# zhenxuan00/graphical-gan

Measured on AMD Instinct MI355X. Metric: images/sec (G+D+GP step) cifar10 32x32 bs=64, higher is better.
Workload: dtype f32; 1 GPU; gan_inference_cifar10.py MODE=wali-gp BATCH_SIZE=64 (per GPU) 32x32x3, CRITIC_ITERS=5; parallelism=dp1, global_batch=64, hip_graph=True, minibatch_feed=device-resident ring, read in place; one graph per iteration, finite_costs=True

## Files before the change

graphical_gan_amd/_lib.py:

```python
import ctypes as C
import os

_HERE = os.path.dirname(os.path.abspath(__file__))
LIB_PATH = os.path.join(_HERE, 'libggan.so')

ACT_NONE, ACT_LRELU, ACT_RELU, ACT_TANH, ACT_SIGMOID = 0, 1, 2, 3, 4
PACK_MAX = 64
HEAD_BCE_MAX_ROWS = 2048
BCE_HEADS = 2
PACK_ARRIVE_INTS = 33 * 1024
POSTERIOR_MAX_K = 8192
MODE_K = {'CONCRETE': 0, 'STRAIGHT_THROUGHT_CONCRETE': 1, 'STRAIGHT_THROUGHT': 2}
BCE_MAX = 16
TSNE_MAX_K = 128
TSNE_MAX_SPLITS = 64
ABI_VERSION = 800


class ConvGeom(C.Structure):
    _fields_ = [(n, C.c_int) for n in ('N', 'Ci', 'H', 'W', 'Co', 'Ho', 'Wo', 'k', 'stride', 'pad_t', 'pad_l',
                                       'plan_wgs', 'plan_wgs_filter', 'plan_flags')]


PLAN_PLAIN = 1


class ProfRec(C.Structure):
    _fields_ = [('name', C.c_char * 48), ('total_ms', C.c_double), ('launches', C.c_long),
                ('flops', C.c_double), ('bytes', C.c_double), ('grid', C.c_long)]


class GganError(RuntimeError):
    pass


_P = C.c_void_p
_F = C.c_float
_I = C.c_int
_Z = C.c_size_t
_G = C.POINTER(ConvGeom)

SIGNATURES = {
    'ggan_version': (_I, []),
    'ggan_last_error': (C.c_char_p, []),
    'ggan_conv2d_workspace': (_Z, [_G]),
    'ggan_conv2d_fwd': (_I, [_G, _P, _P, _P, _P, _I, _F, _P, _Z, _P]),
    'ggan_conv2d_bwd_data': (_I, [_G, _P, _P, _P, _P, _I, _F, _P, _Z, _P]),
    'ggan_conv2d_bwd_filter': (_I, [_G, _P, _P, _P, _P, _P, _Z, _P]),
    'ggan_conv2d_bwd_data_act': (_I, [_G, _P, _P, _I, _F, _P, _P, _P, _Z, _P]),
    'ggan_conv2d_bwd_filter_act': (_I, [_G, _P, _P, _P, _I, _F, _P, _P, _P, _Z, _P]),
    'ggan_conv2d_bwd_filter_parts': (_I, [_G, _P, _P, _P, _I, _F, _I, _P, _Z, C.POINTER(_I), C.POINTER(_Z), _P]),
    'ggan_conv2d_fwd_cast_ring': (_I, [_G, _P, _I, _P, _P, _I, _P, _F, _F, _P, _P, _P, _P, _I, _F, _P]),
    'ggan_conv2d_fwd_masked': (_I, [_G, _P, _P, _P, _P, _I, _F, _P, _Z, _P]),
    'ggan_linear_bn_rows_fwd': (_I, [_P, _P, _P, _P, _P, _P, _P, _P, _P, _I, _I, _I, _F, _I, _F, _P]),
    'ggan_linear_bn_rows_bwd': (_I, [_P, _P, _P, _P, _P, _P, _P, _P, _P, _P, _P, _I, _I, _I, _I, _F, _P]),
    'ggan_deconv2d_fwd': (_I, [_G, _P, _P, _P, _P, _I, _F, _P, _Z, _P]),
    'ggan_deconv2d_bwd_data': (_I, [_G, _P, _P, _P, _P, _Z, _P]),
    'ggan_deconv2d_bwd_filter': (_I, [_G, _P, _P, _P, _P, _P, _Z, _P]),
    'ggan_gemm_workspace': (_Z, [_I, _I, _I]),
    'ggan_gemm': (_I, [_I, _I, _I, _I, _I, _P, _P, _P, _P, _I, _F, _P, _Z, _P]),
    'ggan_conv3d_out_shape': (_I, [_P, _P]),
    'ggan_im2col3d': (_I, [_P, _P, _P, _P]),
    'ggan_col2im3d': (_I, [_P, _P, _P, _P]),
    'ggan_conv3d_igemm_ok': (_I, [_P, _I]),
    'ggan_conv3d_fwd': (_I, [_P, _P, _P, _P, _P, _I, _F, _P, _Z, _P]),
    'ggan_conv3d_wgrad': (_I, [_P, _P, _P, _P, _P, _Z, _P]),
    'ggan_conv3d_dgrad': (_I, [_P, _P, _P, _P, _P]),
    'ggan_mix_rbf_mmd2_fwd': (_I, [_P, _P, _I, _I, _I, _P, _P, _I, _P, _P, _P]),
    'ggan_mix_rbf_mmd2_bwd': (_I, [_P, _P, _I, _I, _I, _P, _P, _I, _P, _P, _P, _P]),
    'ggan_noise_fill': (_I, [_P, _P, _P, _P, _P, _P, _I, _P, _P]),
    'ggan_gmm_latent_fwd': (_I, [_P, _P, _P, _P, _P, _I, _I, _I, _F, _F, _P]),
    'ggan_gmm_latent_bwd': (_I, [_P, _P, _P, _P, _P, _P, _P, _I, _I, _I, _F, _P]),
    'ggan_gmm_latent_st_fwd': (_I, [_P, _P, _P, _P, _P, _P, _I, _I, _I, _F, _F, _I, _P]),
    'ggan_gmm_latent_st_bwd': (_I, [_P, _P, _P, _P, _P, _P, _P, _I, _I, _I, _F, _I, _P]),
    'ggan_gmm_posterior_assign': (_I, [_P, _P, _F, _I, _I, _I, _I, _P, _P, _P, _P]),
    'ggan_cluster_accuracy': (_I, [_P, _P, _P, _I, _I, _P, _P]),
    'ggan_video_sheet_u8': (_I, [_P, _P, _P, _P, _I, _I, _I, _I, _I, _I, _I, _I, _I, _F, _F, _F, _P]),
    'ggan_tsne_sqnorms': (_I, [_P, _I, _I, _P, _P]),
    'ggan_tsne_neighbours': (_I, [_P, _P, _I, _I, _I, _I, _I, _P, _P, _P, _P, _Z, _P]),
    'ggan_tsne_affinities': (_I, [_P, _I, _I, _F, _I, _F, _P, _P, _P]),
    'ggan_tsne_symmetrise': (_I, [_P, _P, _I, _I, _P, _P, _P, _P, _P]),
    'ggan_tsne_gradient': (_I, [_P, _P, _P, _P, _I, _I, _P, _P, _P, _P, _P, _P]),
    'ggan_tsne_kl': (_I, [_P, _P, _P, _P, _I, _I, _P, _P, _P, _P, _P]),
    'ggan_tsne_iterate': (_I, [_P, _P, _P, _P, _P, _P, _P, _I, _I, _P, _P, _I, _I, _I, _F, _F, _F, _F, _F, _P]),
    'ggan_gemm_split': (_I, [_I, _I, _I, _I, _I, _P, _P, _I, _P, _P, _P, _P, _I, _P, _I, _F, _P, _Z, _P]),
    'ggan_gemm_colsum': (_I, [_I, _I, _I, _I, _P, _P, _P, _P, _P, _Z, _P]),
    'ggan_dyn_scan_fwd': (_I, [_I, _I, _I, _I, _I, _P, _P, _P, _P, _P, _P, _P, _P, _P, _P, _F, _P, _P, _P, _P]),
    'ggan_dyn_scan_bwd': (_I, [_I, _I, _I, _I, _I, _P, _P, _P, _P, _P, _P, _P, _P, _P, _F, _P, _P, _P, _P, _P, _P, _P]),
    'ggan_critic_head_fwd': (_I, [_I, _I, _I, _I, _P, _P, _P, _P, _P, _P, _F, _P, _P, _P, _Z, _P]),
    'ggan_critic_head_bwd': (_I, [_I, _I, _I, _I, _P, _P, _P, _P, _P, _P, _F, _P, _P, _P, _P, _P, _P, _P, _P, _Z, _P]),
    'ggan_critic_head_fwd_bce': (_I, [_I, _I, _I, _I, _P, _P, _P, _P, _P, _P, _F, _P, _P, _I, _I, _P, _P, _P, _P, _P, _P, _Z, _P]),
    'ggan_critic_head_bwd_tail': (_I, [_I, _I, _I, _I, _P, _P, _P, _P, _P, _F, _P, _P, _P, _P, _P, _P, _P, _P, _P, _I, _I, _P, _P, _P, _P, _P, _P, _Z, _P]),
    'ggan_linear_bwd_data_act': (_I, [_I, _I, _I, _P, _P, _I, _F, _P, _P, _P, _Z, _P]),
    'ggan_linear_bwd_weight_act': (_I, [_I, _I, _I, _P, _P, _P, _I, _F, _P, _P, _P, _Z, _P]),
    'ggan_colsum': (_I, [_P, _P, _I, _I, _P]),
    'ggan_reparam_fwd': (_I, [_P, _P, _P, _P, _P, _Z, _P]),
    'ggan_reparam_bwd': (_I, [_P, _P, _P, _P, _P, _P, _Z, _P]),
    'ggan_agg_div_fwd': (_I, [_I, _P, _P, _P, _P, _P, _I, _I, _I, _I, _P, _P, _P, _P, _P, _P]),
    'ggan_agg_div_bwd': (_I, [_I, _P, _P, _P, _P, _I, _I, _I, _I, _P, _P, _P, _P, _P, _P, _P, _P, _P]),
    'ggan_colsum_tall': (_I, [_P, _P, _I, _I, _P, _Z, _P]),
    'ggan_chansum': (_I, [_P, _P, _I, _I, _I, _P, _Z, _P]),
    'ggan_bn_fwd_train': (_I, [_P, _P, _P, _P, _P, _P, _I, _I, _I, _F, _I, _F, _P]),
    'ggan_bn_bwd': (_I, [_P, _P, _P, _P, _P, _P, _P, _P, _I, _I, _I, _P]),
    'ggan_bn_bwd_act': (_I, [_P, _P, _P, _I, _F, _P, _P, _P, _P, _P, _P, _P, _I, _I, _I, _P]),
    'ggan_bn_bwd_bwd': (_I, [_P, _P, _P, _I, _F, _P, _P, _P, _P, _P, _P, _P, _I, _I, _I, _P]),
    'ggan_bn_split_fwd_train': (_I, [_P, _P, _P, _P, _P, _P, _I, _I, _I, _I, _F, _I, _F, _P, _Z, _P]),
    'ggan_bn_split_bwd_act': (_I, [_P, _P, _I, _F, _P, _P, _P, _P, _P, _P, _P, _P, _I, _I, _I, _I, _I, _P, _Z, _P]),
    'ggan_bn_sync_stats': (_I, [_P, _P, _I, _I, _I, _P]),
    'ggan_bn_sync_apply': (_I, [_P, _P, _I, _P, _P, _P, _P, _P, _I, _I, _I, _F, _I, _F, _P]),
    'ggan_bn_sync_bwd_stats': (_I, [_P, _P, _P, _I, _F, _P, _P, _P, _I, _I, _I, _P]),
    'ggan_bn_sync_bwd_apply': (_I, [_P, _P, _P, _I, _F, _P, _P, _P, _P, _I, _I, _P, _P, _P, _I, _I, _I, _P]),
    'ggan_act_fwd': (_I, [_P, _P, _Z, _I, _F, _P]),
    'ggan_act_bwd': (_I, [_P, _P, _P, _Z, _I, _F, _P]),
    'ggan_act_bwd_chansum': (_I, [_P, _P, _P, _P, _I, C.POINTER(_I), _I, _I, _I, _I, _F, _P]),
    'ggan_bias_add': (_I, [_P, _P, _P, _I, _I, _I, _P]),
    'ggan_cast_scale_i32': (_I, [_P, _P, _P, _Z, _F, _F, _P]),
    'ggan_cast_scale_ring_i32': (_I, [_P, _I, _P, _P, _I, _P, _P, _Z, _F, _F, _P]),
    'ggan_axpby': (_I, [_P, _P, _P, _Z, _F, _F, _F, _P]),
    'ggan_mix_mean': (_I, [_P, _P, _P, _P, _I, _I, _I, _P]),
    'ggan_row_lerp': (_I, [_P, _P, _P, _P, _I, _I, _P]),
    'ggan_bce_logits_fwd': (_I, [_P, _F, _F, _P, _I, _I, _P]),
    'ggan_bce_logits_bwd': (_I, [_P, _F, _F, _P, _P, _I, _P]),
    'ggan_bce_logits_multi_fwd': (_I, [C.POINTER(_P), C.POINTER(_F), C.POINTER(_F), C.POINTER(_I), _I, _P, _P]),
    'ggan_bce_logits_multi_bwd': (_I, [C.POINTER(_P), C.POINTER(_F), C.POINTER(_F), C.POINTER(_I), _I, _P, C.POINTER(_P), _P]),
    'ggan_bce_logits_multi_fwd_grad': (_I, [C.POINTER(_P), C.POINTER(_F), C.POINTER(_F), C.POINTER(_I), _I, _P, C.POINTER(_P), _P]),
    'ggan_bce_head_bwd': (_I, [C.POINTER(_P), C.POINTER(_F), C.POINTER(_F), C.POINTER(_I), _I, _P, C.POINTER(_P), _I, _I, _P, _P, _F, _P, _P,
                          _P, _P]),
    'ggan_bce_heads_bwd': (_I, [C.POINTER(_P), C.POINTER(_F), C.POINTER(_F), C.POINTER(_I), _I, _P, C.POINTER(_P), _I, C.POINTER(_I),
                           C.POINTER(_I), C.POINTER(_I), C.POINTER(_P), C.POINTER(_P), C.POINTER(_F), C.POINTER(_P), C.POINTER(_P),
                           C.POINTER(_P), _P]),
    'ggan_mean_fwd': (_I, [_P, _F, _P, _I, _I, _P]),
    'ggan_mean_bwd': (_I, [_P, _F, _P, _I, _P]),
    'ggan_mean_multi_fwd_grad': (_I, [C.POINTER(_P), C.POINTER(_F), C.POINTER(_I), _I, _P, C.POINTER(_P), _P]),
    'ggan_dist_fwd': (_I, [_P, _P, _P, _Z, _I, _F, _I, _P]),
    'ggan_dist_bwd': (_I, [_P, _P, _P, _P, _P, _Z, _I, _F, _P]),
    'ggan_gp_penalty_fwd': (_I, [_P, _P, _P, _I, _I, _F, _P]),
    'ggan_gp_penalty_bwd': (_I, [_P, _P, _P, _P, _I, _I, _F, _P]),
    'ggan_gp_penalty_fwd_grad': (_I, [_P, _P, _P, _P, _P, _I, _I, _F, _P]),
    'ggan_adam_step': (_I, [_P, _P, _P, _P, _Z, _P, _F, _F, _F, _F, _F, _P]),
    'ggan_adam_advance': (_I, [_P, _P]),
    'ggan_rmsprop_step': (_I, [_P, _P, _P, _Z, _F, _F, _F, _F, _F, _F, _P]),
    'ggan_adam_step_counted': (_I, [_P, _P, _P, _P, _Z, _P, _F, _F, _F, _F, _F, _P]),
    'ggan_pack': (_I, [C.POINTER(_P), C.POINTER(_Z), C.POINTER(_Z), _I, _P, _P]),
    'ggan_pack_parts': (_I, [C.POINTER(_P), C.POINTER(_Z), C.POINTER(_Z), C.POINTER(_I), C.POINTER(_Z), _I, _P, _P, _P]),
    'ggan_pack_parts2': (_I, [C.POINTER(_P), C.POINTER(_Z), C.POINTER(_Z), C.POINTER(_I), C.POINTER(_Z), C.POINTER(_P), C.POINTER(_I),
                              C.POINTER(_Z), _I, _P, _P, _P]),
    'ggan_pack_adam': (_I, [C.POINTER(_P), C.POINTER(_Z), C.POINTER(_Z), C.POINTER(_I), C.POINTER(_Z), C.POINTER(_P), C.POINTER(_I),
                            C.POINTER(_Z), _I, _P, _P, _P, _P, _P, _P, _F, _F, _F, _F, _F, _P]),
    'ggan_prof_enable': (_I, [_I]),
    'ggan_prof_reset': (_I, []),
    'ggan_prof_report': (_I, [C.POINTER(ProfRec), _I]),
}

_lib = None


def load():
    global _lib
    if _lib is not None:
        return _lib
    if not os.path.exists(LIB_PATH):
        raise GganError('libggan.so not found at %s -- run `python -c "import __graft_entry__ as g; g.build()"` '
                        '(there is no CPU fallback)' % LIB_PATH)
    lib = C.CDLL(LIB_PATH)
    for name, (res, args) in SIGNATURES.items():
        try:
            fn = getattr(lib, name)
        except AttributeError:
            raise GganError('libggan.so does not export %s' % name)
        fn.restype = res
        fn.argtypes = args
    if lib.ggan_version() != ABI_VERSION:
        raise GganError('libggan.so speaks ABI version %d, this binding %d: a stale build -- run `python -c "import __graft_entry__ as g; g.build()"`'
                        % (lib.ggan_version(), ABI_VERSION))
    _lib = lib
    return lib


def check(rc, what):
    if rc != 0:
        msg = load().ggan_last_error()
        raise GganError('%s failed (%d): %s' % (what, rc, msg.decode() if msg else ''))


def prof_report(cap=256):
    lib = load()
    recs = (ProfRec * cap)()
    n = lib.ggan_prof_report(recs, cap)
    out = []
    for i in range(n):
        r = recs[i]
        out.append(dict(name=r.name.decode(), total_ms=r.total_ms, launches=int(r.launches),
                        flops=r.flops, bytes=r.bytes, grid=int(r.grid)))
    return out
```

graphical_gan_amd/csrc/conv.h:

```cpp
#pragma once
#include "common.h"

namespace ggan {

int conv_fwd_naive(const ggan_conv_geom& g, const float* x, const float* w, const float* bias, float* y, int act,
                   float alpha, hipStream_t s);
struct GyMask {
    const float* ref;
    int act;
    float alpha;
};
int conv_dgrad_naive(const ggan_conv_geom& g, const float* gy, GyMask m, const float* w, const float* bias, float* gx,
                     int act, float alpha, hipStream_t s);
int conv_wgrad_naive(const ggan_conv_geom& g, const float* x, const float* gy, GyMask m, float* gw, hipStream_t s);

constexpr int kTargetWgs = 200;
struct OutMask {
    const float* ref;
    int act;
    float alpha;
    bool applied;
};
int conv_fwd_mfma(const ggan_conv_geom& g, const float* x, const float* w, const float* bias, float* y, int act,
                  float alpha, void* ws, size_t ws_bytes, hipStream_t s, OutMask* mask = nullptr);
int conv_dgrad_mfma(const ggan_conv_geom& g, const float* gy, GyMask m, const float* w, const float* bias, float* gx,
                    int act, float alpha, void* ws, size_t ws_bytes, hipStream_t s);
int conv_dgrad_dg16(const ggan_conv_geom& g, const float* gy, GyMask m, const float* w, const float* bias, float* gx, int act,
                    float alpha, int target_wgs, void* ws, size_t ws_bytes, hipStream_t s);
int conv_dgrad_thin(const ggan_conv_geom& g, const float* gy, GyMask m, const float* w, const float* bias, float* gx, int act,
                    float alpha, hipStream_t s);
struct WgradParts {
    float* buf;
    size_t cap_floats;
    int with_bias;
    int n;
    size_t stride;
};
int conv_wgrad_mfma(const ggan_conv_geom& g, const float* x, const float* gy, GyMask m, float* gw, float* gbias, void* ws,
                    size_t ws_bytes, hipStream_t s, WgradParts* parts = nullptr);
struct ThinCastSrc {
    const int32_t* ring;
    const int32_t* ctr_a;
    const int32_t* ctr_b;
    const float* noise;
    float* x_out;
    int nslots, offset;
    float div, mul;
};
int conv_fwd_thin(const ggan_conv_geom& g, const float* x, const float* w, const float* bias, float* y, int act, float alpha,
                  hipStream_t s, const ThinCastSrc* cast = nullptr, const OutMask* mask = nullptr);
int conv_wgrad_thin(const ggan_conv_geom& g, const float* x, const float* gy, GyMask m, float* gw, float* gbias, void* ws,
                    size_t ws_bytes, hipStream_t s, WgradParts* parts = nullptr);
size_t conv_workspace_bytes(const ggan_conv_geom& g);
int launch_splitk_reduce(const float* partial, int SK, size_t elems, float* out, const float* bias, int C, int HW, int act,
                         float alpha, hipStream_t s, size_t slab_stride = 0, float* tail_out = nullptr, size_t tail = 0);

struct FastDiv {
    uint32_t mul, d;
};
inline FastDiv make_fastdiv(uint32_t d) {
    FastDiv f;
    f.d = d;
    f.mul = (d <= 1) ? 0u : (uint32_t)((0x100000000ull / d) + 1ull);
    return f;
}
__device__ __forceinline__ uint32_t fdiv(uint32_t n, FastDiv f) { return f.d <= 1 ? n : __umulhi(n, f.mul); }

struct FastDiv24 {
    uint32_t mul, shift;
};
inline bool make_fastdiv24(uint32_t d, uint32_t nmax, FastDiv24* out) {
    if (d <= 1) { out->mul = 1; out->shift = 0; return true; }
    for (int s = 31; s >= 1; --s) {
        const uint64_t m = ((1ull << s) + d - 1) / d;
        if (m >= (1ull << 24) || m * nmax >= (1ull << 32)) continue;
        const uint64_t err = m * d - (1ull << s);
        if ((uint64_t)nmax * err >= (1ull << s)) return false;
        out->mul = (uint32_t)m; out->shift = (uint32_t)s;
        return true;
    }
    return false;
}
__device__ __forceinline__ uint32_t fdiv24(uint32_t n, FastDiv24 f) { return __umul24(n, f.mul) >> f.shift; }

}
```

graphical_gan_amd/csrc/conv_corr.hip:

```cpp
#include "common.h"
#include "conv.h"
#include <stdlib.h>
#include <map>
#include <mutex>
#include <vector>
using namespace ggan;

namespace {

constexpr int XE_MAX = 24;
constexpr unsigned OOB = 0x7FFFFFF0u;
typedef unsigned int u32x4 __attribute__((ext_vector_type(4)));

__host__ __device__ inline int fwd_region(int data_floats, int lanes_used, int floats_per_lane) {
    const int tail = (((lanes_used + 63) & ~63) - lanes_used) * floats_per_lane;
    return (data_floats + (tail > 4 ? tail : 4) + 3) & ~3;
}

struct CorrClass {
    int Hu, Wv;
    int roff, coff;
    int or0, oc0;
    int wbase;
    int pad_;
// ... 910 lines not shown
    const std::vector<int> key = {dev, P.CKtot, P.Hin, P.Win, P.TI, P.TR, P.TC, P.SR, P.SCp, P.CS, xq, P.row0, P.col0, CK, nthr, P.tiles_r, P.tiles_c, su};
    std::lock_guard<std::mutex> lk(g_xtab_mu);
    auto it = g_xtabs.find(key);
    if (it != g_xtabs.end()) return it->second;
    hipStreamCaptureStatus st = hipStreamCaptureStatusNone;
    if (hipStreamIsCapturing(s, &st) != hipSuccess || st != hipStreamCaptureStatusNone) { (void)hipGetLastError(); return nullptr; }
    const int CSu = P.CS / xq, SCpu = P.SCp / xq, srsc = P.SR * SCpu, xe_cnt = CK * CSu;
    const int npos = P.tiles_r * P.tiles_c;
    std::vector<unsigned> tab((size_t)npos * XE * nthr, OOB);
    for (int tr = 0; tr < P.tiles_r; ++tr)
        for (int tc = 0; tc < P.tiles_c; ++tc) {
            const int in_row0 = su * tr * P.TR + P.row0, in_col0 = su * tc * P.TC + P.col0;
            for (int j = 0; j < XE; ++j)
                for (int tid = 0; tid < nthr; ++tid) {
                    const int e = tid + j * nthr;
                    if (e >= xe_cnt) continue;
                    const int ckl = e / CSu, r1 = e - ckl * CSu;
                    const int img = r1 / srsc, r2 = r1 - img * srsc;
                    const int r = r2 / SCpu, cc = (r2 - r * SCpu) * xq;
                    const int ih = in_row0 + r, iw = in_col0 + cc;
                    if (img >= P.TI || ih < 0 || ih >= P.Hin || iw < 0 || iw >= P.Win) continue;
                    tab[((size_t)(tr * P.tiles_c + tc) * XE + j) * nthr + tid] = (unsigned)((((size_t)img * P.CKtot + ckl) * P.Hin + ih) * P.Win + iw) * 4u;
                }
        }
    unsigned* d = nullptr;
    if (hipMalloc((void**)&d, tab.size() * sizeof(unsigned)) != hipSuccess) { (void)hipGetLastError(); return nullptr; }
    if (hipMemcpy(d, tab.data(), tab.size() * sizeof(unsigned), hipMemcpyHostToDevice) != hipSuccess) { (void)hipGetLastError(); (void)hipFree(d); return nullptr; }
    g_xtabs[key] = d;
    return d;
}

template <int MODE>
int plan_and_launch(CorrParams& P, int Hu, int Wv, int su, int ext_r, int ext_c, int ntaps, int groups, float* dst,
                    const float* bias, int act, float alpha, void* ws, size_t ws_bytes, hipStream_t s, const char* name,
                    double fl, const char* sk_env, OutMask* mask = nullptr) {
    const int target = P.plan_wgs > 0 ? P.plan_wgs : kTargetWgs;
    const WaveCfg* kCfgs = MODE == 1 ? kCfgsDgrad : kCfgsFwd;
    static const int order_fwd[4] = {8, 6, 4, 5}, order_all[4] = {8, 6, 7, 5};
    const int* order = MODE == 2 ? order_all : order_fwd;
    int cfg = 5;
    for (int oi = MODE == 0 ? 0 : 1; oi < 4; ++oi) {
        const int c = order[oi];
        const WaveCfg& wc = kCfgs[c];
        const int CK = 2 * wc.KS * wc.PW, TM = 32 * wc.WM, TNW = 32 * wc.WN;
        if (P.CNtot <= 32 && TNW > 32) continue;
        CorrParams T = P;
        if (!pick_tile(T, Hu, Wv, TM, CK, su, ext_r, ext_c)) continue;
        if (oi < 3 && T.TI * T.TR * T.TC * 2 <= TM && Hu * Wv * P.N >= TM) continue;
        const int wgs = cdiv(P.N, T.TI) * cdiv(Hu, T.TR) * cdiv(Wv, T.TC) * cdiv(P.CNtot, TNW) * groups;
        if (oi == 0 && wgs >= 2 * target) continue;
        if (wgs >= target || oi == 3) { cfg = c; break; }
    }
    if (P.CKtot < 8) cfg = P.CNtot <= 32 ? 1 : 6;
    const WaveCfg& wc = kCfgs[cfg];
    const int CK = 2 * wc.KS * wc.PW, TM = 32 * wc.WM, TNW = 32 * wc.WN;
    if (!pick_tile(P, Hu, Wv, TM, CK, su, ext_r, ext_c)) return 1;
    P.dbg = env_int("GGAN_DBG", 0);
    P.dma = (MODE == 0 || (CK % 16 == 0 && wc.PW <= 2)) && (P.dbg & 3) == 0;
    const int RS = TNW + (MODE != 0 ? 2 : 0);
    P.xq = 1;
    if (MODE == 0 && cfg >= 4 && P.dma && (P.Win & 3) == 0 && (((uintptr_t)P.in) & 15) == 0 && ((su * P.TC) & 3) == 0) {
        const int shift = ((P.col0 % 4) + 4) % 4;
        const int scp4 = (P.SCp + shift + 3) & ~3;
        const size_t cs4 = (size_t)P.TI * P.SR * scp4;
        const int wregion = fwd_region(ntaps * CK * RS, ntaps * CK * (TNW / 4), 4);
        const size_t stage4 = 2 * ((size_t)fwd_region((int)(CK * cs4), (int)(CK * cs4 / 4), 4) + (size_t)wregion);
        const size_t stage1 = 2 * ((size_t)fwd_region(CK * P.CS, CK * P.CS, 1) + (size_t)wregion);
        const bool crosses = stage1 * sizeof(float) <= 80 * 1024 && stage4 * sizeof(float) > 80 * 1024;
        if (stage4 * sizeof(float) <= 160 * 1024 && CK * cs4 / 4 <= (size_t)XE_MAX * 256 && !crosses) {
            P.xq = 4;
            P.col0 -= shift;
            for (int c = 0; c < 4; ++c) P.cls[c].coff += shift;
            P.SCp = scp4;
            P.CS = (int)cs4;
        }
    }
    if (MODE != 0 && dgrad_x4_cfg(MODE, cfg) && (P.Win & 3) == 0 && (((uintptr_t)P.in) & 15) == 0 &&
        (((uintptr_t)P.in_ref) & 15) == 0 && ((su * P.TC) & 3) == 0) {
        const int shift = ((P.col0 % 4) + 4) % 4;
        const int scp4 = (P.SCp + shift + 3) & ~3;
        const size_t cs4 = (size_t)P.TI * P.SR * scp4;
        const int nthr = 64 * wc.WM * wc.WN * wc.KS;
        const int xn = ((XE_MAX / 2) * 256 / nthr + 3) / 4 + 1;
        const size_t stage4 = 2 * ((size_t)((CK * cs4 + 1 + 3) & ~(size_t)3) + (size_t)((ntaps * CK * RS + 4 * RS + 3) & ~3));
        if (stage4 * sizeof(float) <= 160 * 1024 && CK * cs4 / 4 <= (size_t)xn * nthr) {
            P.xq = 4;
            P.col0 -= shift;
            for (int c = 0; c < 4; ++c) P.cls[c].coff += shift;
            P.SCp = scp4;
            P.CS = (int)cs4;
        }
    }
    if (!finish_tile(P, Hu, Wv)) return 1;
    if ((size_t)P.N * P.CKtot * P.Hin >= (1u << 24)) return 1;
    const int gx = P.img_groups * P.tiles_r * P.tiles_c, gy = cdiv(P.CNtot, TNW);
    int sk = env_int(sk_env, 0);
    if (sk <= 0) {
        sk = 1;
        const int base = gx * gy * groups;
        if (base < target / 2) {
            sk = target / base;
            const int max_sk = P.CKtot / (2 * CK);
            if (sk > max_sk) sk = max_sk;
            if (sk > 16) sk = 16;
        }
    }
    if (sk < 1) sk = 1;
    P.cps = cdiv(cdiv(P.CKtot, sk), CK) * CK;
    P.SK = cdiv(P.CKtot, P.cps);
    if (P.SK > 1 && (size_t)P.SK * P.out_elems * sizeof(float) > ws_bytes) {
        P.SK = 1;
        P.cps = cdiv(P.CKtot, CK) * CK;
    }
    P.out = P.SK > 1 ? (float*)ws : dst;
    P.bias = bias; P.act = act; P.alpha = alpha;
    if (mask) {
        if (MODE != 0 || P.SK != 1) return 1;
        P.out_ref = mask->ref; P.out_act = mask->act; P.out_alpha = mask->alpha;
        mask->applied = true;
    }
    if ((P.dbg & 4) && ws && ws_bytes > (64u << 20)) P.stamps = (unsigned long long*)((char*)ws + ws_bytes - (32u << 20));
    size_t stage = MODE == 0 ? 2 * ((size_t)fwd_region(CK * P.CS, CK * P.CS / P.xq, P.xq) + (size_t)fwd_region(ntaps * CK * RS, ntaps * CK * (TNW / 4), 4))
                             : 2 * ((size_t)((CK * P.CS + 1 + 3) & ~3) + (size_t)((ntaps * CK * RS + 4 * RS + 3) & ~3));
    size_t red = (size_t)wc.KS * (MODE == 2 ? 4 : (MODE == 1 ? 2 : 1)) * TNW * TM;
    P.nstg = 2;
    if (MODE == 0 && P.dma) P.xtab = fwd_slab_table(P, CK, 64 * wc.WM * wc.WN * wc.KS, su, s);
    const size_t shmem = (stage > red ? stage : red) * sizeof(float);
    {
        P.xcd_p = 0;
        if ((gx * gy) % 8 == 0) {
            double best = (gx % 8 == 0) ? (double)P.in_bytes + 8.0 * P.w_bytes : 8.0 * ((double)P.in_bytes + P.w_bytes);
            for (int p = 1; p <= 8; p *= 2) {
                if (gx % p || gy % (8 / p)) continue;
                const double cost = 8.0 * P.in_bytes / p + (double)P.w_bytes * p;
                if (cost < 0.9 * best) { best = cost; P.xcd_p = p; }
            }
        }
    }
    int rc = launch_cfg<MODE>(cfg, P, dim3(gx, gy, groups * P.SK), shmem, s, name, fl);
    if (rc) return rc;
    if (P.SK > 1)
        return launch_splitk_reduce((const float*)ws, P.SK, P.out_elems, dst, bias, P.CNtot, P.Hout * P.Wout, act, alpha, s);
    return 0;
}

}

namespace ggan {

int launch_splitk_reduce(const float* partial, int SK, size_t elems, float* out, const float* bias, int C, int HW, int act,
                         float alpha, hipStream_t s, size_t slab_stride, float* tail_out, size_t tail) {
    if (slab_stride == 0) slab_stride = elems;
    if (!tail_out) tail = 0;
    if (SK >= 8 && elems + tail <= 65536) {
        GGAN_LAUNCH("splitk_reduce_small_k", 0, 4.0 * (elems + tail) * (SK + 1), splitk_reduce_small_k,
                    dim3((int)((elems + tail + 63) / 64)), dim3(256), 0, s, partial, SK, elems, slab_stride, out, bias, C, HW, act,
                    alpha, tail_out, tail);
        return 0;
    }
    size_t b = (elems + tail + 255) / 256;
    if (b > 2048) b = 2048;
    GGAN_LAUNCH("splitk_reduce_k", 0, 4.0 * (elems + tail) * (SK + 1), splitk_reduce_k, dim3((int)b), dim3(256), 0, s, partial,
                SK, elems, slab_stride, out, bias, C, HW, act, alpha, tail_out, tail);
    return 0;
}

size_t conv_workspace_bytes(const ggan_conv_geom& g) {
    size_t big = (size_t)g.N * g.Ci * g.H * g.W, small_ = (size_t)g.N * g.Co * g.Ho * g.Wo;
    size_t wsz = (size_t)g.k * g.k * g.Ci * g.Co;
    size_t m = big > small_ ? big : small_;
    size_t a = 16 * m * sizeof(float), b = 64 * wsz * sizeof(float);
    return a > b ? a : b;
}

static bool hot_geometry(const ggan_conv_geom& g) { return g.k == 5 && g.stride == 2; }
static bool fits32(size_t bytes) { return bytes < 0x7FFFFFF0ull; }

int conv_fwd_mfma(const ggan_conv_geom& g, const float* x, const float* w, const float* bias, float* y, int act,
                  float alpha, void* ws, size_t ws_bytes, hipStream_t s, OutMask* mask) {
    if (!hot_geometry(g) || (g.Co & 3)) return 1;
    ws = ws_scratch(ws, ws_bytes);
    const size_t in_bytes = (size_t)g.N * g.Ci * g.H * g.W * 4, w_bytes = (size_t)25 * g.Ci * g.Co * 4;
    if (!fits32(in_bytes) || !fits32(w_bytes) || !fits32((size_t)g.N * g.Co * g.Ho * g.Wo * 4)) return 1;
    if (((uintptr_t)w & 15) != 0) return 1;
    CorrParams P;
    memset(&P, 0, sizeof(P));
    P.in = x; P.w = w;
    P.plan_wgs = g.plan_wgs;
    P.in_bytes = (unsigned)in_bytes; P.w_bytes = (unsigned)w_bytes;
    P.N = g.N; P.CKtot = g.Ci; P.Hin = g.H; P.Win = g.W;
    P.CNtot = g.Co; P.Hout = g.Ho; P.Wout = g.Wo;
    P.ors = 1; P.ocs = 1;
    P.w_si = g.k * g.Ci * g.Co; P.w_sj = g.Ci * g.Co; P.w_sk = g.Co; P.w_sn = 1;
    P.row0 = -g.pad_t; P.col0 = -g.pad_l;
    CorrClass& c = P.cls[0];
    c.Hu = g.Ho; c.Wv = g.Wo; c.roff = 0; c.coff = 0; c.or0 = 0; c.oc0 = 0; c.wbase = 0;
    P.out_elems = (size_t)g.N * g.Co * g.Ho * g.Wo;
    const double fl = 2.0 * P.out_elems * g.Ci * 25.0;
    return plan_and_launch<0>(P, g.Ho, g.Wo, 2, 5, 5, 25, 1, y, bias, act, alpha, ws, ws_bytes, s, "conv_fwd_mfma", fl,
                              "GGAN_FWD_SK", mask);
}

int conv_dgrad_mfma(const ggan_conv_geom& g, const float* gy, GyMask m, const float* w, const float* bias, float* gx,
                    int act, float alpha, void* ws, size_t ws_bytes, hipStream_t s) {
    if (!hot_geometry(g)) return 1;
    ws = ws_scratch(ws, ws_bytes);
    if ((g.Co & 3) || ((uintptr_t)w & 15)) return 1;
    const size_t in_bytes = (size_t)g.N * g.Co * g.Ho * g.Wo * 4, w_bytes = (size_t)25 * g.Ci * g.Co * 4;
    if (!fits32(in_bytes) || !fits32(w_bytes) || !fits32((size_t)g.N * g.Ci * g.H * g.W * 4)) return 1;
    const int S = 2;
    CorrParams P;
    memset(&P, 0, sizeof(P));
    P.in = gy; P.w = w;
    P.plan_wgs = g.plan_wgs;
    if (m.act != GGAN_ACT_NONE && m.act != GGAN_ACT_LRELU && m.act != GGAN_ACT_RELU) return 1;
    if (m.act != GGAN_ACT_NONE) { P.in_ref = m.ref; P.in_act = m.act; P.in_alpha = m.alpha; }
    P.in_bytes = (unsigned)in_bytes; P.w_bytes = (unsigned)w_bytes;
    P.N = g.N; P.CKtot = g.Co; P.Hin = g.Ho; P.Win = g.Wo;
    P.CNtot = g.Ci; P.Hout = g.H; P.Wout = g.W;
    P.ors = S; P.ocs = S;
    P.w_si = S * g.k * g.Ci * g.Co; P.w_sj = S * g.Ci * g.Co; P.w_sk = 1; P.w_sn = g.Co;
    int offs[2][2], bases[2][2], cnt[2][2], th[2][2], lo[2], hi[2];
    for (int d = 0; d < 2; ++d) {
        const int pad = d == 0 ? g.pad_t : g.pad_l, L = d == 0 ? g.H : g.W;
        lo[d] = 1 << 30; hi[d] = -(1 << 30);
        for (int p = 0; p < S; ++p) {
            const int off = ((p - pad) % S + S) % S;
            offs[d][p] = off;
            bases[d][p] = (off + pad - p) / S;
            cnt[d][p] = off < L ? (L - off + S - 1) / S : 0;
            th[d][p] = (g.k - p + S - 1) / S;
            if (bases[d][p] - (th[d][p] - 1) < lo[d]) lo[d] = bases[d][p] - (th[d][p] - 1);
            if (bases[d][p] > hi[d]) hi[d] = bases[d][p];
        }
    }
    const int Hu = cnt[0][0] > cnt[0][1] ? cnt[0][0] : cnt[0][1];
    const int Wv = cnt[1][0] > cnt[1][1] ? cnt[1][0] : cnt[1][1];
    P.row0 = lo[0]; P.col0 = lo[1];
    for (int ph = 0; ph < S; ++ph)
        for (int pw = 0; pw < S; ++pw) {
            CorrClass& c = P.cls[ph * 2 + pw];
            c.Hu = cnt[0][ph]; c.Wv = cnt[1][pw];
            c.roff = bases[0][ph] - lo[0]; c.coff = bases[1][pw] - lo[1];
            c.or0 = offs[0][ph]; c.oc0 = offs[1][pw];
            c.wbase = (ph * g.k + pw) * g.Ci * g.Co;
        }
    P.out_elems = (size_t)g.N * g.Ci * g.H * g.W;
    const double fl = 2.0 * g.N * g.Co * g.Ho * g.Wo * (double)g.Ci * 25.0;
    const long wgs_all = (long)cdiv(g.N * Hu * Wv, 32) * cdiv(g.Ci, 32);
    if (wgs_all >= (g.plan_wgs > 0 ? g.plan_wgs : kTargetWgs))
        return plan_and_launch<2>(P, Hu, Wv, 1, hi[0] - lo[0] + 1, hi[1] - lo[1] + 1, 25, 1, gx, bias, act, alpha, ws, ws_bytes,
                                  s, "conv_dgrad_mfma", fl, "GGAN_DGRAD_SK");
    return plan_and_launch<1>(P, Hu, Wv, 1, hi[0] - lo[0] + 1, hi[1] - lo[1] + 1, 13, 2, gx, bias, act, alpha, ws, ws_bytes,
                              s, "conv_dgrad_mfma", fl, "GGAN_DGRAD_SK");
}

}
```

graphical_gan_amd/csrc/gemm.hip:

```cpp
#include "common.h"
#include "conv.h"
#include <stdlib.h>
using namespace ggan;

namespace {

constexpr int BM = 64, BN = 64, BK = 16, LDP = 68;
constexpr int KSTEP = 32;
constexpr int LDPK = 66;

struct GemmParams {
    const float* A;
    const float* B;
    const float* bias;
    float* C;
    int M, N, K;
    int lda, ldb;
    int kps;
    int SK;
    int vecA, vecB;
    int act;
    float alpha;
    size_t out_elems;
    float* colsum;
// ... 401 lines not shown

template <int NWAVE>
__global__ __launch_bounds__(64 * NWAVE) void gemm_group_kernel(const GemmGroup G) {
    warm_kernarg(G);
    __shared__ __attribute__((aligned(16))) float As[2 * TSZ];
    __shared__ __attribute__((aligned(16))) float Bs[2 * TSZ];
    if (G.has_tail && (int)blockIdx.x >= G.tail.first) {
        head_tail_wg(G.tail, (int)blockIdx.x - G.tail.first, As);
        return;
    }
    int j = 0;
    if (G.n > 1 && (int)blockIdx.x >= G.first[1]) j = 1;
    if (G.n > 2 && (int)blockIdx.x >= G.first[2]) j = 2;
    const int local = blockIdx.x - G.first[j];
    const int bx = local % G.gx[j], by = local / G.gx[j];
    const GemmParams& P = G.p[j];
    switch (G.kind[j]) {
        case 0: gemm_tile<true, false, 0, 1, NWAVE>(P, bx, by, 0, As, Bs); break;
        case 1: gemm_tile<false, true, 0, 1, NWAVE>(P, bx, by, 0, As, Bs); break;
        default: gemm_tile<false, false, 0, 1, NWAVE>(P, bx, by, 0, As, Bs); break;
    }
}

__global__ __launch_bounds__(256) void head_out_fwd_k(const float* __restrict__ part, int SK, size_t slab, const float* __restrict__ b,
                                                      const float* __restrict__ w_out, const float* __restrict__ b_out, float alpha,
                                                      float* __restrict__ h, float* __restrict__ logits, int M, int H) {
    __shared__ float red[4];
    const int tid = threadIdx.x, rl = tid >> 7, t = tid & 127;
    const int row = blockIdx.x * 2 + rl;
    float dot = 0.f;
    if (row < M) {
        for (int c = t * 4; c < H; c += 512) {
            const size_t o = (size_t)row * H + c;
            float4 v = *reinterpret_cast<const float4*>(part + o);
#pragma unroll 8
            for (int s = 1; s < SK; ++s) {
                const float4 u = *reinterpret_cast<const float4*>(part + (size_t)s * slab + o);
                v.x += u.x; v.y += u.y; v.z += u.z; v.w += u.w;
            }
            const float4 bb = *reinterpret_cast<const float4*>(b + c);
            const float4 ww = *reinterpret_cast<const float4*>(w_out + c);
            v.x = fmaxf(alpha * (v.x + bb.x), v.x + bb.x); v.y = fmaxf(alpha * (v.y + bb.y), v.y + bb.y);
            v.z = fmaxf(alpha * (v.z + bb.z), v.z + bb.z); v.w = fmaxf(alpha * (v.w + bb.w), v.w + bb.w);
            *reinterpret_cast<float4*>(h + o) = v;
            dot = fmaf(v.x, ww.x, fmaf(v.y, ww.y, fmaf(v.z, ww.z, fmaf(v.w, ww.w, dot))));
        }
    }
    dot = wave_sum(dot);
    if ((tid & 63) == 0) red[tid >> 6] = dot;
    __syncthreads();
    if (t == 0 && row < M) logits[row] = (red[2 * rl] + red[2 * rl + 1]) + b_out[0];
}

__global__ __launch_bounds__(256) void head_out_fwd_bce_k(const float* __restrict__ part, int SK, size_t slab, const float* __restrict__ b,
                                                          const float* __restrict__ w_out, const float* __restrict__ b_out, float alpha,
                                                          float* __restrict__ h, float* __restrict__ logits, int M, int H,
                                                          const HeadTerms T, float* __restrict__ g_out, float* __restrict__ gh) {
    __shared__ float red[4];
    const int tid = threadIdx.x, rl = tid >> 7, t = tid & 127;
    const int row = blockIdx.x * 2 + rl;
    float dot = 0.f;
    float4 hv[4], wv[4];
#pragma unroll
    for (int it = 0; it < 4; ++it) {
        const int c = t * 4 + it * 512;
        if (row < M && c < H) {
            const size_t o = (size_t)row * H + c;
            float4 v = *reinterpret_cast<const float4*>(part + o);
#pragma unroll 8
            for (int s = 1; s < SK; ++s) {
                const float4 u = *reinterpret_cast<const float4*>(part + (size_t)s * slab + o);
                v.x += u.x; v.y += u.y; v.z += u.z; v.w += u.w;
            }
            const float4 bb = *reinterpret_cast<const float4*>(b + c);
            const float4 ww = *reinterpret_cast<const float4*>(w_out + c);
            v.x = fmaxf(alpha * (v.x + bb.x), v.x + bb.x); v.y = fmaxf(alpha * (v.y + bb.y), v.y + bb.y);
            v.z = fmaxf(alpha * (v.z + bb.z), v.z + bb.z); v.w = fmaxf(alpha * (v.w + bb.w), v.w + bb.w);
            *reinterpret_cast<float4*>(h + o) = v;
            dot = fmaf(v.x, ww.x, fmaf(v.y, ww.y, fmaf(v.z, ww.z, fmaf(v.w, ww.w, dot))));
            hv[it] = v; wv[it] = ww;
        }
    }
    dot = wave_sum(dot);
    if ((tid & 63) == 0) red[tid >> 6] = dot;
    __syncthreads();
    if (row >= M) return;
    const float lg = (red[2 * rl] + red[2 * rl + 1]) + b_out[0];
    if (t == 0) logits[row] = lg;
    float z = 0.f, sc = 0.f;
    {
        int r0 = 0;
        for (int k = 0; k < T.count; ++k) {
            if (T.ext[k]) continue;
            if (row >= r0 && row < r0 + T.rows[k]) { z = T.z[k]; sc = 1.f * T.w[k] / (float)T.rows[k]; }
            r0 += T.rows[k];
        }
    }
    const float gr = T.kind == 1 ? sc : sc * (1.f / (1.f + expf(-lg)) - z);
    if (t == 0) g_out[row] = gr;
#pragma unroll
    for (int it = 0; it < 4; ++it) {
        const int c = t * 4 + it * 512;
        if (c < H) {
            float4 o4;
            o4.x = gr * wv[it].x * (hv[it].x > 0.f ? 1.f : alpha); o4.y = gr * wv[it].y * (hv[it].y > 0.f ? 1.f : alpha);
            o4.z = gr * wv[it].z * (hv[it].z > 0.f ? 1.f : alpha); o4.w = gr * wv[it].w * (hv[it].w > 0.f ? 1.f : alpha);
            *reinterpret_cast<float4*>(gh + (size_t)row * H + c) = o4;
        }
    }
}

__global__ __launch_bounds__(256) void head_out_bwd_k(const float* __restrict__ g, const float* __restrict__ h,
                                                      const float* __restrict__ w_out, float alpha, float* __restrict__ gh,
                                                      float* __restrict__ d_wout, float* __restrict__ d_bout, int M, int H) {
    __shared__ float red[16][16];
    const int tid = threadIdx.x, cl = tid & 15, rg = tid >> 4;
    const int c = blockIdx.x * 16 + cl;
    float acc = 0.f, gs = 0.f;
    if (c < H) {
        const float w = w_out[c];
#pragma unroll 8
        for (int r = rg; r < M; r += 16) {
            const float gr = g[r], hv = h[(size_t)r * H + c];
            gh[(size_t)r * H + c] = gr * w * (hv > 0.f ? 1.f : alpha);
            acc = fmaf(gr, hv, acc);
            gs += gr;
        }
    }
    red[rg][cl] = acc;
    __syncthreads();
    if (rg == 0 && c < H && d_wout)
        d_wout[c] = (((red[0][cl] + red[1][cl]) + (red[2][cl] + red[3][cl])) + ((red[4][cl] + red[5][cl]) + (red[6][cl] + red[7][cl]))) +
                    (((red[8][cl] + red[9][cl]) + (red[10][cl] + red[11][cl])) + ((red[12][cl] + red[13][cl]) + (red[14][cl] + red[15][cl])));
    if (blockIdx.x == 0 && d_bout) {
        __syncthreads();
        if (cl == 0) red[rg][0] = gs;
        __syncthreads();
        if (tid == 0) d_bout[0] = (((red[0][0] + red[1][0]) + (red[2][0] + red[3][0])) + ((red[4][0] + red[5][0]) + (red[6][0] + red[7][0]))) +
                                (((red[8][0] + red[9][0]) + (red[10][0] + red[11][0])) + ((red[12][0] + red[13][0]) + (red[14][0] + red[15][0])));
    }
}

__global__ __launch_bounds__(256) void gemv_rows_k(const float* __restrict__ A, const float* __restrict__ w, const float* __restrict__ bias,
                                                   float* __restrict__ C, int M, int K, int act, float alpha) {
    const int row = blockIdx.x * 4 + (threadIdx.x >> 6), lane = threadIdx.x & 63;
    if (row >= M) return;
    const float* a = A + (size_t)row * K;
    float s = 0.f;
    for (int k = lane; k < K; k += 64) s = fmaf(a[k], w[k], s);
    s = wave_sum(s);
    if (lane == 0) C[row] = act_apply(s + (bias ? bias[0] : 0.f), act, alpha);
}

struct SkinnyParams {
    const float* A; const float* B; const float* bias; float* C; const float* a_ref;
    const float* A2;
    float* C2;
    int a_split, c_split, vecA2;
    int M, N, K, lda, ldb, act, ref_act, vecA, vecB;
    float alpha, ref_alpha;
    unsigned a_bytes, b_bytes, a2_bytes;
};

template <bool TB, bool MASK, int NS>
__global__ __launch_bounds__(512) void gemm_skinny_k(const SkinnyParams P) {
    __shared__ float red[8 * 4 * 64];
    constexpr unsigned SOOB = 0x7FFFFFF0u;
    const int tid = threadIdx.x, lane = tid & 63, l15 = lane & 15, kq = lane >> 4;
    const int wave = __builtin_amdgcn_readfirstlane(tid >> 6);
    const int m = blockIdx.y * 16 + l15, n = blockIdx.x * 16 + l15;
    const auto ra = __builtin_amdgcn_make_buffer_rsrc((void*)P.A, (short)0, (int)P.a_bytes, 0x00020000);
    const auto rr = __builtin_amdgcn_make_buffer_rsrc((void*)(MASK ? P.a_ref : P.A), (short)0, (int)P.a_bytes, 0x00020000);
    const auto rb = __builtin_amdgcn_make_buffer_rsrc((void*)P.B, (short)0, (int)P.b_bytes, 0x00020000);
    const auto ra2 = __builtin_amdgcn_make_buffer_rsrc((void*)(P.A2 ? P.A2 : P.A), (short)0, (int)(P.A2 ? P.a2_bytes : P.a_bytes), 0x00020000);
    const int KA = P.A2 ? P.a_split : P.K;
    float a[NS][4], b[NS][4], r[MASK ? NS : 1][4];
    auto load_kc = [&](decltype(ra) rs, bool vec, int row, bool row_ok, int ld, int kk, int kend, float* dst) {
        const unsigned base = (unsigned)(row * ld + kk) * 4u;
        if (vec) {
            const u32x4g t = __builtin_amdgcn_raw_buffer_load_b128(rs, (row_ok && kk < kend) ? base : SOOB, 0, 0);
            dst[0] = __uint_as_float(t.x); dst[1] = __uint_as_float(t.y); dst[2] = __uint_as_float(t.z); dst[3] = __uint_as_float(t.w);
        } else {
#pragma unroll
            for (int j = 0; j < 4; ++j)
                dst[j] = __uint_as_float(__builtin_amdgcn_raw_buffer_load_b32(rs, (row_ok && kk + j < kend) ? base + 4u * j : SOOB, 0, 0));
        }
    };
#pragma unroll
    for (int i = 0; i < NS; ++i) {
        const int kk = (wave + 8 * i) * 16 + 4 * kq;
        if (P.A2 && (wave + 8 * i) * 16 >= P.a_split) load_kc(ra2, P.vecA2 != 0, m, m < P.M, P.K - P.a_split, kk - P.a_split, P.K - P.a_split, a[i]);
        else load_kc(ra, P.vecA != 0, m, m < P.M, P.lda, kk, KA, a[i]);
        if (MASK) load_kc(rr, P.vecA != 0, m, m < P.M, P.lda, kk, P.K, r[i]);
        if (TB) load_kc(rb, P.vecB != 0, n, n < P.N, P.ldb, kk, P.K, b[i]);
        else {
#pragma unroll
            for (int j = 0; j < 4; ++j)
                b[i][j] = __uint_as_float(__builtin_amdgcn_raw_buffer_load_b32(rb, (n < P.N && kk + j < P.K) ? (unsigned)((kk + j) * P.ldb + n) * 4u : SOOB, 0, 0));
        }
    }
    f32x4 acc = {0.f, 0.f, 0.f, 0.f};
#pragma unroll
    for (int i = 0; i < NS; ++i)
#pragma unroll
        for (int j = 0; j < 4; ++j) {
            const float av = MASK ? act_grad(a[i][j], r[i][j], P.ref_act, P.ref_alpha) : a[i][j];
            acc = __builtin_amdgcn_mfma_f32_16x16x4f32(av, b[i][j], acc, 0, 0, 0);
        }
#pragma unroll
    for (int q = 0; q < 4; ++q) red[(wave * 4 + q) * 64 + lane] = acc[q];
    __syncthreads();
    if (tid < 256) {
        const int q = tid >> 6;
        float v = red[q * 64 + lane];
#pragma unroll
        for (int w = 1; w < 8; ++w) v += red[(w * 4 + q) * 64 + lane];
        const int row = blockIdx.y * 16 + 4 * kq + q;
        if (row < P.M && n < P.N) {
            if (P.bias) v += P.bias[n];
            v = act_apply(v, P.act, P.alpha);
            if (P.C2 && n >= P.c_split) P.C2[(size_t)row * (P.N - P.c_split) + (n - P.c_split)] = v;
            else P.C[(size_t)row * (P.C2 ? P.c_split : P.N) + n] = v;
        }
    }
}

inline bool al16(const void* p) { return ((uintptr_t)p & 15) == 0; }

}

extern "C" {

size_t ggan_gemm_workspace(int M, int N, int K) {
    (void)K;
    return (size_t)64 * M * N * sizeof(float);
}

constexpr int kSplitTarget = 256;
constexpr int kHeadSplitTarget = 512;

struct GemmPlan {
    GemmParams P;
    int gx, gy;
    void* ws;
};

static int gemm_plan(GemmPlan& G, int mode, int ta, int tb, int M, int N, int K, const float* A, const float* B, const float* bias,
                     float* C, float* colsum, int act, float alpha, void* ws, size_t ws_bytes, const float* a_ref = nullptr,
                     const float* b_ref = nullptr, int ref_act = 0, float ref_alpha = 0.f, const float* A2 = nullptr,
                     int a_split = 0, float* C2 = nullptr, int c_split = 0, int split_target = kSplitTarget) {
    GemmParams& P = G.P;
    memset(&P, 0, sizeof(P));
    P.a_ref = a_ref; P.b_ref = b_ref; P.ref_act = ref_act; P.ref_alpha = ref_alpha;
    P.A = A; P.B = B; P.bias = bias; P.C = C;
    P.M = M; P.N = N; P.K = K;
    P.lda = ta ? M : K;
    P.ldb = tb ? K : N;
    if (A2) {
        const int whole = ta ? M : K;
        if (a_split <= 0 || a_split >= whole || (a_split % 64) || a_ref) { set_error("gemm: bad operand split"); return -1; }
        P.A2 = A2; P.a_split = a_split;
        P.lda = a_split; P.lda2 = whole - a_split;
    }
    if (C2) {
        if (c_split <= 0 || c_split >= N || (c_split % BN) || colsum || bias || act != GGAN_ACT_NONE) { set_error("gemm: bad output split"); return -1; }
        P.C2 = C2; P.c_split = c_split;
    }
    P.vecA = al16(A) && (P.lda % 4 == 0) && (!a_ref || al16(a_ref)) && (!A2 || (al16(A2) && P.lda2 % 4 == 0));
    P.vecB = al16(B) && (P.ldb % 4 == 0) && (!b_ref || al16(b_ref));
    P.act = act; P.alpha = alpha;
    P.out_elems = (size_t)M * N;
    P.colsum = colsum;
    ws = ws_scratch(ws, ws_bytes);
    G.ws = ws;
    const int gx = cdiv(N, BN), gy = cdiv(M, BM);
    G.gx = gx; G.gy = gy;
    int sk = 1;
    if (mode == 0 && ws && !C2) {
        const char* e = getenv("GGAN_GEMM_SK");
        if (e) sk = atoi(e);
        else {
            const int base = gx * gy;
            const bool tall = K >= 16384;
            sk = (tall ? 1024 : split_target) / base;
            const int max_sk = K / BK;
            if (sk > max_sk) sk = max_sk;
            if (sk > (tall ? 256 : split_target / 4)) sk = tall ? 256 : split_target / 4;
            if (K <= 128 && base >= 32) sk = 1;
        }
        if (sk < 1) sk = 1;
        if (colsum && !(gx * gy < 64 && K >= 512)) sk = 1;
        while (sk > 1 && (size_t)sk * (P.out_elems + (colsum ? N : 0)) * sizeof(float) > ws_bytes) sk /= 2;
    }
    const int kq = (A2 && !ta) ? KSTEP : BK;
    P.kps = cdiv(cdiv(K, sk), kq) * kq;
    P.SK = cdiv(K, P.kps);
    P.slab_stride = P.out_elems + ((colsum && P.SK > 1) ? (size_t)N : 0);
    if (P.SK > 1) {
        P.C = (float*)ws;
        if (colsum) P.colsum = (float*)ws + P.out_elems;
    }
    const size_t szA = (size_t)(A2 ? (ta ? (size_t)K * a_split : (size_t)M * a_split) : (size_t)M * K) * 4;
    const size_t szA2 = A2 ? (size_t)(ta ? (size_t)K * (M - a_split) : (size_t)M * (K - a_split)) * 4 : 0;
    const size_t szB = (size_t)N * K * 4;
    const bool dims4 = (K % 4 == 0) && (P.kps % 4 == 0) && (ta ? (M % 4 == 0 && (!A2 || a_split % 4 == 0)) : true) && (tb ? true : N % 4 == 0);
    const bool small = szA < 0x7FFFFFF0ull && szA2 < 0x7FFFFFF0ull && szB < 0x7FFFFFF0ull;
    P.fast = !small ? 0 : ((P.vecA && P.vecB && dims4) ? 1 : 2);
    P.a_bytes = (unsigned)szA; P.a2_bytes = (unsigned)szA2; P.b_bytes = (unsigned)szB;
    return 0;
}

static int gemm_launch_planned(const GemmPlan& G, int ta, int tb, hipStream_t s) {
    const GemmParams& P = G.P;
    const double fl = 2.0 * P.M * P.N * (double)P.K;
    const dim3 grid(G.gx, G.gy, P.SK), block(256);
    const bool w8 = P.fast != 0 && P.kps >= 2 * KSTEP;
#define GGAN_GEMM_CASE(TA_, TB_, MK_, NAME_)                                                                                      \
    do {                                                                                                                           \
        if (w8 && P.fast == 1) { GGAN_LAUNCH("gemm_kernel8" NAME_, fl, 0, (gemm_kernel8<TA_, TB_, MK_, 1>), grid, dim3(512), 0, s, P); }   \
        else if (w8) { GGAN_LAUNCH("gemm_kernel8" NAME_, fl, 0, (gemm_kernel8<TA_, TB_, MK_, 2>), grid, dim3(512), 0, s, P); }            \
        else if (P.fast == 1) { GGAN_LAUNCH("gemm_kernel" NAME_, fl, 0, (gemm_kernel<TA_, TB_, MK_, 1>), grid, block, 0, s, P); }              \
        else if (P.fast == 2) { GGAN_LAUNCH("gemm_kernel" NAME_, fl, 0, (gemm_kernel<TA_, TB_, MK_, 2>), grid, block, 0, s, P); }               \
        else { GGAN_LAUNCH("gemm_kernel" NAME_, fl, 0, (gemm_kernel<TA_, TB_, MK_, 0>), grid, block, 0, s, P); }                                \
    } while (0)
    if (P.a_ref || P.b_ref) {
        if (P.a_ref && !P.b_ref && !ta && tb) GGAN_GEMM_CASE(false, true, 1, "<false, true, 1>");
        else if (P.b_ref && !P.a_ref && ta && !tb) GGAN_GEMM_CASE(true, false, 2, "<true, false, 2>");
        else { set_error("gemm: unsupported mask/transposition combination"); return -1; }
    } else
    if (!ta && !tb) GGAN_GEMM_CASE(false, false, 0, "<false, false>");
    else if (!ta && tb) GGAN_GEMM_CASE(false, true, 0, "<false, true>");
    else if (ta && !tb) GGAN_GEMM_CASE(true, false, 0, "<true, false>");
    else GGAN_GEMM_CASE(true, true, 0, "<true, true>");
#undef GGAN_GEMM_CASE
    return 0;
}

static int gemm_launch(int ta, int tb, int M, int N, int K, const float* A, const float* B, const float* bias, float* C,
                       float* colsum, int act, float alpha, void* ws, size_t ws_bytes, hipStream_t s,
                       const float* a_ref = nullptr, const float* b_ref = nullptr, int ref_act = 0, float ref_alpha = 0.f,
                       const float* A2 = nullptr, int a_split = 0, float* C2 = nullptr, int c_split = 0) {
    if (N == 1 && !ta && !tb && !colsum && !a_ref && !b_ref) {
        GGAN_LAUNCH("gemv_rows_k", 2.0 * M * K, 0, gemv_rows_k, dim3(cdiv(M, 4)), dim3(256), 0, s, A, B, bias, C, M, K, act, alpha);
        return 0;
    }
    if (!ta && !colsum && (!A2 || (a_split % 16 == 0 && !a_ref)) && (!C2 || c_split % 16 == 0) && !b_ref && (!a_ref || tb) && M >= 32 &&
        K >= 64 && K <= 1024 && cdiv(M, BM) * cdiv(N, BN) < 64 &&
        cdiv(M, 16) * cdiv(N, 16) <= 1024 && !(K <= 128 && cdiv(M, BM) * cdiv(N, BN) >= 32) && (size_t)M * K * 4 < 0x7FFFFFF0ull &&
        (size_t)N * K * 4 < 0x7FFFFFF0ull) {
        SkinnyParams P;
        memset(&P, 0, sizeof(P));
        P.A = A; P.B = B; P.bias = bias; P.C = C; P.a_ref = a_ref;
        P.M = M; P.N = N; P.K = K; P.lda = A2 ? a_split : K; P.ldb = tb ? K : N;
        P.act = act; P.alpha = alpha; P.ref_act = ref_act; P.ref_alpha = ref_alpha;
        P.A2 = A2; P.a_split = a_split; P.C2 = C2; P.c_split = c_split;
        P.vecA = al16(A) && (P.lda % 4 == 0) && (!a_ref || al16(a_ref));
        P.vecA2 = A2 && al16(A2) && ((K - a_split) % 4 == 0);
        P.vecB = tb && al16(B) && (K % 4 == 0);
        P.a_bytes = (unsigned)((size_t)M * P.lda * 4); P.a2_bytes = A2 ? (unsigned)((size_t)M * (K - a_split) * 4) : 0u;
        P.b_bytes = (unsigned)((size_t)N * K * 4);
        const int steps = cdiv(cdiv(K, 16), 8);
        const int ns = steps <= 1 ? 1 : (steps <= 2 ? 2 : (steps <= 4 ? 4 : 8));
        const dim3 grid(cdiv(N, 16), cdiv(M, 16));
        const double fl = 2.0 * M * N * (double)K;
#define GGAN_SKINNY_NS(TB_, MK_, NAME_)                                                                                              \
        do {                                                                                                                         \
            if (ns == 1) { GGAN_LAUNCH("gemm_skinny_k" NAME_, fl, 0, (gemm_skinny_k<TB_, MK_, 1>), grid, dim3(512), 0, s, P); }      \
            else if (ns == 2) { GGAN_LAUNCH("gemm_skinny_k" NAME_, fl, 0, (gemm_skinny_k<TB_, MK_, 2>), grid, dim3(512), 0, s, P); } \
            else if (ns == 4) { GGAN_LAUNCH("gemm_skinny_k" NAME_, fl, 0, (gemm_skinny_k<TB_, MK_, 4>), grid, dim3(512), 0, s, P); } \
            else { GGAN_LAUNCH("gemm_skinny_k" NAME_, fl, 0, (gemm_skinny_k<TB_, MK_, 8>), grid, dim3(512), 0, s, P); }              \
        } while (0)
        if (a_ref) GGAN_SKINNY_NS(true, true, "<true, true>");
        else if (tb) GGAN_SKINNY_NS(true, false, "<true, false>");
        else GGAN_SKINNY_NS(false, false, "<false, false>");
#undef GGAN_SKINNY_NS
        return 0;
    }
    GemmPlan G;
    int rc = gemm_plan(G, 0, ta, tb, M, N, K, A, B, bias, C, colsum, act, alpha, ws, ws_bytes, a_ref, b_ref, ref_act, ref_alpha, A2,
                       a_split, C2, c_split);
    if (rc) return rc;
    rc = gemm_launch_planned(G, ta, tb, s);
    if (rc) return rc;
    if (G.P.SK > 1)
        return launch_splitk_reduce((const float*)G.ws, G.P.SK, G.P.out_elems, C, bias, N, 1, act, alpha, s, G.P.slab_stride, colsum,
                                    colsum ? (size_t)N : 0);
    return 0;
}

int ggan_critic_head_fwd(int M, int K1, int K2, int H, const float* a1, const float* a2, const float* w, const float* b,
                         const float* w_out, const float* b_out, float alpha, float* h, float* logits, void* ws, size_t ws_bytes,
                         ggan_stream_t stream) {
    GGAN_CHECK_ARG(a1 && w && b && w_out && b_out && h && logits, "null pointer");
    GGAN_CHECK_ARG(M > 0 && K1 > 0 && K2 >= 0 && H > 0 && (H % 4) == 0 && (a2 || K2 == 0), "bad shape");
    GGAN_CHECK_ARG(al16(b) && al16(w_out) && al16(h), "b, w_out, h must be 16-byte aligned");
    hipStream_t s = (hipStream_t)stream;
    GemmPlan G;
    int rc = gemm_plan(G, 0, 0, 0, M, H, K1 + K2, a1, w, nullptr, h, nullptr, GGAN_ACT_NONE, 0.f, ws, ws_bytes, nullptr, nullptr, 0, 0.f,
                       K2 ? a2 : nullptr, K2 ? K1 : 0, nullptr, 0, kHeadSplitTarget);
    if (rc) return rc;
    rc = gemm_launch_planned(G, 0, 0, s);
    if (rc) return rc;
    const float* part = G.P.SK > 1 ? (const float*)G.ws : h;
    GGAN_LAUNCH("head_out_fwd_k", 2.0 * M * H, 4.0 * M * H * (G.P.SK + 1), head_out_fwd_k, dim3(cdiv(M, 2)), dim3(256), 0, s, part,
                G.P.SK, G.P.slab_stride, b, w_out, b_out, alpha, h, logits, M, H);
    return 0;
}

static int head_terms(HeadTerms& T, int M, int kind, int nterms, const int* rows, const float* labels, const float* weights,
                      const float* const* ext) {
    memset(&T, 0, sizeof(T));
    if (nterms < 1 || nterms > 4 || !rows || !labels || !weights || kind < 0 || kind > 1) return -1;
    int tot = 0;
    for (int k = 0; k < nterms; ++k) {
        if (rows[k] <= 0) return -1;
        T.rows[k] = rows[k]; T.z[k] = labels[k]; T.w[k] = weights[k];
        T.ext[k] = ext ? ext[k] : nullptr;
        if (!T.ext[k]) tot += rows[k];
    }
    T.count = nterms; T.kind = kind;
    return tot == M ? 0 : -1;
}

int ggan_critic_head_fwd_bce(int M, int K1, int K2, int H, const float* a1, const float* a2, const float* w, const float* b,
                             const float* w_out, const float* b_out, float alpha, float* h, float* logits, int kind, int nterms,
                             const int* term_rows, const float* labels, const float* weights, float* g, float* gh, void* ws,
                             size_t ws_bytes, ggan_stream_t stream) {
    GGAN_CHECK_ARG(a1 && w && b && w_out && b_out && h && logits && g && gh, "null pointer");
    GGAN_CHECK_ARG(M > 0 && K1 > 0 && K2 >= 0 && H > 0 && (H % 4) == 0 && H <= 2048 && (a2 || K2 == 0), "bad shape");
    GGAN_CHECK_ARG(al16(b) && al16(w_out) && al16(h) && al16(gh), "b, w_out, h, gh must be 16-byte aligned");
    HeadTerms T;
    GGAN_CHECK_ARG(head_terms(T, M, kind, nterms, term_rows, labels, weights, nullptr) == 0, "terms must be 1..4 row ranges covering the M rows");
    hipStream_t s = (hipStream_t)stream;
    GemmPlan G;
    int rc = gemm_plan(G, 0, 0, 0, M, H, K1 + K2, a1, w, nullptr, h, nullptr, GGAN_ACT_NONE, 0.f, ws, ws_bytes, nullptr, nullptr, 0, 0.f,
                       K2 ? a2 : nullptr, K2 ? K1 : 0, nullptr, 0, kHeadSplitTarget);
    if (rc) return rc;
    rc = gemm_launch_planned(G, 0, 0, s);
    if (rc) return rc;
    const float* part = G.P.SK > 1 ? (const float*)G.ws : h;
    GGAN_LAUNCH("head_out_fwd_bce_k", 5.0 * M * H, 4.0 * M * H * (G.P.SK + 2), head_out_fwd_bce_k, dim3(cdiv(M, 2)), dim3(256), 0, s, part,
                G.P.SK, G.P.slab_stride, b, w_out, b_out, alpha, h, logits, M, H, T, g, gh);
    return 0;
}

static int critic_head_bwd_impl(int M, int K1, int K2, int H, const float* g, const float* a1, const float* a2, const float* w, const float* h,
                                const float* w_out, float alpha, float* gh, float* d_a1, float* d_a2, float* d_w, float* d_b, float* d_wout,
                                float* d_bout, void* ws, size_t ws_bytes, ggan_stream_t stream, const HeadTail* tail) {
    GGAN_CHECK_ARG(a1 && w && h && w_out && gh, "null pointer");
    GGAN_CHECK_ARG(M > 0 && K1 > 0 && K2 >= 0 && H > 0 && (a2 || K2 == 0), "bad shape");
    GGAN_CHECK_ARG(!d_a1 || K2 == 0 || d_a2, "d_a2 missing");
    GGAN_CHECK_ARG(!d_b || d_w, "d_b comes out of the weight-gradient product");
    hipStream_t s = (hipStream_t)stream;
    const int K = K1 + K2;
    if (g) {
        GGAN_LAUNCH("head_out_bwd_k", 3.0 * M * H, 8.0 * M * H, head_out_bwd_k, dim3(cdiv(H, 16)), dim3(256), 0, s, g, h, w_out, alpha, gh,
                    d_wout, d_bout, M, H);
    }
    GemmPlan Gw, Ga;
    int nw = 0, na = 0;
    if (d_w) {
        int rc = gemm_plan(Gw, 1, 1, 0, K, H, M, a1, gh, nullptr, d_w, d_b, GGAN_ACT_NONE, 0.f, ws, ws_bytes, nullptr, nullptr, 0, 0.f,
                           K2 ? a2 : nullptr, K2 ? K1 : 0);
        if (rc) return rc;
        nw = 1;
    }
    if (d_a1) {
        int rc = gemm_plan(Ga, 1, 0, 1, M, K, H, gh, w, nullptr, d_a1, nullptr, GGAN_ACT_NONE, 0.f, ws, ws_bytes, nullptr, nullptr, 0, 0.f,
                           nullptr, 0, K2 ? d_a2 : nullptr, K2 ? K1 : 0);
        if (rc) return rc;
        na = 1;
    }
    if (nw && na && Gw.P.fast == 1 && Ga.P.fast == 1) {
        GemmGroup GG;
        memset(&GG, 0, sizeof(GG));
        GG.n = 2;
        GG.kind[0] = 1; GG.gx[0] = Ga.gx; GG.p[0] = Ga.P; GG.first[0] = 0;
        GG.kind[1] = 0; GG.gx[1] = Gw.gx; GG.p[1] = Gw.P; GG.first[1] = Ga.gx * Ga.gy;
        GG.first[2] = GG.first[1] + Gw.gx * Gw.gy;
        int nwg = GG.first[2];
        if (tail) {
            GG.has_tail = 1;
            GG.tail = *tail;
            GG.tail.first = nwg;
            nwg += 1 + cdiv(H, 16);
        }
        GGAN_LAUNCH("gemm_group_kernel<8>", 4.0 * M * K * (double)H, 0, gemm_group_kernel<8>, dim3(nwg), dim3(512), 0, s, GG);
        return 0;
    }
    if (tail && na && !nw && Ga.P.fast == 1) {
        GemmGroup GG;
        memset(&GG, 0, sizeof(GG));
        GG.n = 1;
        GG.kind[0] = 1; GG.gx[0] = Ga.gx; GG.p[0] = Ga.P; GG.first[0] = 0;
        GG.first[1] = Ga.gx * Ga.gy;
        GG.has_tail = 1;
        GG.tail = *tail;
        GG.tail.first = GG.first[1];
        GGAN_LAUNCH("gemm_group_kernel<8>", 2.0 * M * K * (double)H, 0, gemm_group_kernel<8>, dim3(GG.first[1] + 1 + cdiv(H, 16)), dim3(512), 0,
                    s, GG);
        return 0;
    }
    if (tail) {
        HeadTail T = *tail;
        T.first = 0;
        GGAN_LAUNCH("head_tail_k", 3.0 * M * H, 4.0 * M * H, head_tail_k, dim3(1 + cdiv(H, 16)), dim3(256), 0, s, T);
    }
    if (nw) { int rc = gemm_launch_planned(Gw, 1, 0, s); if (rc) return rc; }
    if (na) { int rc = gemm_launch_planned(Ga, 0, 1, s); if (rc) return rc; }
    return 0;
}

int ggan_critic_head_bwd(int M, int K1, int K2, int H, const float* g, const float* a1, const float* a2, const float* w, const float* h,
                         const float* w_out, float alpha, float* gh, float* d_a1, float* d_a2, float* d_w, float* d_b, float* d_wout,
                         float* d_bout, void* ws, size_t ws_bytes, ggan_stream_t stream) {
    return critic_head_bwd_impl(M, K1, K2, H, g, a1, a2, w, h, w_out, alpha, gh, d_a1, d_a2, d_w, d_b, d_wout, d_bout, ws, ws_bytes, stream,
                                nullptr);
}

int ggan_critic_head_bwd_tail(int M, int K1, int K2, int H, const float* a1, const float* a2, const float* w, const float* h,
                              const float* w_out, float alpha, const float* gh, float* d_a1, float* d_a2, float* d_w, float* d_b,
                              float* d_wout, float* d_bout, const float* logits, const float* g, int kind, int nterms, const int* term_rows,
                              const float* labels, const float* weights, const float* const* ext, float* loss, void* ws, size_t ws_bytes,
                              ggan_stream_t stream) {
    GGAN_CHECK_ARG(logits && g && gh, "null pointer");
    HeadTail T;
    memset(&T, 0, sizeof(T));
    GGAN_CHECK_ARG(head_terms(T.terms, M, kind, nterms, term_rows, labels, weights, ext) == 0,
                   "terms must be 1..4: row ranges covering the M rows, plus terms read elsewhere (ext)");
    T.logits = logits; T.g = g; T.h = h; T.d_wout = d_wout; T.d_bout = d_bout; T.loss = loss; T.M = M; T.H = H;
    return critic_head_bwd_impl(M, K1, K2, H, nullptr, a1, a2, w, h, w_out, alpha, const_cast<float*>(gh), d_a1, d_a2, d_w, d_b, d_wout,
                                d_bout, ws, ws_bytes, stream, &T);
}

int ggan_gemm(int ta, int tb, int M, int N, int K, const float* A, const float* B, const float* bias, float* C, int act,
              float alpha, void* ws, size_t ws_bytes, ggan_stream_t stream) {
    GGAN_CHECK_ARG(A && B && C, "null pointer");
    GGAN_CHECK_ARG(M > 0 && N > 0 && K > 0, "bad shape");
    return gemm_launch(ta, tb, M, N, K, A, B, bias, C, nullptr, act, alpha, ws, ws_bytes, (hipStream_t)stream);
}

int ggan_gemm_split(int ta, int tb, int M, int N, int K, const float* A, const float* A2, int a_split, const float* B,
                    const float* bias, float* C, float* C2, int c_split, float* colsum_b, int act, float alpha, void* ws,
                    size_t ws_bytes, ggan_stream_t stream) {
    GGAN_CHECK_ARG(A && B && C, "null pointer");
    GGAN_CHECK_ARG(M > 0 && N > 0 && K > 0, "bad shape");
    GGAN_CHECK_ARG(!colsum_b || !tb, "column sums need B stored [K,N]");
    return gemm_launch(ta, tb, M, N, K, A, B, bias, C, colsum_b, act, alpha, ws, ws_bytes, (hipStream_t)stream, nullptr, nullptr, 0,
                       0.f, A2, a_split, C2, c_split);
}

int ggan_gemm_colsum(int ta, int M, int N, int K, const float* A, const float* B, float* C, float* colsum_b, void* ws,
                     size_t ws_bytes, ggan_stream_t stream) {
    GGAN_CHECK_ARG(A && B && C && colsum_b, "null pointer");
    GGAN_CHECK_ARG(M > 0 && N > 0 && K > 0, "bad shape");
    return gemm_launch(ta, 0, M, N, K, A, B, nullptr, C, colsum_b, GGAN_ACT_NONE, 0.f, ws, ws_bytes, (hipStream_t)stream);
}

int ggan_linear_bwd_data_act(int M, int N, int K, const float* g, const float* y, int y_act, float y_alpha, const float* w,
                             float* dx, void* ws, size_t ws_bytes, ggan_stream_t stream) {
    GGAN_CHECK_ARG(g && w && dx && (y || y_act == GGAN_ACT_NONE), "null pointer");
    GGAN_CHECK_ARG(M > 0 && N > 0 && K > 0, "bad shape");
    return gemm_launch(0, 1, M, K, N, g, w, nullptr, dx, nullptr, GGAN_ACT_NONE, 0.f, ws, ws_bytes, (hipStream_t)stream,
                       y_act != GGAN_ACT_NONE ? y : nullptr, nullptr, y_act, y_alpha);
}

int ggan_linear_bwd_weight_act(int M, int N, int K, const float* x, const float* g, const float* y, int y_act, float y_alpha,
                               float* dw, float* db, void* ws, size_t ws_bytes, ggan_stream_t stream) {
    GGAN_CHECK_ARG(x && g && dw && (y || y_act == GGAN_ACT_NONE), "null pointer");
    GGAN_CHECK_ARG(M > 0 && N > 0 && K > 0, "bad shape");
    return gemm_launch(1, 0, K, N, M, x, g, nullptr, dw, db, GGAN_ACT_NONE, 0.f, ws, ws_bytes, (hipStream_t)stream, nullptr,
                       y_act != GGAN_ACT_NONE ? y : nullptr, y_act, y_alpha);
}

}
```

graphical_gan_amd/csrc/pointwise.hip:

```cpp
#include "common.h"
#include "conv.h"
using namespace ggan;

namespace {

constexpr int kBlock = 256;
inline int grid_for(size_t n, int per_thread = 4) {
    size_t b = cdivz(n, (size_t)kBlock * per_thread);
    if (b < 1) b = 1;
    if (b > 2048) b = 2048;
    return (int)b;
}

__global__ void act_fwd_k(const float* __restrict__ x, float* __restrict__ y, size_t n, int act, float alpha) {
    size_t i = (size_t)blockIdx.x * blockDim.x + threadIdx.x, stride = (size_t)gridDim.x * blockDim.x;
    size_t n4 = n >> 2;
    const float4* x4 = reinterpret_cast<const float4*>(x);
    float4* y4 = reinterpret_cast<float4*>(y);
    for (size_t j = i; j < n4; j += stride) {
        float4 v = x4[j];
        v.x = act_apply(v.x, act, alpha); v.y = act_apply(v.y, act, alpha);
        v.z = act_apply(v.z, act, alpha); v.w = act_apply(v.w, act, alpha);
        y4[j] = v;
    }
// ... 428 lines not shown
            float* gx = t.gx[k];
            const float g = 1.f * t.w[k] / (float)t.n[k];
            for (int i = threadIdx.x; i < t.n[k]; i += blockDim.x) {
                float v = x[i];
                s += fmaxf(v, 0.f) - v * z + log1pf(expf(-fabsf(v)));
                if (gx) gx[i] = g * (1.f / (1.f + expf(-v)) - z);
            }
            s = block_sum(s, sm);
            const float r = t.w[k] * (s / (float)t.n[k]);
            tot = k ? tot + r : r;
        }
        if (threadIdx.x == 0) loss[0] = tot;
        return;
    }
    const int hi = (hs.count > 1 && (int)blockIdx.x >= hs.hd[1].first) ? 1 : 0;
    const BceHead& hd = hs.hd[hi];
    const float* __restrict__ h = hd.h;
    const float* __restrict__ w_out = hd.w_out;
    float* __restrict__ gh = hd.gh;
    float* __restrict__ d_wout = hd.d_wout;
    float* __restrict__ d_bout = hd.d_bout;
    const float alpha = hd.alpha;
    const int M = hd.M, H = hd.H;
    {
        int r0 = 0;
        for (int k = hd.k0; k < hd.k1; ++k) {
            const float g = 1.f * t.w[k] / (float)t.n[k], z = t.z[k];
            for (int i = threadIdx.x; i < t.n[k]; i += blockDim.x) gs_[r0 + i] = g * (1.f / (1.f + expf(-t.x[k][i])) - z);
            r0 += t.n[k];
        }
    }
    __syncthreads();
    const int tid = threadIdx.x, cl = tid & 15, rg = tid >> 4;
    const int c = ((int)blockIdx.x - hd.first) * 16 + cl;
    float acc = 0.f, gsum = 0.f;
    if (c < H) {
        const float w = w_out[c];
#pragma unroll 8
        for (int r = rg; r < M; r += 16) {
            const float gr = gs_[r], hv = h[(size_t)r * H + c];
            gh[(size_t)r * H + c] = gr * w * (hv > 0.f ? 1.f : alpha);
            acc = fmaf(gr, hv, acc);
            gsum += gr;
        }
    }
    red[rg][cl] = acc;
    __syncthreads();
    if (rg == 0 && c < H && d_wout)
        d_wout[c] = (((red[0][cl] + red[1][cl]) + (red[2][cl] + red[3][cl])) + ((red[4][cl] + red[5][cl]) + (red[6][cl] + red[7][cl]))) +
                    (((red[8][cl] + red[9][cl]) + (red[10][cl] + red[11][cl])) + ((red[12][cl] + red[13][cl]) + (red[14][cl] + red[15][cl])));
    if ((int)blockIdx.x == hd.first && d_bout) {
        __syncthreads();
        if (cl == 0) red[rg][0] = gsum;
        __syncthreads();
        if (tid == 0) d_bout[0] = (((red[0][0] + red[1][0]) + (red[2][0] + red[3][0])) + ((red[4][0] + red[5][0]) + (red[6][0] + red[7][0]))) +
                                (((red[8][0] + red[9][0]) + (red[10][0] + red[11][0])) + ((red[12][0] + red[13][0]) + (red[14][0] + red[15][0])));
    }
}

__global__ void bce_multi_bwd_k(BceTable t, const float* __restrict__ gloss) {
    const int k = blockIdx.y;
    const int n = t.n[k];
    const float g = gloss[0] * t.w[k] / (float)n, z = t.z[k];
    const float* x = t.x[k];
    float* gx = t.gx[k];
    for (int i = blockIdx.x * blockDim.x + threadIdx.x; i < n; i += gridDim.x * blockDim.x) {
        float v = x[i];
        float sg = 1.f / (1.f + expf(-v));
        gx[i] = g * (sg - z);
    }
}

__global__ void dist_fwd_k(const float* __restrict__ x, const float* __restrict__ y, float* __restrict__ out, size_t n, int p,
                           float weight, int accumulate) {
    __shared__ float sm[32];
    float s = 0.f;
    for (size_t i = threadIdx.x; i < n; i += blockDim.x) {
        const float d = x[i] - y[i];
        s += p == 2 ? d * d : fabsf(d);
    }
    s = block_sum(s, sm);
    if (threadIdx.x == 0) {
        const float r = weight * (s / (float)n);
        out[0] = accumulate ? out[0] + r : r;
    }
}

__global__ void dist_bwd_k(const float* __restrict__ x, const float* __restrict__ y, const float* __restrict__ gout,
                           float* __restrict__ gx, float* __restrict__ gy, size_t n, int p, float weight) {
    const float g = gout[0] * weight / (float)n;
    for (size_t i = (size_t)blockIdx.x * blockDim.x + threadIdx.x; i < n; i += (size_t)gridDim.x * blockDim.x) {
        const float d = x[i] - y[i];
        const float v = g * (p == 2 ? 2.f * d : (d > 0.f ? 1.f : (d < 0.f ? -1.f : 0.f)));
        if (gx) gx[i] = v;
        if (gy) gy[i] = -v;
    }
}

__global__ void mean_fwd_k(const float* __restrict__ x, float weight, float* __restrict__ loss, int n, int accumulate) {
    __shared__ float sm[32];
    float s = 0.f;
    for (int i = threadIdx.x; i < n; i += blockDim.x) s += x[i];
    s = block_sum(s, sm);
    if (threadIdx.x == 0) {
        float r = weight * (s / (float)n);
        loss[0] = accumulate ? loss[0] + r : r;
    }
}

__global__ void mean_multi_fwd_k(BceTable t, float* __restrict__ loss) {
    __shared__ float sm[32];
    float tot = 0.f;
    for (int k = 0; k < t.count; ++k) {
        const float* x = t.x[k];
        float* gx = t.gx[k];
        const float g = 1.f * t.w[k] / (float)t.n[k];
        float s = 0.f;
        for (int i = threadIdx.x; i < t.n[k]; i += blockDim.x) {
            s += x[i];
            if (gx) gx[i] = g;
        }
        s = block_sum(s, sm);
        const float r = t.w[k] * (s / (float)t.n[k]);
        tot = k ? tot + r : r;
    }
    if (threadIdx.x == 0) loss[0] = tot;
}

__global__ void mean_bwd_k(const float* __restrict__ gloss, float weight, float* __restrict__ gx, int n) {
    const float g = gloss[0] * weight / (float)n;
    for (int i = blockIdx.x * blockDim.x + threadIdx.x; i < n; i += gridDim.x * blockDim.x) gx[i] = g;
}

__global__ void gp_slopes_k(const float* __restrict__ g, float* __restrict__ slopes, int D) {
    __shared__ float sm[32];
    const float* row = g + (size_t)blockIdx.x * D;
    float s = 0.f;
    for (int i = threadIdx.x; i < D; i += blockDim.x) s += row[i] * row[i];
    s = block_sum(s, sm);
    if (threadIdx.x == 0) slopes[blockIdx.x] = sqrtf(s);
}

__global__ void gp_pen_k(const float* __restrict__ slopes, float* __restrict__ pen, int B, float lam) {
    __shared__ float sm[32];
    float s = 0.f;
    for (int i = threadIdx.x; i < B; i += blockDim.x) {
        float d = slopes[i] - 1.f;
        s += d * d;
    }
    s = block_sum(s, sm);
    if (threadIdx.x == 0) pen[0] = lam * (s / (float)B);
}

__global__ void gp_fwd_grad_k(const float* __restrict__ g, float* __restrict__ slopes, float* __restrict__ pen, float* __restrict__ gg,
                              int32_t* __restrict__ arrive, int B, int D, float lam) {
    __shared__ float sm[32];
    __shared__ int last;
    const int b = blockIdx.x;
    const float* row = g + (size_t)b * D;
    float s = 0.f;
    for (int i = threadIdx.x; i < D; i += blockDim.x) s += row[i] * row[i];
    s = block_sum(s, sm);
    const float sl = sqrtf(s);
    const float coef = lam * 2.f * (sl - 1.f) / ((float)B * sl);
    float* orow = gg + (size_t)b * D;
    for (int i = threadIdx.x; i < D; i += blockDim.x) orow[i] = coef * row[i];
    if (threadIdx.x == 0) {
        __hip_atomic_store(slopes + b, sl, __ATOMIC_RELAXED, __HIP_MEMORY_SCOPE_AGENT);
        __threadfence();
        last = atomicAdd(arrive, 1) == B - 1;
    }
    __syncthreads();
    if (!last) return;
    __threadfence();
    float t = 0.f;
    for (int i = threadIdx.x; i < B; i += blockDim.x) {
        const float d = __hip_atomic_load(slopes + i, __ATOMIC_RELAXED, __HIP_MEMORY_SCOPE_AGENT) - 1.f;
        t += d * d;
    }
    t = block_sum(t, sm);
    if (threadIdx.x == 0) {
        pen[0] = lam * (t / (float)B);
        arrive[0] = 0;
    }
}

__global__ void gp_bwd_k(const float* __restrict__ g, const float* __restrict__ slopes, const float* __restrict__ gpen,
                         float* __restrict__ gg, int B, int D, float lam) {
    const int b = blockIdx.x;
    const float s = slopes[b];
    const float coef = gpen[0] * lam * 2.f * (s - 1.f) / ((float)B * s);
    const float* row = g + (size_t)b * D;
    float* orow = gg + (size_t)b * D;
    for (int i = threadIdx.x; i < D; i += blockDim.x) orow[i] = coef * row[i];
}

template <bool PRE>
__global__ void adam_k(float* __restrict__ theta, const float* __restrict__ g, float* __restrict__ m,
                       float* __restrict__ v, size_t n, const int32_t* __restrict__ step, float lr, float b1,
                       float b2, float eps, float gscale) {
    const float t = (float)(step[0] + (PRE ? 0 : 1));
    const float lr_t = lr * sqrtf(1.f - powf(b2, t)) / (1.f - powf(b1, t));
    size_t i = (size_t)blockIdx.x * blockDim.x + threadIdx.x, stride = (size_t)gridDim.x * blockDim.x;
    size_t n4 = n >> 2;
    float4* th4 = reinterpret_cast<float4*>(theta);
    const float4* g4 = reinterpret_cast<const float4*>(g);
    float4* m4 = reinterpret_cast<float4*>(m);
    float4* v4 = reinterpret_cast<float4*>(v);
#define ADAM1(TH, G, M, V)                                     \
    {                                                          \
        float gg = (G) * gscale;                               \
        (M) = b1 * (M) + (1.f - b1) * gg;                      \
        (V) = b2 * (V) + (1.f - b2) * gg * gg;                 \
        (TH) = (TH) - lr_t * (M) / (sqrtf(V) + eps);           \
    }
    for (size_t j = i; j < n4; j += stride) {
        float4 th = th4[j], gg4 = g4[j], mm = m4[j], vv = v4[j];
        ADAM1(th.x, gg4.x, mm.x, vv.x) ADAM1(th.y, gg4.y, mm.y, vv.y)
        ADAM1(th.z, gg4.z, mm.z, vv.z) ADAM1(th.w, gg4.w, mm.w, vv.w)
        th4[j] = th; m4[j] = mm; v4[j] = vv;
    }
    for (size_t j = (n4 << 2) + i; j < n; j += stride) {
        float th = theta[j], mm = m[j], vv = v[j];
        ADAM1(th, g[j], mm, vv)
        theta[j] = th; m[j] = mm; v[j] = vv;
    }
#undef ADAM1
}

__global__ void adam_advance_k(int32_t* step) { step[0] += 1; }

__global__ void rmsprop_k(float* __restrict__ theta, const float* __restrict__ g, float* __restrict__ ms, size_t n, float lr,
                          float decay, float eps, float gscale, float lo, float hi) {
    for (size_t i = (size_t)blockIdx.x * blockDim.x + threadIdx.x; i < n; i += (size_t)gridDim.x * blockDim.x) {
        const float gg = g[i] * gscale;
        const float m = decay * ms[i] + (1.f - decay) * gg * gg;
        ms[i] = m;
        theta[i] = fminf(fmaxf(theta[i] - lr * gg / sqrtf(m + eps), lo), hi);
    }
}

struct PackTable {
    const float* src[GGAN_PACK_MAX];
    size_t size[GGAN_PACK_MAX];
    size_t off[GGAN_PACK_MAX];
    size_t pstride[GGAN_PACK_MAX];
    int parts[GGAN_PACK_MAX];
    const float* src2[GGAN_PACK_MAX];
    size_t pstride2[GGAN_PACK_MAX];
    int parts2[GGAN_PACK_MAX];
    int count;
    int32_t* bump;
    int first[GGAN_PACK_MAX + 1];
};
constexpr int kPackChunk = 4096;
__host__ __device__ inline int pack_chunk(int slabs) { return slabs > 4 ? 1024 : kPackChunk; }

__global__ void pack_k(PackTable t, float* __restrict__ flat) {
    const int k = blockIdx.y;
    const float* s = t.src[k];
    const float* s2 = t.src2[k];
    float* d = flat + t.off[k];
    const size_t n = t.size[k];
    const int np = t.parts[k], np2 = s2 ? t.parts2[k] : 0;
    const size_t ps = t.pstride[k], ps2 = t.pstride2[k];
    const size_t i0 = (size_t)blockIdx.x * blockDim.x + threadIdx.x, stride = (size_t)gridDim.x * blockDim.x;
    if (t.bump && blockIdx.x == 0 && blockIdx.y == 0 && threadIdx.x == 0) t.bump[0] += 1;
    if (s && ((((uintptr_t)s) | ((uintptr_t)d) | ((uintptr_t)s2)) & 15) == 0 && (np == 1 || (ps & 3) == 0) && (np2 <= 1 || (ps2 & 3) == 0)) {
        const size_t n4 = n >> 2;
        float4* d4 = reinterpret_cast<float4*>(d);
        for (size_t i = i0; i < n4; i += stride) {
            float4 a = reinterpret_cast<const float4*>(s)[i];
#pragma unroll 8
            for (int p = 1; p < np; ++p) {
                const float4 b = reinterpret_cast<const float4*>(s + (size_t)p * ps)[i];
                a.x += b.x; a.y += b.y; a.z += b.z; a.w += b.w;
            }
#pragma unroll 8
            for (int p = 0; p < np2; ++p) {
                const float4 b = reinterpret_cast<const float4*>(s2 + (size_t)p * ps2)[i];
                a.x += b.x; a.y += b.y; a.z += b.z; a.w += b.w;
            }
            d4[i] = a;
        }
        for (size_t i = (n4 << 2) + i0; i < n; i += stride) {
            float a = s[i];
            for (int p = 1; p < np; ++p) a += s[(size_t)p * ps + i];
            for (int p = 0; p < np2; ++p) a += s2[(size_t)p * ps2 + i];
            d[i] = a;
        }
    } else {
        for (size_t i = i0; i < n; i += stride) {
            float a = 0.f;
            if (s) {
                a = s[i];
                for (int p = 1; p < np; ++p) a += s[(size_t)p * ps + i];
            }
            for (int p = 0; p < np2; ++p) a += s2[(size_t)p * ps2 + i];
            d[i] = a;
        }
    }
}

__global__ void pack_adam_k(PackTable t, float* __restrict__ flat, float* __restrict__ theta, float* __restrict__ m,
                            float* __restrict__ v, int32_t* __restrict__ arrive, float lr, float b1, float b2, float eps,
                            float gscale) {
    int k = 0;
    while (k + 1 < t.count && (int)blockIdx.x >= t.first[k + 1]) ++k;
    const float* s = t.src[k];
    const float* s2 = t.src2[k];
    const size_t off = t.off[k];
    float* d = flat + off;
    float* th = theta + off;
    float* mp = m + off;
    float* vp = v + off;
    const size_t n = t.size[k];
    const int np = t.parts[k], np2 = s2 ? t.parts2[k] : 0;
    const size_t ps = t.pstride[k], ps2 = t.pstride2[k];
    const int chunk = pack_chunk(t.parts[k] + (s2 ? t.parts2[k] : 0));
// ... 654 lines not shown
    }
    const int threads = HW >= 1024 ? 256 : (HW >= 256 ? 128 : 64);
    float* part = (float*)ws;
    GGAN_LAUNCH("chansum", 0, 4.0 * N * C * HW, chansum_part_k, dim3(C, P), dim3(threads), 0, s, x, part, N, C, HW, P);
    GGAN_LAUNCH("chansum_final", 0, 4.0 * C * P, chansum_final_k, dim3(cdiv(C, 4)), dim3(256), 0, s, (const float*)part, out, C, P);
    return 0;
}

int ggan_bce_logits_fwd(const float* x, float label, float weight, float* loss, int n, int accumulate, ggan_stream_t stream) {
    GGAN_CHECK_ARG(x && loss && n > 0, "bad argument");
    GGAN_LAUNCH("bce_logits_fwd", 0, 4.0 * n, bce_fwd_k, dim3(1), dim3(256), 0, (hipStream_t)stream, x, label, weight, loss, n, accumulate);
    return 0;
}

int ggan_bce_logits_bwd(const float* x, float label, float weight, const float* gloss, float* gx, int n, ggan_stream_t stream) {
    GGAN_CHECK_ARG(x && gloss && gx && n > 0, "bad argument");
    GGAN_LAUNCH("bce_logits_bwd", 0, 8.0 * n, bce_bwd_k, dim3(cdiv(n, 256)), dim3(256), 0, (hipStream_t)stream, x, label, weight, gloss, gx, n);
    return 0;
}

static int bce_table(BceTable& t, const float* const* xs, float* const* gxs, const float* labels, const float* weights,
                     const int* ns, int count, int* max_n) {
    *max_n = 0;
    for (int i = 0; i < count; ++i) {
        if (!xs[i] || ns[i] <= 0 || (gxs && !gxs[i])) return -1;
        t.x[i] = xs[i]; t.gx[i] = gxs ? gxs[i] : nullptr; t.z[i] = labels[i]; t.w[i] = weights[i]; t.n[i] = ns[i];
        if (ns[i] > *max_n) *max_n = ns[i];
    }
    t.count = count;
    return 0;
}

int ggan_bce_logits_multi_fwd(const float* const* xs, const float* labels, const float* weights, const int* ns, int count,
                              float* loss, ggan_stream_t stream) {
    GGAN_CHECK_ARG(xs && labels && weights && ns && loss, "null pointer");
    GGAN_CHECK_ARG(count > 0 && count <= GGAN_BCE_MAX, "count out of range");
    BceTable t;
    int mx;
    GGAN_CHECK_ARG(bce_table(t, xs, nullptr, labels, weights, ns, count, &mx) == 0, "bad term");
    GGAN_LAUNCH("bce_logits_fwd", 0, 4.0 * mx * count, bce_multi_fwd_k, dim3(1), dim3(256), 0, (hipStream_t)stream, t, loss);
    return 0;
}

int ggan_bce_logits_multi_fwd_grad(const float* const* xs, const float* labels, const float* weights, const int* ns, int count,
                                   float* loss, float* const* gxs, ggan_stream_t stream) {
    GGAN_CHECK_ARG(xs && labels && weights && ns && loss && gxs, "null pointer");
    GGAN_CHECK_ARG(count > 0 && count <= GGAN_BCE_MAX, "count out of range");
    BceTable t;
    int mx;
    GGAN_CHECK_ARG(bce_table(t, xs, gxs, labels, weights, ns, count, &mx) == 0, "bad term");
    GGAN_LAUNCH("bce_logits_fwd_grad", 0, 8.0 * mx * count, bce_multi_fwd_k, dim3(1), dim3(256), 0, (hipStream_t)stream, t, loss);
    return 0;
}

int ggan_bce_heads_bwd(const float* const* xs, const float* labels, const float* weights, const int* ns, int count, float* loss,
                       float* const* gxs, int nheads, const int* head_terms, const int* Ms, const int* Hs, const float* const* hs,
                       const float* const* w_outs, const float* alphas, float* const* ghs, float* const* d_wouts,
                       float* const* d_bouts, ggan_stream_t stream) {
    GGAN_CHECK_ARG(xs && labels && weights && ns && loss && gxs && head_terms && Ms && Hs && hs && w_outs && alphas && ghs, "null pointer");
    GGAN_CHECK_ARG(count > 0 && count <= GGAN_BCE_MAX && nheads >= 1 && nheads <= GGAN_BCE_HEADS, "count out of range");
    BceTable t;
    int mx;
    GGAN_CHECK_ARG(bce_table(t, xs, gxs, labels, weights, ns, count, &mx) == 0, "bad term");
    BceHeads H;
    memset(&H, 0, sizeof(H));
    H.count = nheads;
    int k = 0, wg = 1;
    for (int a = 0; a < nheads; ++a) {
        BceHead& d = H.hd[a];
        GGAN_CHECK_ARG(hs[a] && w_outs[a] && ghs[a] && Ms[a] > 0 && Ms[a] <= GGAN_HEAD_BCE_MAX_ROWS && Hs[a] > 0 && head_terms[a] > 0 &&
                       k + head_terms[a] <= count, "bad head");
        d.h = hs[a]; d.w_out = w_outs[a]; d.gh = ghs[a]; d.d_wout = d_wouts ? d_wouts[a] : nullptr; d.d_bout = d_bouts ? d_bouts[a] : nullptr;
        d.alpha = alphas[a]; d.M = Ms[a]; d.H = Hs[a]; d.k0 = k; d.k1 = k + head_terms[a]; d.first = wg;
        int rows = 0;
        for (int i = d.k0; i < d.k1; ++i) {
            GGAN_CHECK_ARG(xs[i] == xs[d.k0] + rows, "a head's terms must be consecutive row ranges of one logits vector");
            rows += ns[i];
        }
        GGAN_CHECK_ARG(rows == d.M, "a head's terms must cover its rows");
        k = d.k1;
        wg += cdiv(d.H, 16);
    }
    GGAN_CHECK_ARG(k == count, "every term belongs to a head");
    GGAN_LAUNCH("bce_head_bwd", 0, 0, bce_head_bwd_k, dim3(wg), dim3(256), 0, (hipStream_t)stream, t, loss, H);
    return 0;
}

int ggan_bce_head_bwd(const float* const* xs, const float* labels, const float* weights, const int* ns, int count, float* loss,
                      float* const* gxs, int M, int H, const float* h, const float* w_out, float alpha, float* gh, float* d_wout,
                      float* d_bout, ggan_stream_t stream) {
    return ggan_bce_heads_bwd(xs, labels, weights, ns, count, loss, gxs, 1, &count, &M, &H, &h, &w_out, &alpha, &gh, &d_wout, &d_bout, stream);
}

int ggan_bce_logits_multi_bwd(const float* const* xs, const float* labels, const float* weights, const int* ns, int count,
                              const float* gloss, float* const* gxs, ggan_stream_t stream) {
    GGAN_CHECK_ARG(xs && labels && weights && ns && gloss && gxs, "null pointer");
    GGAN_CHECK_ARG(count > 0 && count <= GGAN_BCE_MAX, "count out of range");
    BceTable t;
    int mx;
    GGAN_CHECK_ARG(bce_table(t, xs, gxs, labels, weights, ns, count, &mx) == 0, "bad term");
    GGAN_LAUNCH("bce_logits_bwd", 0, 8.0 * mx * count, bce_multi_bwd_k, dim3(cdiv(mx, 256), count), dim3(256), 0,
                (hipStream_t)stream, t, gloss);
    return 0;
}

int ggan_dist_fwd(const float* x, const float* y, float* out, size_t n, int p, float weight, int accumulate, ggan_stream_t stream) {
    GGAN_CHECK_ARG(x && y && out && n > 0 && (p == 1 || p == 2), "bad argument");
    GGAN_LAUNCH("dist_fwd", 0, 8.0 * n, dist_fwd_k, dim3(1), dim3(1024), 0, (hipStream_t)stream, x, y, out, n, p, weight, accumulate);
    return 0;
}

int ggan_dist_bwd(const float* x, const float* y, const float* gout, float* gx, float* gy, size_t n, int p, float weight,
                  ggan_stream_t stream) {
    GGAN_CHECK_ARG(x && y && gout && (gx || gy) && n > 0 && (p == 1 || p == 2), "bad argument");
    GGAN_LAUNCH("dist_bwd", 0, 16.0 * n, dist_bwd_k, dim3(grid_for(n)), dim3(kBlock), 0, (hipStream_t)stream, x, y, gout, gx, gy, n, p, weight);
    return 0;
}

int ggan_mean_fwd(const float* x, float weight, float* loss, int n, int accumulate, ggan_stream_t stream) {
    GGAN_CHECK_ARG(x && loss && n > 0, "bad argument");
    GGAN_LAUNCH("mean_fwd", 0, 4.0 * n, mean_fwd_k, dim3(1), dim3(256), 0, (hipStream_t)stream, x, weight, loss, n, accumulate);
    return 0;
}

int ggan_mean_multi_fwd_grad(const float* const* xs, const float* weights, const int* ns, int count, float* loss, float* const* gxs,
                             ggan_stream_t stream) {
    GGAN_CHECK_ARG(xs && weights && ns && loss, "null pointer");
    GGAN_CHECK_ARG(count > 0 && count <= GGAN_BCE_MAX, "count out of range");
    BceTable t;
    int mx;
    float zeros[GGAN_BCE_MAX] = {0.f};
    GGAN_CHECK_ARG(bce_table(t, xs, gxs, zeros, weights, ns, count, &mx) == 0, "bad term");
    GGAN_LAUNCH("mean_multi_fwd", 0, 8.0 * mx * count, mean_multi_fwd_k, dim3(1), dim3(256), 0, (hipStream_t)stream, t, loss);
    return 0;
}

int ggan_mean_bwd(const float* gloss, float weight, float* gx, int n, ggan_stream_t stream) {
    GGAN_CHECK_ARG(gloss && gx && n > 0, "bad argument");
    GGAN_LAUNCH("mean_bwd", 0, 4.0 * n, mean_bwd_k, dim3(cdiv(n, 256)), dim3(256), 0, (hipStream_t)stream, gloss, weight, gx, n);
    return 0;
}

int ggan_gp_penalty_fwd(const float* g, float* slopes, float* pen, int B, int D, float lam, ggan_stream_t stream) {
    GGAN_CHECK_ARG(g && slopes && pen && B > 0 && D > 0, "bad argument");
    hipStream_t s = (hipStream_t)stream;
    GGAN_LAUNCH("gp_slopes", 0, 4.0 * B * D, gp_slopes_k, dim3(B), dim3(256), 0, s, g, slopes, D);
    GGAN_LAUNCH("gp_penalty", 0, 4.0 * B, gp_pen_k, dim3(1), dim3(256), 0, s, slopes, pen, B, lam);
    return 0;
}

int ggan_gp_penalty_fwd_grad(const float* g, float* slopes, float* pen, float* gg_unit, int32_t* arrive, int B, int D, float lam,
                             ggan_stream_t stream) {
    GGAN_CHECK_ARG(g && slopes && pen && gg_unit && arrive && B > 0 && D > 0, "bad argument");
    GGAN_LAUNCH("gp_fwd_grad", 0, 8.0 * B * D, gp_fwd_grad_k, dim3(B), dim3(256), 0, (hipStream_t)stream, g, slopes, pen, gg_unit, arrive, B, D,
                lam);
    return 0;
}

int ggan_gp_penalty_bwd(const float* g, const float* slopes, const float* gpen, float* gg, int B, int D, float lam, ggan_stream_t stream) {
    GGAN_CHECK_ARG(g && slopes && gpen && gg && B > 0 && D > 0, "bad argument");
    GGAN_LAUNCH("gp_penalty_bwd", 0, 8.0 * B * D, gp_bwd_k, dim3(B), dim3(256), 0, (hipStream_t)stream, g, slopes, gpen, gg, B, D, lam);
    return 0;
}

int ggan_adam_step(float* theta, const float* g, float* m, float* v, size_t n, const int32_t* step, float lr,
                   float beta1, float beta2, float eps, float grad_scale, ggan_stream_t stream) {
    GGAN_CHECK_ARG(theta && g && m && v && step, "null pointer");
    if (n == 0) return 0;
    GGAN_CHECK_ARG(aligned16(theta) && aligned16(g) && aligned16(m) && aligned16(v), "buffers must be 16-byte aligned");
    GGAN_LAUNCH("adam_step", 0, 28.0 * n, adam_k<false>, dim3(grid_for(n, 8)), dim3(kBlock), 0, (hipStream_t)stream, theta, g, m, v, n, step, lr, beta1, beta2, eps, grad_scale);
    return 0;
}

int ggan_adam_step_counted(float* theta, const float* g, float* m, float* v, size_t n, const int32_t* step, float lr,
                           float beta1, float beta2, float eps, float grad_scale, ggan_stream_t stream) {
    GGAN_CHECK_ARG(theta && g && m && v && step, "null pointer");
    if (n == 0) return 0;
    GGAN_CHECK_ARG(aligned16(theta) && aligned16(g) && aligned16(m) && aligned16(v), "buffers must be 16-byte aligned");
    GGAN_LAUNCH("adam_step", 0, 28.0 * n, adam_k<true>, dim3(grid_for(n, 8)), dim3(kBlock), 0, (hipStream_t)stream, theta, g, m, v, n, step, lr, beta1, beta2, eps, grad_scale);
    return 0;
}

int ggan_rmsprop_step(float* theta, const float* g, float* ms, size_t n, float lr, float decay, float eps, float grad_scale,
                      float clip_lo, float clip_hi, ggan_stream_t stream) {
    GGAN_CHECK_ARG(theta && g && ms, "null pointer");
    GGAN_CHECK_ARG(clip_lo <= clip_hi, "empty clip interval");
    if (n == 0) return 0;
    GGAN_LAUNCH("rmsprop_step", 0, 20.0 * n, rmsprop_k, dim3(grid_for(n, 8)), dim3(kBlock), 0, (hipStream_t)stream, theta, g, ms, n, lr,
                decay, eps, grad_scale, clip_lo, clip_hi);
    return 0;
}

int ggan_adam_advance(int32_t* step, ggan_stream_t stream) {
    GGAN_CHECK_ARG(step, "null pointer");
    GGAN_LAUNCH("adam_advance", 0, 8, adam_advance_k, dim3(1), dim3(1), 0, (hipStream_t)stream, step);
    return 0;
}

int ggan_pack_parts2(const float* const* srcs, const size_t* sizes, const size_t* offsets, const int* parts, const size_t* strides,
                     const float* const* srcs2, const int* parts2, const size_t* strides2, int count, float* flat, int32_t* bump,
                     ggan_stream_t stream) {
    GGAN_CHECK_ARG(srcs && sizes && offsets && flat, "null pointer");
    GGAN_CHECK_ARG(count > 0 && count <= GGAN_PACK_MAX, "count out of range");
    PackTable t;
    size_t mx = 0, tot = 0;
    for (int i = 0; i < count; ++i) {
        t.src[i] = srcs[i]; t.size[i] = sizes[i]; t.off[i] = offsets[i];
        t.parts[i] = parts ? parts[i] : 1;
        t.pstride[i] = strides ? strides[i] : 0;
        t.src2[i] = srcs2 ? srcs2[i] : nullptr;
        t.parts2[i] = (srcs2 && parts2) ? parts2[i] : 1;
        t.pstride2[i] = (srcs2 && strides2) ? strides2[i] : 0;
        GGAN_CHECK_ARG(t.parts[i] >= 1 && t.parts2[i] >= 1, "parts must be >= 1");
        if (sizes[i] > mx) mx = sizes[i];
        tot += sizes[i] * (size_t)(t.parts[i] + (t.src2[i] ? t.parts2[i] : 0));
    }
    t.count = count;
    t.bump = bump;
    int gx = (int)cdivz(mx, (size_t)kBlock * 16);
    if (gx < 1) gx = 1;
    if (gx > 512) gx = 512;
    GGAN_LAUNCH("pack", 0, 4.0 * tot + 4.0 * mx, pack_k, dim3(gx, count), dim3(kBlock), 0, (hipStream_t)stream, t, flat);
    return 0;
}

int ggan_pack_adam(const float* const* srcs, const size_t* sizes, const size_t* offsets, const int* parts, const size_t* strides,
                   const float* const* srcs2, const int* parts2, const size_t* strides2, int count, float* flat, float* theta,
                   float* m, float* v, int32_t* step, int32_t* arrive, float lr, float beta1, float beta2, float eps,
                   float grad_scale, ggan_stream_t stream) {
    GGAN_CHECK_ARG(srcs && sizes && offsets && flat && theta && m && v && step, "null pointer");
    GGAN_CHECK_ARG(count > 0 && count <= GGAN_PACK_MAX, "count out of range");
    PackTable t;
    size_t mx = 0, tot = 0, all = 0;
    for (int i = 0; i < count; ++i) {
        t.src[i] = srcs[i]; t.size[i] = sizes[i]; t.off[i] = offsets[i];
        t.parts[i] = parts ? parts[i] : 1;
        t.pstride[i] = strides ? strides[i] : 0;
        t.src2[i] = srcs2 ? srcs2[i] : nullptr;
        t.parts2[i] = (srcs2 && parts2) ? parts2[i] : 1;
        t.pstride2[i] = (srcs2 && strides2) ? strides2[i] : 0;
        GGAN_CHECK_ARG(t.parts[i] >= 1 && t.parts2[i] >= 1, "parts must be >= 1");
        if (sizes[i] > mx) mx = sizes[i];
        tot += sizes[i] * (size_t)(t.parts[i] + (t.src2[i] ? t.parts2[i] : 0));
        all += sizes[i];
    }
    t.count = count;
    t.bump = step;
    int nb = 0;
    for (int i = 0; i < count; ++i) {
        t.first[i] = nb;
        nb += (int)cdivz(sizes[i] > 0 ? sizes[i] : 1, (size_t)pack_chunk(t.parts[i] + (t.src2[i] ? t.parts2[i] : 0)));
    }
    t.first[count] = nb;
    (void)mx;
    GGAN_LAUNCH("pack_adam", 0, 4.0 * tot + 28.0 * all, pack_adam_k, dim3(nb), dim3(kBlock), 0, (hipStream_t)stream, t, flat, theta,
                m, v, arrive, lr, beta1, beta2, eps, grad_scale);
    return 0;
}

int ggan_pack_parts(const float* const* srcs, const size_t* sizes, const size_t* offsets, const int* parts,
                    const size_t* strides, int count, float* flat, int32_t* bump, ggan_stream_t stream) {
    return ggan_pack_parts2(srcs, sizes, offsets, parts, strides, nullptr, nullptr, nullptr, count, flat, bump, stream);
}

int ggan_pack(const float* const* srcs, const size_t* sizes, const size_t* offsets, int count, float* flat, ggan_stream_t stream) {
    return ggan_pack_parts(srcs, sizes, offsets, nullptr, nullptr, count, flat, nullptr, stream);
}

int ggan_gmm_latent_fwd(const float* z, const float* mu, const float* gumbel_u, float* logits, float* k, int B, int K, int D,
                        float log_pi, float temp, ggan_stream_t stream) {
    GGAN_CHECK_ARG(z && mu && gumbel_u && k, "null pointer");
    GGAN_CHECK_ARG(B > 0 && K > 0 && K <= kGmmMaxK && D > 0 && temp > 0.f, "bad shape");
    GGAN_LAUNCH("gmm_latent_fwd", 3.0 * B * K * D, 0, gmm_latent_fwd_k, dim3(B), dim3(256), 0, (hipStream_t)stream, z, mu, gumbel_u, logits, k,
                K, D, log_pi, 1.f / temp);
    return 0;
}

int ggan_gmm_latent_bwd(const float* z, const float* mu, const float* k, const float* g_logits, const float* g_k, float* dz,
                        float* dmu, int B, int K, int D, float temp, ggan_stream_t stream) {
    GGAN_CHECK_ARG(z && mu && k && (g_logits || g_k) && (dz || dmu), "null pointer");
    GGAN_CHECK_ARG(B > 0 && B <= kGmmMaxK && K > 0 && K <= kGmmMaxK && D > 0 && temp > 0.f, "bad shape");
    GGAN_LAUNCH("gmm_latent_bwd", 4.0 * B * K * D, 0, gmm_latent_bwd_k, dim3(B + (dmu ? K : 0)), dim3(256), 0, (hipStream_t)stream, z, mu, k,
                g_logits, g_k, dz, dmu, B, K, D, 1.f / temp);
    return 0;
}

int ggan_gmm_latent_st_fwd(const float* z, const float* mu, const float* gumbel_u, float* logits, float* k, float* soft, int B, int K,
                           int D, float log_pi, float temp, int mode, ggan_stream_t stream) {
    GGAN_CHECK_ARG(mode == GGAN_MODE_K_STC || mode == GGAN_MODE_K_ST, "mode is not a straight-through MODE_K");
    GGAN_CHECK_ARG(z && mu && k && (mode == GGAN_MODE_K_ST || (gumbel_u && soft)), "null pointer");
    GGAN_CHECK_ARG(B > 0 && K > 0 && K <= kGmmMaxK && D > 0 && (mode == GGAN_MODE_K_ST || temp > 0.f), "bad shape");
    if (mode == GGAN_MODE_K_STC) {
        GGAN_LAUNCH("gmm_latent_stc_fwd", 3.0 * B * K * D, 0, gmm_latent_st_fwd_k<kModeKStc>, dim3(B), dim3(256), 0, (hipStream_t)stream, z,
                    mu, gumbel_u, logits, k, soft, K, D, log_pi, 1.f / temp);
    } else {
        GGAN_LAUNCH("gmm_latent_st_fwd", 3.0 * B * K * D, 0, gmm_latent_st_fwd_k<kModeKSt>, dim3(B), dim3(256), 0, (hipStream_t)stream, z,
                    mu, nullptr, logits, k, nullptr, K, D, log_pi, 1.f);
    }
    return 0;
}

int ggan_gmm_latent_st_bwd(const float* z, const float* mu, const float* soft, const float* g_logits, const float* g_k, float* dz,
                           float* dmu, int B, int K, int D, float temp, int mode, ggan_stream_t stream) {
    GGAN_CHECK_ARG(mode == GGAN_MODE_K_STC || mode == GGAN_MODE_K_ST, "mode is not a straight-through MODE_K");
    GGAN_CHECK_ARG(z && mu && (mode == GGAN_MODE_K_ST || soft) && (g_logits || g_k) && (dz || dmu), "null pointer");
    GGAN_CHECK_ARG(B > 0 && B <= kGmmMaxK && K > 0 && K <= kGmmMaxK && D > 0 && (mode == GGAN_MODE_K_ST || temp > 0.f), "bad shape");
    if (mode == GGAN_MODE_K_STC)
        return ggan_gmm_latent_bwd(z, mu, soft, g_logits, g_k, dz, dmu, B, K, D, temp, stream);
// ... 127 lines not shown
```

graphical_gan_amd/functional/__init__.py:

```python

from ._core import (
    C, os, weakref, torch, Function, once_differentiable, _lib, ACT_NONE, ACT_LRELU, ACT_RELU, ACT_TANH, ACT_SIGMOID, ConvGeom,
    check, _WS, _WS_BYTES, _L, _p, _stream, _dev, _c, _DEFER, _DATA_ONLY, _is_param, data_grad_only,
    _skip_undefined, defer_wgrad_reduce, _wgrad_parts, _STREAMS, shared_stream, workspace, _PLAN, _PLAIN, _SERIAL_BWD, target_workgroups,
    launch_hint, serial_backward, _remembers_plan, force_plain,
    same_geometry, conv_geom, _geom, _SITE, site_scope, site_plan, RowSlot, _new_out, _adjacent, HEAD_LOGITS, _PENDING_COSTS, _tail_value, settle_cost,
    pending_costs, drop_pending_costs, UNIT_SEEDS, unit_seed, is_unit_seed, LATE_EXT, _LATE_TERMS, mark_ready, wait_ready, add_late_terms,
    drop_late_terms)
from .pointwise import ActFwd, ActBwd, leaky_relu, relu, tanh, sigmoid
from .conv import (
    DEBUG_POISON_CHECK, PendingCast, ConvFwd, _fused_conv_backward, ConvDgrad, ConvDgradMasked, ConvWgrad, ChanSum, TALL_ROWS,
    ColSum)
from .linear import (
    Gemm, _fused_linear_backward, Gemm2, _CONSTS, cached_const, Gemm2Dgrad, _HEAD_HINT, head_bce_hint, CriticHead, DynScan,
    gemm_colsum_, linear)
from .norm import BatchNormTrain, BatchNormGroupedTrain, BatchNormBwd, LinearBatchNormRows, _all_gather_rows, SyncBatchNormTrain
from .rows import (
    JoinRows, Fanout, fanout, SplitRows, CastScaleI32, Axpby, MixMean, GmmLatent, GmmLatentST, MixRbfMmd2, Reparam, AGG_KL, AGG_IKL, AGG_JSD,
    AggDiv, RowLerp, gmm_posterior_assign_, cluster_accuracy_, sheet_grid, video_sheet_u8)
from .conv3d import _dims3, Im2Col3d, Col2Im3d, _conv3d_patch, _igemm_ok, Conv3dImplicit, conv3d
from .losses import BceSum, Distance, MeanSum, GradPenalty
from .optim_ops import adam_step_, rmsprop_step_, NOISE_NORMAL, NOISE_UNIFORM, NOISE_ONEHOT, noise_state, noise_fill_, pack_
from .tsne import (
    tsne, tsne_splits, tsne_neighbours, tsne_affinities, tsne_symmetrise, tsne_gradient, tsne_kl, tsne_step, tsne_affinity_graph)
```

graphical_gan_amd/functional/linear.py:

```python
import ctypes as C
import os
import threading as _threading
import torch
import weakref
from .. import _lib
from torch.autograd import Function
from torch.autograd.function import once_differentiable
from .._lib import ACT_NONE, check
from ._core import (
    _L, _p, _stream, _c, _DATA_ONLY, _is_param, _skip_undefined, workspace, _new_out, HEAD_LOGITS, _PENDING_COSTS,
    _tail_value)
from .pointwise import ActBwd
from .conv import TALL_ROWS, ColSum


@_skip_undefined
class Gemm(Function):

    @staticmethod
    def forward(ctx, a, b, bias, ta, tb, act, alpha, slot=None):
        a, b = _c(a), _c(b)
        M, K = (a.shape[1], a.shape[0]) if ta else (a.shape[0], a.shape[1])
        K2, N = (b.shape[1], b.shape[0]) if tb else (b.shape[0], b.shape[1])
        assert K == K2, (a.shape, b.shape, ta, tb)
# ... 135 lines not shown

class Gemm2Dgrad(Function):

    @staticmethod
    def forward(ctx, g, w, K1):
        g, w = _c(g), _c(w)
        M, N = g.shape
        K = w.shape[0]
        da1 = torch.empty((M, K1), dtype=torch.float32, device=g.device)
        da2 = torch.empty((M, K - K1), dtype=torch.float32, device=g.device)
        ws = workspace(g.device)
        check(_L().ggan_gemm_split(0, 1, M, K, N, _p(g), _p(None), 0, _p(w), _p(None), _p(da1), _p(da2), K1, _p(None), ACT_NONE, 0.0,
                                   _p(ws), ws.numel(), _stream()), 'ggan_gemm_split')
        ctx.K1 = K1
        ctx.w_param = _is_param(w)
        ctx.set_materialize_grads(False)
        ctx.save_for_backward(g, w)
        return da1, da2

    @staticmethod
    def backward(ctx, h1, h2):
        if h1 is None and h2 is None:
            return None, None, None
        g, w = ctx.saved_tensors
        K1 = ctx.K1
        M, N = g.shape
        K = w.shape[0]
        h1 = _c(h1) if h1 is not None else cached_const(0.0, (M, K1), g.device)
        h2 = _c(h2) if h2 is not None else cached_const(0.0, (M, K - K1), g.device)
        dg = dw = None
        if ctx.needs_input_grad[0]:
            dg = Gemm2.apply(h1, h2, w, None, ACT_NONE, 0.0)
        if ctx.needs_input_grad[1] and not (_DATA_ONLY[0] and ctx.w_param):
            if torch.is_grad_enabled():
                dw = Gemm.apply(torch.cat([h1, h2], 1), g, None, True, False, ACT_NONE, 0.0)
            else:
                dw = torch.empty((K, N), dtype=torch.float32, device=g.device)
                ws = workspace(g.device)
                check(_L().ggan_gemm_split(1, 0, K, N, M, _p(h1), _p(h2), K1, _p(g), _p(None), _p(dw), _p(None), 0, _p(None), ACT_NONE,
                                           0.0, _p(ws), ws.numel(), _stream()), 'ggan_gemm_split')
        return dg, dw, None


_HEAD_HINT = _threading.local()


class head_bce_hint(object):

    def __init__(self, terms, kind='bce'):
        self.terms = (kind, tuple((int(n), float(z), float(w)) for n, z, w in terms)) if terms else None

    def __enter__(self):
        self.prev = getattr(_HEAD_HINT, 'terms', None)
        _HEAD_HINT.terms = self.terms
        return self

    def __exit__(self, *exc):
        _HEAD_HINT.terms = self.prev
        return False


@_skip_undefined
class CriticHead(Function):

    @staticmethod
    def forward(ctx, a1, a2, w, b, w_out, b_out, alpha):
        a1, w, b, w_out, b_out = _c(a1), _c(w), _c(b), _c(w_out), _c(b_out)
        a2 = _c(a2) if a2 is not None else None
        M, K1 = a1.shape
        K2 = a2.shape[1] if a2 is not None else 0
        H = w.shape[1]
        assert w.shape[0] == K1 + K2 and w_out.numel() == H and b.numel() == H, (a1.shape, w.shape, w_out.shape)
        h = torch.empty((M, H), dtype=torch.float32, device=a1.device)
        logits = torch.empty((M,), dtype=torch.float32, device=a1.device)
        ws = workspace(a1.device)
        registers = M <= _lib.HEAD_BCE_MAX_ROWS and any(ctx.needs_input_grad) and not os.environ.get('GGAN_NO_HEAD_BCE')
        hint = getattr(_HEAD_HINT, 'terms', None)
        hinted = None
        hkind, hterms = hint if hint is not None else (None, ())
        if (registers and hint is not None and 1 <= len(hterms) <= 3 and sum(n for n, _, _ in hterms) == M and H <= 2048
                and not os.environ.get('GGAN_NO_HEAD_HINT')):
            g = torch.empty((M,), dtype=torch.float32, device=a1.device)
            gh = torch.empty((M, H), dtype=torch.float32, device=a1.device)
            nt = len(hterms)
            tabs = ((C.c_int * nt)(*[n for n, _, _ in hterms]), (C.c_float * nt)(*[z for _, z, _ in hterms]),
                    (C.c_float * nt)(*[wt for _, _, wt in hterms]))
            check(_L().ggan_critic_head_fwd_bce(M, K1, K2, H, _p(a1), _p(a2), _p(w), _p(b), _p(w_out), _p(b_out), float(alpha), _p(h),
                                                _p(logits), 1 if hkind == 'mean' else 0, nt, tabs[0], tabs[1], tabs[2], _p(g), _p(gh), _p(ws),
                                                ws.numel(), _stream()), 'ggan_critic_head_fwd_bce')
            hinted = dict(kind=hkind, terms=hterms, g=g, gh=gh)
        else:
            check(_L().ggan_critic_head_fwd(M, K1, K2, H, _p(a1), _p(a2), _p(w), _p(b), _p(w_out), _p(b_out), float(alpha), _p(h),
                                            _p(logits), _p(ws), ws.numel(), _stream()), 'ggan_critic_head_fwd')
        ctx.alpha, ctx.has_a2 = float(alpha), a2 is not None
        ctx.save_for_backward(a1, a2, w, w_out, h)
        ctx.rec = None
        if registers:
            ctx.rec = dict(ptr=logits.data_ptr(), M=M, H=H, h=weakref.ref(h), w_out=weakref.ref(w_out), alpha=float(alpha),
                           want_out=ctx.needs_input_grad[4],
                           want_bout=ctx.needs_input_grad[5], g_ptr=None, hinted=hinted, tail=None)
            if len(HEAD_LOGITS) >= 8:
                HEAD_LOGITS.clear()
            HEAD_LOGITS[ctx.rec['ptr']] = ctx.rec
        return logits

    @staticmethod
    @once_differentiable
    def backward(ctx, g):
        a1, a2, w, w_out, h = ctx.saved_tensors
        g = _c(g)
        M, K1 = a1.shape
        K2 = a2.shape[1] if a2 is not None else 0
        H = w.shape[1]
        need = ctx.needs_input_grad
        dev = g.device
        new = lambda *shape: torch.empty(shape, dtype=torch.float32, device=dev)
        rec = ctx.rec
        fused = rec is not None and rec['g_ptr'] is not None and rec['g_ptr'] == g.data_ptr() and rec.get('g_version') == g._version
        gh = rec['gh'] if fused else new(M, H)
        want_a = need[0] or (a2 is not None and need[1])
        d_a1 = new(M, K1) if want_a else None
        d_a2 = new(M, K2) if (want_a and a2 is not None) else None
        d_w = new(K1 + K2, H) if (need[2] or need[3]) else None
        d_b = new(H) if need[3] else None
        d_wout = (rec['d_wout'].view(w_out.shape) if fused else new(*w_out.shape)) if need[4] else None
        d_bout = (rec['d_bout'] if fused else new(1)) if need[5] else None
        ws = workspace(dev)
        tail = rec.get('tail') if rec is not None else None
        if tail is not None:
            rec['tail'] = None
            if tail.get('loss') is not None:
                _PENDING_COSTS.pop(tail['loss'].data_ptr(), None)
            if fused:
                nt = len(tail['terms'])
                tabs = ((C.c_int * nt)(*[n for n, _, _ in tail['terms']]), (C.c_float * nt)(*[z for _, z, _ in tail['terms']]),
                        (C.c_float * nt)(*[wt for _, _, wt in tail['terms']]))
                ext = tail.get('ext')
                pext = (C.c_void_p * nt)(*[(e.data_ptr() if e is not None else 0) for e in ext]) if ext else None
                check(_L().ggan_critic_head_bwd_tail(M, K1, K2, H, _p(a1), _p(a2), _p(w), _p(h), _p(w_out), ctx.alpha, _p(gh), _p(d_a1), _p(d_a2),
                                                     _p(d_w), _p(d_b), _p(d_wout), _p(d_bout), _p(tail['logits']), _p(tail['g']),
                                                     1 if tail.get('kind') == 'mean' else 0, nt, tabs[0], tabs[1], tabs[2], pext,
                                                     _p(tail['loss']), _p(ws), ws.numel(), _stream()), 'ggan_critic_head_bwd_tail')
                return (d_a1 if need[0] else None, d_a2 if (a2 is not None and need[1]) else None, d_w if need[2] else None, d_b, d_wout,
                        d_bout, None)
            if tail.get('loss') is not None:
                _tail_value(tail)
        check(_L().ggan_critic_head_bwd(M, K1, K2, H, _p(None if fused else g), _p(a1), _p(a2), _p(w), _p(h), _p(w_out), ctx.alpha, _p(gh), _p(d_a1),
                                        _p(d_a2), _p(d_w), _p(d_b), _p(d_wout), _p(d_bout), _p(ws), ws.numel(), _stream()),
              'ggan_critic_head_bwd')
        return (d_a1 if need[0] else None, d_a2 if (a2 is not None and need[1]) else None, d_w if need[2] else None, d_b, d_wout,
                d_bout, None)


class DynScan(Function):

    @staticmethod
    def usable(z0, eps, w_1):
        return w_1.shape[0] == 256 and w_1.shape[1] == 256 and z0.shape[1] <= 16 and eps.shape[1] <= 16

    @staticmethod
    def forward(ctx, z0, eps, w_in, b_in, w_1, b_1, w_out, b_out, zw, b_zw, T, alpha):
        z0, eps, w_in, b_in, w_1, b_1, w_out, b_out = (_c(t) for t in (z0, eps, w_in, b_in, w_1, b_1, w_out, b_out))
        zw, b_zw = (_c(zw), _c(b_zw)) if zw is not None else (None, None)
        B, dl = z0.shape
        dt, Hd = eps.shape[1], w_1.shape[0]
        assert w_in.shape == (dl + dt, Hd) and w_out.shape == (Hd, dl), (w_in.shape, w_out.shape)
        new = lambda *shape: torch.empty(shape, dtype=torch.float32, device=z0.device)
        zs, h1, h2 = new(B, T + 1, dl), new(T, B, Hd), new(T, B, Hd)
        check(_L().ggan_dyn_scan_fwd(B, T, dl, dt, Hd, _p(z0), _p(eps), _p(w_in), _p(b_in), _p(w_1), _p(b_1), _p(w_out), _p(b_out),
                                     _p(zw), _p(b_zw), float(alpha), _p(zs), _p(h1), _p(h2), _stream()), 'ggan_dyn_scan_fwd')
        ctx.T, ctx.alpha = T, float(alpha)
        ctx.save_for_backward(eps, w_in, w_1, w_out, zw, zs, h1, h2)
        return zs

    @staticmethod
    @once_differentiable
    def backward(ctx, g_zs):
        eps, w_in, w_1, w_out, zw, zs, h1, h2 = ctx.saved_tensors
        g_zs = _c(g_zs)
        B, T1, dl = zs.shape
        T, dt, Hd = T1 - 1, eps.shape[1], w_1.shape[0]
        new = lambda *shape: torch.empty(shape, dtype=torch.float32, device=zs.device)
        G1, G2, Go, Xin = new(T * B, Hd), new(T * B, Hd), new(T * B, dl), new(T * B, dl + dt)
        d_z0, d_eps = new(B, dl), new(B, dt)
        check(_L().ggan_dyn_scan_bwd(B, T, dl, dt, Hd, _p(g_zs), _p(zs), _p(eps), _p(h1), _p(h2), _p(w_in), _p(w_1), _p(w_out), _p(zw),
                                     ctx.alpha, _p(G1), _p(G2), _p(Go), _p(Xin), _p(d_z0), _p(d_eps), _stream()), 'ggan_dyn_scan_bwd')
        need = ctx.needs_input_grad
        d_win = d_bin = d_w1 = d_b1 = d_wout = d_bout = d_zw = d_bzw = None
        if need[2] or need[3]:
            d_win, d_bin = gemm_colsum_(Xin, G1, True)
        if need[4] or need[5]:
            d_w1, d_b1 = gemm_colsum_(h1.view(T * B, Hd), G2, True)
        if need[6] or need[7] or need[9]:
            d_wout, d_bout = gemm_colsum_(h2.view(T * B, Hd), Go, True)
        if zw is not None and need[8]:
            d_zw = Gemm.apply(Xin[:, :dl].contiguous(), Go, None, True, False, ACT_NONE, 0.0)
            d_bzw = d_bout
        return (d_z0 if need[0] else None, d_eps if need[1] else None, d_win, d_bin, d_w1, d_b1, d_wout, d_bout, d_zw, d_bzw,
                None, None)


def gemm_colsum_(a, g, ta):
    a, g = _c(a), _c(g)
    M, K = (a.shape[1], a.shape[0]) if ta else (a.shape[0], a.shape[1])
    K2, N = g.shape
    assert K == K2
    out = torch.empty((M, N), dtype=torch.float32, device=a.device)
    cs = torch.empty((N,), dtype=torch.float32, device=a.device)
    ws = workspace(a.device)
    check(_L().ggan_gemm_colsum(int(ta), M, N, K, _p(a), _p(g), _p(out), _p(cs), _p(ws), ws.numel(), _stream()),
          'ggan_gemm_colsum')
    return out, cs


def linear(x, w, bias=None, act=ACT_NONE, alpha=0.0):
    return Gemm.apply(x, w, bias, False, False, act, alpha)
```

graphical_gan_amd/tflib/ops/linear.py:

```python
import numpy as np

from ... import functional as F
from .. import param as _param
from .. import initial_values_needed as _draw

_default_weightnorm = False


def enable_default_weightnorm():
    global _default_weightnorm
    _default_weightnorm = True


def disable_default_weightnorm():
    global _default_weightnorm
    _default_weightnorm = False


_weights_stdev = None


def set_weights_stdev(weights_stdev):
    global _weights_stdev
    _weights_stdev = weights_stdev


def unset_weights_stdev():
    global _weights_stdev
    _weights_stdev = None


def _uniform(stdev, size):
    if _weights_stdev is not None:
        stdev = _weights_stdev
    return np.random.uniform(low=-stdev * np.sqrt(3), high=stdev * np.sqrt(3), size=size).astype('float32')


def _initial(initialization, input_dim, output_dim):
    if initialization == 'lecun':
        return _uniform(np.sqrt(1. / input_dim), (input_dim, output_dim))
    if initialization == 'glorot' or initialization is None:
        return _uniform(np.sqrt(2. / (input_dim + output_dim)), (input_dim, output_dim))
    if initialization == 'he':
        return _uniform(np.sqrt(2. / input_dim), (input_dim, output_dim))
    if initialization == 'glorot_he':
        return _uniform(np.sqrt(4. / (input_dim + output_dim)), (input_dim, output_dim))
    if initialization == 'orthogonal':
        a = np.random.normal(0.0, 1.0, (input_dim, output_dim))
        u, _, v = np.linalg.svd(a, full_matrices=False)
        q = u if u.shape == (input_dim, output_dim) else v
        return q.reshape((input_dim, output_dim)).astype('float32')
    if initialization[0] == 'uniform':
        return np.random.uniform(low=-initialization[1], high=initialization[1],
                                 size=(input_dim, output_dim)).astype('float32')
    raise Exception('Invalid initialization!')


def Linear(name, input_dim, output_dim, inputs, biases=True, initialization=None, weightnorm=None, gain=1.,
           activation=None, alpha=0.2, out=None):
    if _draw(name + '.W'):
        weight_values = _initial(initialization, input_dim, output_dim)
        weight_values *= gain
    else:
        weight_values = None
    weight = _param(name + '.W', weight_values)
    if weightnorm is None:
        weightnorm = _default_weightnorm
    if weightnorm:
        norm_values = np.sqrt(np.sum(np.square(weight_values), axis=0)) if weight_values is not None else None
        target_norms = _param(name + '.g', norm_values)
        norms = (weight * weight).sum(dim=0).sqrt()
        weight = weight * (target_norms / norms)
    b = _param(name + '.b', np.zeros((output_dim,), dtype='float32')) if biases else None
    act = F.ACT_NONE if activation is None else activation
    if isinstance(inputs, (tuple, list)):
        x1, x2 = inputs
        assert x1.dim() == 2 and x2.dim() == 2 and x1.shape[1] + x2.shape[1] == input_dim, (name, x1.shape, x2.shape, input_dim)
        if out is None and F.Gemm2.usable(x1, x2):
            return F.Gemm2.apply(x1, x2, weight, b, act, float(alpha))
        import torch
        inputs = torch.cat([x1, x2], 1)
    x = inputs if inputs.dim() == 2 else inputs.reshape(-1, input_dim)
    result = F.Gemm.apply(x, weight, b, False, False, act, float(alpha), out)
    if inputs.dim() != 2:
        result = result.reshape(tuple(inputs.shape[:-1]) + (output_dim,))
    return result


def LinearLReLULinear(name1, input_dim, hidden_dim, name2, inputs, alpha=0.2, differentiable=False):
    pair = isinstance(inputs, (tuple, list))
    x1, x2 = inputs if pair else (inputs, None)
    usable = (not differentiable and x1.dim() == 2 and hidden_dim % 4 == 0
              and (x2 is None or (x2.dim() == 2 and F.Gemm2.usable(x1, x2))))
    if not usable:
        h = Linear(name1, input_dim, hidden_dim, inputs, activation=F.ACT_LRELU, alpha=alpha)
        return Linear(name2, hidden_dim, 1, h).reshape(-1)
    w1 = _param(name1 + '.W', _initial(None, input_dim, hidden_dim) if _draw(name1 + '.W') else None)
    b1 = _param(name1 + '.b', np.zeros((hidden_dim,), dtype='float32'))
    w2 = _param(name2 + '.W', _initial(None, hidden_dim, 1) if _draw(name2 + '.W') else None)
    b2 = _param(name2 + '.b', np.zeros((1,), dtype='float32'))
    assert x1.shape[1] + (x2.shape[1] if x2 is not None else 0) == input_dim, (name1, x1.shape, input_dim)
    return F.CriticHead.apply(x1, x2, w1, b1, w2, b2, float(alpha))


def linear_params(name, input_dim, output_dim):
    w = _param(name + '.W', _initial(None, input_dim, output_dim) if _draw(name + '.W') else None)
    b = _param(name + '.b', np.zeros((output_dim,), dtype='float32'))
    return w, b


def LinearBatchnormRows(name, input_dim, output_dim, inputs, bn_name, activation=None, alpha=0.2):
    from . import batchnorm
    w = _param(name + '.W', _initial(None, input_dim, output_dim) if _draw(name + '.W') else None)
    b = _param(name + '.b', np.zeros((output_dim,), dtype='float32'))
    x = inputs if inputs.dim() == 2 else inputs.reshape(-1, input_dim)
    act = F.ACT_NONE if activation is None else activation
    if batchnorm._SYNC_GROUP in (None, False) and F.LinearBatchNormRows.usable(x, w):
        shape = [1, output_dim]
        offset = _param(bn_name + '.offset', np.zeros(shape, dtype='float32'))
        scale = _param(bn_name + '.scale', np.ones(shape, dtype='float32'))
        return F.LinearBatchNormRows.apply(x, w, b, scale, offset, 1e-5, act, float(alpha))
    out = F.Gemm.apply(x, w, b, False, False, F.ACT_NONE, 0.0, None)
    return batchnorm.Batchnorm(bn_name, [0], out, activation=activation, alpha=alpha)
```

include/ggan.h:

```cpp
#ifndef GGAN_H
#define GGAN_H
#include <stddef.h>
#include <stdint.h>

#ifdef __cplusplus
extern "C" {
#endif

typedef void* ggan_stream_t;
#define GGAN_WS_RESERVED 16384

enum { GGAN_ACT_NONE = 0, GGAN_ACT_LRELU = 1, GGAN_ACT_RELU = 2, GGAN_ACT_TANH = 3, GGAN_ACT_SIGMOID = 4 };

#define GGAN_ABI_VERSION 800
int ggan_version(void);
const char* ggan_last_error(void);
typedef struct {
    int N, Ci, H, W;
    int Co, Ho, Wo;
    int k, stride, pad_t, pad_l;
    int plan_wgs, plan_wgs_filter, plan_flags;
} ggan_conv_geom;
#define GGAN_PLAN_PLAIN 1

size_t ggan_conv2d_workspace(const ggan_conv_geom* g);
int ggan_conv2d_fwd(const ggan_conv_geom* g, const float* x, const float* w, const float* bias,
                    float* y, int act, float alpha, void* ws, size_t ws_bytes, ggan_stream_t stream);
int ggan_conv2d_bwd_data(const ggan_conv_geom* g, const float* gy, const float* w, const float* bias,
                         float* gx, int act, float alpha, void* ws, size_t ws_bytes, ggan_stream_t stream);
int ggan_conv2d_bwd_filter(const ggan_conv_geom* g, const float* x, const float* gy, float* gw,
                           float* gbias, void* ws, size_t ws_bytes, ggan_stream_t stream);
int ggan_conv2d_bwd_data_act(const ggan_conv_geom* g, const float* gy, const float* y, int y_act, float y_alpha,
                             const float* w, float* gx, void* ws, size_t ws_bytes, ggan_stream_t stream);
int ggan_conv2d_bwd_filter_act(const ggan_conv_geom* g, const float* x, const float* gy, const float* y, int y_act,
                               float y_alpha, float* gw, float* gbias, void* ws, size_t ws_bytes, ggan_stream_t stream);
int ggan_conv2d_bwd_filter_parts(const ggan_conv_geom* g, const float* x, const float* gy, const float* y, int y_act,
                                 float y_alpha, int with_bias, float* part, size_t part_cap, int* n_parts,
                                 size_t* stride, ggan_stream_t stream);

int ggan_deconv2d_fwd(const ggan_conv_geom* g, const float* x_small, const float* w, const float* bias,
                      float* y_big, int act, float alpha, void* ws, size_t ws_bytes, ggan_stream_t stream);
int ggan_deconv2d_bwd_data(const ggan_conv_geom* g, const float* gy_big, const float* w, float* gx_small,
                           void* ws, size_t ws_bytes, ggan_stream_t stream);
int ggan_deconv2d_bwd_filter(const ggan_conv_geom* g, const float* gy_big, const float* x_small, float* gw,
                             float* gbias , void* ws, size_t ws_bytes,
                             ggan_stream_t stream);

int ggan_linear_bwd_data_act(int M, int N, int K, const float* g, const float* y, int y_act, float y_alpha,
                             const float* w, float* dx, void* ws, size_t ws_bytes, ggan_stream_t stream);
int ggan_linear_bwd_weight_act(int M, int N, int K, const float* x, const float* g, const float* y, int y_act,
                               float y_alpha, float* dw, float* db, void* ws, size_t ws_bytes, ggan_stream_t stream);

int ggan_gemm_split(int ta, int tb, int M, int N, int K, const float* A, const float* A2, int a_split, const float* B,
                    const float* bias, float* C, float* C2, int c_split, float* colsum_b, int act, float alpha, void* ws,
                    size_t ws_bytes, ggan_stream_t stream);

int ggan_dyn_scan_fwd(int B, int T, int dl, int dt, int H, const float* z0, const float* eps, const float* w_in, const float* b_in,
                      const float* w_1, const float* b_1, const float* w_out, const float* b_out, const float* zw, const float* b_zw,
                      float alpha, float* zs, float* h1, float* h2, ggan_stream_t stream);
int ggan_dyn_scan_bwd(int B, int T, int dl, int dt, int H, const float* g_zs, const float* zs, const float* eps, const float* h1,
                      const float* h2, const float* w_in, const float* w_1, const float* w_out, const float* zw, float alpha, float* G1,
                      float* G2, float* Go, float* Xin, float* d_z0, float* d_eps, ggan_stream_t stream);

int ggan_critic_head_fwd(int M, int K1, int K2, int H, const float* a1, const float* a2, const float* w, const float* b,
                         const float* w_out, const float* b_out, float alpha, float* h, float* logits, void* ws, size_t ws_bytes,
                         ggan_stream_t stream);
int ggan_critic_head_bwd(int M, int K1, int K2, int H, const float* g, const float* a1, const float* a2, const float* w, const float* h,
                         const float* w_out, float alpha, float* gh, float* d_a1, float* d_a2, float* d_w, float* d_b, float* d_wout,
                         float* d_bout, void* ws, size_t ws_bytes, ggan_stream_t stream);

int ggan_critic_head_fwd_bce(int M, int K1, int K2, int H, const float* a1, const float* a2, const float* w, const float* b,
                             const float* w_out, const float* b_out, float alpha, float* h, float* logits, int kind, int nterms,
                             const int* term_rows, const float* labels, const float* weights, float* g, float* gh, void* ws,
                             size_t ws_bytes, ggan_stream_t stream);
int ggan_critic_head_bwd_tail(int M, int K1, int K2, int H, const float* a1, const float* a2, const float* w, const float* h,
                              const float* w_out, float alpha, const float* gh, float* d_a1, float* d_a2, float* d_w, float* d_b,
                              float* d_wout, float* d_bout, const float* logits, const float* g, int kind, int nterms, const int* term_rows,
                              const float* labels, const float* weights, const float* const* ext, float* loss, void* ws, size_t ws_bytes,
                              ggan_stream_t stream);

size_t ggan_gemm_workspace(int M, int N, int K);
int ggan_gemm(int ta, int tb, int M, int N, int K, const float* A, const float* B, const float* bias,
              float* C, int act, float alpha, void* ws, size_t ws_bytes, ggan_stream_t stream);
int ggan_gemm_colsum(int ta, int M, int N, int K, const float* A, const float* B, float* C, float* colsum_b,
                     void* ws, size_t ws_bytes, ggan_stream_t stream);
int ggan_colsum(const float* x, float* out, int rows, int cols, ggan_stream_t stream);
int ggan_colsum_tall(const float* x, float* out, int rows, int cols, void* ws, size_t ws_bytes, ggan_stream_t stream);
int ggan_chansum(const float* x, float* out, int N, int C, int HW, void* ws, size_t ws_bytes, ggan_stream_t stream);

int ggan_bn_fwd_train(const float* x, const float* scale, const float* offset, float* y,
                      float* save_mean, float* save_invstd, int N, int C, int HW, float eps,
                      int act, float alpha, ggan_stream_t stream);
int ggan_bn_bwd(const float* x, const float* gy, const float* scale, const float* save_mean,
                const float* save_invstd, float* gx, float* gscale, float* goffset,
                int N, int C, int HW, ggan_stream_t stream);
int ggan_bn_bwd_act(const float* x, const float* gy, const float* y, int y_act, float y_alpha, const float* scale,
                    const float* save_mean, const float* save_invstd, float* gx, float* gscale, float* goffset,
                    float* gx_chansum, int N, int C, int HW, ggan_stream_t stream);

int ggan_conv2d_fwd_masked(const ggan_conv_geom* g, const float* x, const float* w, float* y, const float* yref, int ref_act,
                           float ref_alpha, void* ws, size_t ws_bytes, ggan_stream_t stream);

int ggan_linear_bn_rows_fwd(const float* x, const float* w, const float* b, const float* scale, const float* offset, float* h,
                            float* y, float* save_mean, float* save_invstd, int M, int K, int N, float eps, int act,
                            float alpha, ggan_stream_t stream);
int ggan_linear_bn_rows_bwd(const float* x, const float* gy, const float* h, const float* y, const float* scale, const float* save_mean,
                            const float* save_invstd, float* dw, float* db, float* dscale, float* doffset, int M, int K, int N, int act,
                            float alpha, ggan_stream_t stream);

int ggan_bn_bwd_bwd(const float* x, const float* gy, const float* y, int y_act, float y_alpha, const float* h, const float* scale,
                    const float* save_mean, const float* save_invstd, float* ggy, float* gx2, float* gscale2, int N, int C, int HW,
                    ggan_stream_t stream);

int ggan_bn_split_fwd_train(const float* x, const float* scale, const float* offset, float* y, float* save_mean, float* save_invstd,
                            int N, int C, int HW, int groups, float eps, int act, float alpha, void* ws, size_t ws_bytes,
                            ggan_stream_t stream);
int ggan_bn_split_bwd_act(const float* x, const float* gy, int act, float alpha, const float* scale, const float* offset,
                          const float* save_mean, const float* save_invstd, float* gx, float* gscale, float* goffset,
                          float* gx_chansum, int N, int C, int HW, int groups, int gx_groups, void* ws, size_t ws_bytes,
                          ggan_stream_t stream);

int ggan_bn_sync_stats(const float* x, float* stats, int N, int C, int HW, ggan_stream_t stream);
int ggan_bn_sync_apply(const float* x, const float* stats, int world, const float* scale, const float* offset, float* y,
                       float* save_mean, float* save_invstd, int N, int C, int HW, float eps, int act, float alpha,
                       ggan_stream_t stream);
int ggan_bn_sync_bwd_stats(const float* x, const float* gy, const float* y, int y_act, float y_alpha, const float* save_mean,
                           const float* save_invstd, float* sums, int N, int C, int HW, ggan_stream_t stream);
int ggan_bn_sync_bwd_apply(const float* x, const float* gy, const float* y, int y_act, float y_alpha, const float* scale,
                           const float* save_mean, const float* save_invstd, const float* sums, int world, int rank, float* gx,
                           float* gscale, float* goffset, int N, int C, int HW, ggan_stream_t stream);

int ggan_act_fwd(const float* x, float* y, size_t n, int act, float alpha, ggan_stream_t stream);
int ggan_act_bwd(const float* gy, const float* ref, float* gx, size_t n, int act, float alpha,
                 ggan_stream_t stream);
int ggan_act_bwd_chansum(const float* gy, const float* ref, float* gx, float* parts, int parts_cap, int* n_parts, int N, int C, int HW,
                         int act, float alpha, ggan_stream_t stream);
int ggan_bias_add(const float* x, const float* bias, float* y, int N, int C, int HW, ggan_stream_t stream);
int ggan_cast_scale_i32(const int32_t* x, const float* noise , float* y, size_t n,
                        float div, float mul, ggan_stream_t stream);
int ggan_cast_scale_ring_i32(const int32_t* ring, int nslots, const int32_t* ctr_a, const int32_t* ctr_b, int offset,
                             const float* noise , float* y, size_t n, float div, float mul, ggan_stream_t stream);
int ggan_conv2d_fwd_cast_ring(const ggan_conv_geom* g, const int32_t* ring, int nslots, const int32_t* ctr_a, const int32_t* ctr_b, int offset,
                              const float* noise , float div, float mul, float* x_out, const float* w,
                              const float* bias , float* y, int act, float alpha, ggan_stream_t stream);
int ggan_mix_mean(const float* k, const float* mu, const float* noise, float* out, int B, int K, int D, ggan_stream_t stream);
int ggan_axpby(const float* x, const float* y, float* out, size_t n, float a, float b, float c,
               ggan_stream_t stream);
int ggan_row_lerp(const float* x, const float* y, const float* alpha, float* out, int rows, int cols,
                  ggan_stream_t stream);

int ggan_bce_logits_fwd(const float* x, float label, float weight, float* loss, int n, int accumulate,
                        ggan_stream_t stream);
int ggan_bce_logits_bwd(const float* x, float label, float weight, const float* gloss, float* gx, int n,
                        ggan_stream_t stream);
#define GGAN_BCE_MAX 16
int ggan_bce_logits_multi_fwd(const float* const* xs, const float* labels, const float* weights, const int* ns,
                              int count, float* loss, ggan_stream_t stream);
#define GGAN_HEAD_BCE_MAX_ROWS 2048
int ggan_bce_head_bwd(const float* const* xs, const float* labels, const float* weights, const int* ns, int count, float* loss,
                      float* const* gxs, int M, int H, const float* h, const float* w_out, float alpha, float* gh, float* d_wout,
                      float* d_bout, ggan_stream_t stream);
#define GGAN_BCE_HEADS 2
int ggan_bce_heads_bwd(const float* const* xs, const float* labels, const float* weights, const int* ns, int count, float* loss,
                       float* const* gxs, int nheads, const int* head_terms, const int* Ms, const int* Hs, const float* const* hs,
                       const float* const* w_outs, const float* alphas, float* const* ghs, float* const* d_wouts ,
                       float* const* d_bouts , ggan_stream_t stream);
int ggan_bce_logits_multi_bwd(const float* const* xs, const float* labels, const float* weights, const int* ns,
                              int count, const float* gloss, float* const* gxs, ggan_stream_t stream);
int ggan_bce_logits_multi_fwd_grad(const float* const* xs, const float* labels, const float* weights, const int* ns,
                                   int count, float* loss, float* const* gxs, ggan_stream_t stream);
int ggan_mean_fwd(const float* x, float weight, float* loss, int n, int accumulate, ggan_stream_t stream);
int ggan_mean_bwd(const float* gloss, float weight, float* gx, int n, ggan_stream_t stream);
int ggan_mean_multi_fwd_grad(const float* const* xs, const float* weights, const int* ns, int count, float* loss,
                             float* const* gxs , ggan_stream_t stream);

int ggan_conv3d_out_shape(const int* dims10, int* lo_ho_wo);
int ggan_im2col3d(const int* dims10, const float* x, float* col, ggan_stream_t stream);
int ggan_col2im3d(const int* dims10, const float* col, float* gx, ggan_stream_t stream);
int ggan_conv3d_igemm_ok(const int* dims10, int kind);
int ggan_conv3d_fwd(const int* dims10, const float* x, const float* w, const float* bias , float* y, int act,
                    float alpha, void* ws, size_t ws_bytes, ggan_stream_t stream);
int ggan_conv3d_wgrad(const int* dims10, const float* x, const float* gy, float* gw, void* ws, size_t ws_bytes,
                      ggan_stream_t stream);
int ggan_conv3d_dgrad(const int* dims10, const float* gy, const float* w, float* gx, ggan_stream_t stream);

int ggan_mix_rbf_mmd2_fwd(const float* X, const float* Y, int m, int n, int d, const float* sigmas, const float* wts, int ns,
                          float* out, float* row_scratch, ggan_stream_t stream);
int ggan_mix_rbf_mmd2_bwd(const float* X, const float* Y, int m, int n, int d, const float* sigmas, const float* wts, int ns,
                          const float* gout, float* dX, float* dY, ggan_stream_t stream);

int ggan_reparam_fwd(const float* mean, const float* log_std, const float* eps, float* z, float* std_out, size_t n, ggan_stream_t stream);
int ggan_reparam_bwd(const float* gz, const float* gstd, const float* eps, const float* std_in, float* gmean, float* glog_std, size_t n,
                     ggan_stream_t stream);

int ggan_agg_div_fwd(int kind, const float* mu, const float* sd, const float* k_onehot, const float* eps_q, const float* z_p, int nx, int nz,
                     int d, int n_coms, float* out, float* Z, float* A, float* Bv, float* T, ggan_stream_t stream);
int ggan_agg_div_bwd(int kind, const float* mu, const float* sd, const float* k_onehot, const float* eps_q, int nx, int nz, int d, int n_coms,
                     const float* Z, const float* A, const float* Bv, const float* gout, float* W, float* GZ, float* gmu, float* gsd,
                     ggan_stream_t stream);

#define GGAN_NOISE_MAX 16
int ggan_noise_fill(float* const* dsts, const size_t* sizes, const int* kinds, const float* a, const float* b, const int* widths,
                    int count, uint64_t* state, ggan_stream_t stream);
int ggan_gmm_latent_fwd(const float* z, const float* mu, const float* gumbel_u, float* logits, float* k, int B, int K, int D,
                        float log_pi, float temp, ggan_stream_t stream);
int ggan_gmm_latent_bwd(const float* z, const float* mu, const float* k, const float* g_logits, const float* g_k, float* dz,
                        float* dmu, int B, int K, int D, float temp, ggan_stream_t stream);
enum { GGAN_MODE_K_CONCRETE = 0, GGAN_MODE_K_STC = 1, GGAN_MODE_K_ST = 2 };
int ggan_gmm_latent_st_fwd(const float* z, const float* mu, const float* gumbel_u, float* logits, float* k, float* soft, int B, int K,
                           int D, float log_pi, float temp, int mode, ggan_stream_t stream);
int ggan_gmm_latent_st_bwd(const float* z, const float* mu, const float* soft, const float* g_logits, const float* g_k, float* dz,
                           float* dmu, int B, int K, int D, float temp, int mode, ggan_stream_t stream);
#define GGAN_POSTERIOR_MAX_K 8192
int ggan_gmm_posterior_assign(const float* z, const float* mu, float log_pi, int B, int K, int D, int row0, float* probs,
                              int32_t* assign, uint64_t* colbest, ggan_stream_t stream);
int ggan_cluster_accuracy(const int32_t* assign, const int32_t* labels, const uint64_t* colbest, int N, int K, int32_t* correct,
                          ggan_stream_t stream);
int ggan_video_sheet_u8(const float* gen, const float* data, uint8_t* sheet, uint8_t* gif, int n, int rows, int LEN, int C, int H, int W,
                        int nh, int nw, int interleave, float a, float b, float d, ggan_stream_t stream);

#define GGAN_TSNE_MAX_K 128
#define GGAN_TSNE_MAX_SPLITS 64
// ... 59 lines not shown
```

Baseline: 17270 images/sec.

## Add fused twice-differentiable critic head for gradient-penalty path

Adds a fused critic head (linear, LReLU, linear) that supports double backward, so the WGAN-GP gradient-penalty path no longer falls back to two separate Linear layers. New kernels fuse the split-K reduction with bias, activation and the output dot product, and fuse the double-backward computation of the output-weight and g gradients. Uncommon cases fall back to composed Gemm ops. This is meant to cut kernel launches and intermediate traffic in the critic's GP step, at the cost of extra code and slightly different float summation order.

```diff
diff --git a/graphical_gan_amd/_lib.py b/graphical_gan_amd/_lib.py
--- a/graphical_gan_amd/_lib.py
+++ b/graphical_gan_amd/_lib.py
@@ -91,6 +91,9 @@
     'ggan_critic_head_bwd': (_I, [_I, _I, _I, _I, _P, _P, _P, _P, _P, _P, _F, _P, _P, _P, _P, _P, _P, _P, _P, _Z, _P]),
     'ggan_critic_head_fwd_bce': (_I, [_I, _I, _I, _I, _P, _P, _P, _P, _P, _P, _F, _P, _P, _I, _I, _P, _P, _P, _P, _P, _P, _Z, _P]),
     'ggan_critic_head_bwd_tail': (_I, [_I, _I, _I, _I, _P, _P, _P, _P, _P, _F, _P, _P, _P, _P, _P, _P, _P, _P, _P, _I, _I, _P, _P, _P, _P, _P, _P, _Z, _P]),
+    'ggan_critic_head_twice_fwd': (_I, [_I, _I, _I, _I, _P, _P, _P, _P, _P, _P, _F, _P, _P, _P, _Z, _P]),
+    'ggan_critic_head_dgrad': (_I, [_I, _I, _I, _I, _P, _P, _P, _P, _F, _P, _P, _P, _P, _Z, _P]),
+    'ggan_critic_head_dgrad_bwd': (_I, [_I, _I, _I, _I, _P, _P, _P, _P, _P, _P, _F, _P, _P, _P, _P, _Z, _P]),
     'ggan_linear_bwd_data_act': (_I, [_I, _I, _I, _P, _P, _I, _F, _P, _P, _P, _Z, _P]),
     'ggan_linear_bwd_weight_act': (_I, [_I, _I, _I, _P, _P, _P, _I, _F, _P, _P, _P, _Z, _P]),
     'ggan_colsum': (_I, [_P, _P, _I, _I, _P]),
diff --git a/graphical_gan_amd/csrc/conv.h b/graphical_gan_amd/csrc/conv.h
--- a/graphical_gan_amd/csrc/conv.h
+++ b/graphical_gan_amd/csrc/conv.h
@@ -54,6 +54,7 @@
 size_t conv_workspace_bytes(const ggan_conv_geom& g);
 int launch_splitk_reduce(const float* partial, int SK, size_t elems, float* out, const float* bias, int C, int HW, int act,
                          float alpha, hipStream_t s, size_t slab_stride = 0, float* tail_out = nullptr, size_t tail = 0);
+inline bool splitk_reduce_is_small(int SK, size_t n) { return SK >= 8 && n <= 65536; }
 
 struct FastDiv {
     uint32_t mul, d;
diff --git a/graphical_gan_amd/csrc/conv_corr.hip b/graphical_gan_amd/csrc/conv_corr.hip
--- a/graphical_gan_amd/csrc/conv_corr.hip
+++ b/graphical_gan_amd/csrc/conv_corr.hip
@@ -1086,7 +1086,7 @@
                          float alpha, hipStream_t s, size_t slab_stride, float* tail_out, size_t tail) {
     if (slab_stride == 0) slab_stride = elems;
     if (!tail_out) tail = 0;
-    if (SK >= 8 && elems + tail <= 65536) {
+    if (splitk_reduce_is_small(SK, elems + tail)) {
         GGAN_LAUNCH("splitk_reduce_small_k", 0, 4.0 * (elems + tail) * (SK + 1), splitk_reduce_small_k,
                     dim3((int)((elems + tail + 63) / 64)), dim3(256), 0, s, partial, SK, elems, slab_stride, out, bias, C, HW, act,
                     alpha, tail_out, tail);
diff --git a/graphical_gan_amd/csrc/gemm.hip b/graphical_gan_amd/csrc/gemm.hip
--- a/graphical_gan_amd/csrc/gemm.hip
+++ b/graphical_gan_amd/csrc/gemm.hip
@@ -577,6 +577,156 @@
     if (lane == 0) C[row] = act_apply(s + (bias ? bias[0] : 0.f), act, alpha);
 }
 
+template <bool G4>
+__global__ __launch_bounds__(256) void head_twice_fwd_k(const float* __restrict__ part, int SK, size_t slab, const float* __restrict__ b,
+                                                        const float* __restrict__ w_out, const float* __restrict__ b_out, float alpha,
+                                                        float* __restrict__ h, float* __restrict__ logits, int M, int H) {
+    __shared__ float red[4];
+    const int tid = threadIdx.x, rl = tid >> 7, t = tid & 127;
+    const int row = blockIdx.x * 2 + rl;
+    float dot = 0.f;
+    if (row < M) {
+        for (int c = t * 4; c < H; c += 512) {
+            const size_t o = (size_t)row * H + c;
+            float4 v;
+            if (SK == 0) {
+                v = *reinterpret_cast<const float4*>(h + o);
+            } else {
+                if (G4) {
+                    float4 g[4];
+#pragma unroll
+                    for (int k = 0; k < 4; ++k) g[k] = make_float4(0.f, 0.f, 0.f, 0.f);
+                    for (int s0 = 0; s0 < SK; s0 += 16) {
+                        float4 u[16];
+#pragma unroll
+                        for (int k = 0; k < 16; ++k)
+                            u[k] = *reinterpret_cast<const float4*>(part + (size_t)(s0 + k < SK ? s0 + k : SK - 1) * slab + o);
+#pragma unroll
+                        for (int k = 0; k < 16; ++k) {
+                            if (s0 + k < SK) { g[k & 3].x += u[k].x; g[k & 3].y += u[k].y; g[k & 3].z += u[k].z; g[k & 3].w += u[k].w; }
+                        }
+                    }
+                    v.x = (g[0].x + g[1].x) + (g[2].x + g[3].x); v.y = (g[0].y + g[1].y) + (g[2].y + g[3].y);
+                    v.z = (g[0].z + g[1].z) + (g[2].z + g[3].z); v.w = (g[0].w + g[1].w) + (g[2].w + g[3].w);
+                } else {
+                    v = make_float4(0.f, 0.f, 0.f, 0.f);
+#pragma unroll 8
+                    for (int s = 0; s < SK; ++s) {
+                        const float4 u = *reinterpret_cast<const float4*>(part + (size_t)s * slab + o);
+                        v.x += u.x; v.y += u.y; v.z += u.z; v.w += u.w;
+                    }
+                }
+                const float4 bb = *reinterpret_cast<const float4*>(b + c);
+                v.x += bb.x; v.y += bb.y; v.z += bb.z; v.w += bb.w;
+                v.x = act_apply(v.x, GGAN_ACT_LRELU, alpha); v.y = act_apply(v.y, GGAN_ACT_LRELU, alpha);
+                v.z = act_apply(v.z, GGAN_ACT_LRELU, alpha); v.w = act_apply(v.w, GGAN_ACT_LRELU, alpha);
+                *reinterpret_cast<float4*>(h + o) = v;
+            }
+            const float4 ww = *reinterpret_cast<const float4*>(w_out + c);
+            dot = fmaf(v.x, ww.x, fmaf(v.y, ww.y, fmaf(v.z, ww.z, fmaf(v.w, ww.w, dot))));
+        }
+    }
+    dot = wave_sum(dot);
+    if ((tid & 63) == 0) red[tid >> 6] = dot;
+    __syncthreads();
+    if (t == 0 && row < M) logits[row] = (red[2 * rl] + red[2 * rl + 1]) + b_out[0];
+}
+
+constexpr int kHeadTwiceRows = 512;
+template <bool G4>
+__device__ __forceinline__ float4 slab_sum4(const float* __restrict__ part, int SK, size_t slab, size_t o) {
+    if (SK == 0) return *reinterpret_cast<const float4*>(part + o);
+    float4 v;
+    if (G4) {
+        float4 g[4];
+#pragma unroll
+        for (int k = 0; k < 4; ++k) g[k] = make_float4(0.f, 0.f, 0.f, 0.f);
+        for (int s0 = 0; s0 < SK; s0 += 16) {
+            float4 u[16];
+#pragma unroll
+            for (int k = 0; k < 16; ++k) u[k] = *reinterpret_cast<const float4*>(part + (size_t)(s0 + k < SK ? s0 + k : SK - 1) * slab + o);
+#pragma unroll
+            for (int k = 0; k < 16; ++k)
+                if (s0 + k < SK) { g[k & 3].x += u[k].x; g[k & 3].y += u[k].y; g[k & 3].z += u[k].z; g[k & 3].w += u[k].w; }
+        }
+        v.x = (g[0].x + g[1].x) + (g[2].x + g[3].x); v.y = (g[0].y + g[1].y) + (g[2].y + g[3].y);
+        v.z = (g[0].z + g[1].z) + (g[2].z + g[3].z); v.w = (g[0].w + g[1].w) + (g[2].w + g[3].w);
+    } else {
+        v = make_float4(0.f, 0.f, 0.f, 0.f);
+#pragma unroll 8
+        for (int s = 0; s < SK; ++s) {
+            const float4 u = *reinterpret_cast<const float4*>(part + (size_t)s * slab + o);
+            v.x += u.x; v.y += u.y; v.z += u.z; v.w += u.w;
+        }
+    }
+    return v;
+}
+
+template <bool G4>
+__global__ __launch_bounds__(256) void head_twice_bwd2_k(const float* __restrict__ part, int SK, size_t slab, const float* __restrict__ g,
+                                                         const float* __restrict__ h, const float* __restrict__ w_out, float alpha,
+                                                         float* __restrict__ d_wout, float* __restrict__ d_g, int M, int H, int ncol,
+                                                         int wk, int WS, int W4) {
+    __shared__ __attribute__((aligned(16))) float tm[kHeadTwiceRows][16];
+    __shared__ float ps[32][16];
+    const int tid = threadIdx.x;
+    if ((int)blockIdx.x >= ncol) {
+        const int rl = tid >> 7, t = tid & 127;
+        const int row = ((int)blockIdx.x - ncol) * 2 + rl;
+        float dot = 0.f;
+        if (row < M) {
+            for (int c = t * 4; c < H; c += 512) {
+                const size_t o = (size_t)row * H + c;
+                const float4 v = slab_sum4<G4>(part, SK, slab, o);
+                const float4 hv = *reinterpret_cast<const float4*>(h + o);
+                const float4 ww = *reinterpret_cast<const float4*>(w_out + c);
+                const float a0 = v.x * (hv.x > 0.f ? 1.f : alpha), a1 = v.y * (hv.y > 0.f ? 1.f : alpha);
+                const float a2 = v.z * (hv.z > 0.f ? 1.f : alpha), a3 = v.w * (hv.w > 0.f ? 1.f : alpha);
+                dot = fmaf(a0, ww.x, fmaf(a1, ww.y, fmaf(a2, ww.z, fmaf(a3, ww.w, dot))));
+            }
+        }
+        dot = wave_sum(dot);
+        if ((tid & 63) == 0) ps[0][tid >> 6] = dot;
+        __syncthreads();
+        if (t == 0 && row < M) d_g[row] = ps[0][2 * rl] + ps[0][2 * rl + 1];
+        return;
+    }
+    const int q = tid & 3, rs = tid >> 2;
+    const int c = blockIdx.x * 16 + 4 * q;
+    for (int r = rs; r < M; r += 64) {
+        float4 v = make_float4(0.f, 0.f, 0.f, 0.f);
+        if (c < H) {
+            const size_t o = (size_t)r * H + c;
+            v = slab_sum4<G4>(part, SK, slab, o);
+            const float4 hv = *reinterpret_cast<const float4*>(h + o);
+            v.x *= hv.x > 0.f ? 1.f : alpha; v.y *= hv.y > 0.f ? 1.f : alpha; v.z *= hv.z > 0.f ? 1.f : alpha; v.w *= hv.w > 0.f ? 1.f : alpha;
+        }
+        *reinterpret_cast<float4*>(&tm[r][4 * q]) = v;
+    }
+    __syncthreads();
+    const int cl = tid & 15, sj = tid >> 4;
+    for (int j = sj; j < WS; j += 16) {
+        float acc = 0.f;
+        const int r1 = min((j + 1) * wk, M);
+        for (int r = j * wk; r < r1; ++r) acc = fmaf(tm[r][cl], g[r], acc);
+        ps[j][cl] = acc;
+    }
+    __syncthreads();
+    if (tid < 16 && (int)blockIdx.x * 16 + tid < H) {
+        float v;
+        if (WS == 1) v = ps[0][tid];
+        else if (W4) {
+            float s4[4] = {0.f, 0.f, 0.f, 0.f};
+            for (int j = 0; j < WS; ++j) s4[j & 3] += ps[j][tid];
+            v = (s4[0] + s4[1]) + (s4[2] + s4[3]);
+        } else {
+            v = 0.f;
+            for (int j = 0; j < WS; ++j) v += ps[j][tid];
+        }
+        d_wout[blockIdx.x * 16 + tid] = v;
+    }
+}
+
 struct SkinnyParams {
     const float* A; const float* B; const float* bias; float* C; const float* a_ref;
     const float* A2;
@@ -761,6 +911,13 @@
     return 0;
 }
 
+static bool skinny_shape(int ta, int tb, int M, int N, int K, bool colsum, bool a_ref, bool b_ref, bool A2, int a_split, bool C2, int c_split) {
+    const int big = cdiv(M, BM) * cdiv(N, BN), small = cdiv(M, 16) * cdiv(N, 16);
+    const bool fits = big < 64 && small <= 1024;
+    return !ta && !colsum && (!A2 || (a_split % 16 == 0 && !a_ref)) && (!C2 || c_split % 16 == 0) && !b_ref && (!a_ref || tb) && M >= 32 &&
+           K >= 64 && K <= 1024 && fits && !(K <= 128 && big >= 32) && (size_t)M * K * 4 < 0x7FFFFFF0ull && (size_t)N * K * 4 < 0x7FFFFFF0ull;
+}
+
 static int gemm_launch(int ta, int tb, int M, int N, int K, const float* A, const float* B, const float* bias, float* C,
                        float* colsum, int act, float alpha, void* ws, size_t ws_bytes, hipStream_t s,
                        const float* a_ref = nullptr, const float* b_ref = nullptr, int ref_act = 0, float ref_alpha = 0.f,
@@ -769,10 +926,7 @@
         GGAN_LAUNCH("gemv_rows_k", 2.0 * M * K, 0, gemv_rows_k, dim3(cdiv(M, 4)), dim3(256), 0, s, A, B, bias, C, M, K, act, alpha);
         return 0;
     }
-    if (!ta && !colsum && (!A2 || (a_split % 16 == 0 && !a_ref)) && (!C2 || c_split % 16 == 0) && !b_ref && (!a_ref || tb) && M >= 32 &&
-        K >= 64 && K <= 1024 && cdiv(M, BM) * cdiv(N, BN) < 64 &&
-        cdiv(M, 16) * cdiv(N, 16) <= 1024 && !(K <= 128 && cdiv(M, BM) * cdiv(N, BN) >= 32) && (size_t)M * K * 4 < 0x7FFFFFF0ull &&
-        (size_t)N * K * 4 < 0x7FFFFFF0ull) {
+    if (skinny_shape(ta, tb, M, N, K, colsum != nullptr, a_ref != nullptr, b_ref != nullptr, A2 != nullptr, a_split, C2 != nullptr, c_split)) {
         SkinnyParams P;
         memset(&P, 0, sizeof(P));
         P.A = A; P.B = B; P.bias = bias; P.C = C; P.a_ref = a_ref;
@@ -958,6 +1112,125 @@
                                 d_bout, ws, ws_bytes, stream, &T);
 }
 
+int ggan_critic_head_twice_fwd(int M, int K1, int K2, int H, const float* a1, const float* a2, const float* w, const float* b,
+                               const float* w_out, const float* b_out, float alpha, float* h, float* logits, void* ws, size_t ws_bytes,
+                               ggan_stream_t stream) {
+    GGAN_CHECK_ARG(a1 && w && b && w_out && b_out && h && logits, "null pointer");
+    GGAN_CHECK_ARG(M > 0 && K1 > 0 && K2 >= 0 && H > 0 && (H % 4) == 0 && (a2 || K2 == 0) && (K2 == 0 || K1 % 64 == 0), "bad shape");
+    GGAN_CHECK_ARG(al16(b) && al16(w_out) && al16(h), "b, w_out, h must be 16-byte aligned");
+    hipStream_t s = (hipStream_t)stream;
+    const int K = K1 + K2;
+    const float* A2 = K2 ? a2 : nullptr;
+    const int a_split = K2 ? K1 : 0;
+    const float* part = h;
+    int SK = 0;
+    size_t slab = 0;
+    if (skinny_shape(0, 0, M, H, K, false, false, false, A2 != nullptr, a_split, false, 0)) {
+        int rc = gemm_launch(0, 0, M, H, K, a1, w, b, h, nullptr, GGAN_ACT_LRELU, alpha, ws, ws_bytes, s, nullptr, nullptr, 0, 0.f, A2, a_split);
+        if (rc) return rc;
+    } else {
+        GemmPlan G;
+        int rc = gemm_plan(G, 0, 0, 0, M, H, K, a1, w, b, h, nullptr, GGAN_ACT_LRELU, alpha, ws, ws_bytes, nullptr, nullptr, 0, 0.f, A2, a_split);
+        if (rc) return rc;
+        GGAN_CHECK_ARG(G.P.SK == 1 || (al16(G.ws) && (G.P.slab_stride % 4) == 0), "slabs must be 16-byte aligned");
+        rc = gemm_launch_planned(G, 0, 0, s);
+        if (rc) return rc;
+        if (G.P.SK > 1) { part = (const float*)G.ws; SK = G.P.SK; slab = G.P.slab_stride; }
+    }
+    if (SK > 1 && splitk_reduce_is_small(SK, (size_t)M * H)) {
+        GGAN_LAUNCH("head_twice_fwd_k<4>", 2.0 * M * H, 4.0 * M * H * (SK + 1), head_twice_fwd_k<true>, dim3(cdiv(M, 2)), dim3(256), 0, s, part, SK,
+                    slab, b, w_out, b_out, alpha, h, logits, M, H);
+    } else {
+        GGAN_LAUNCH("head_twice_fwd_k<1>", 2.0 * M * H, 4.0 * M * H * (SK + 1), head_twice_fwd_k<false>, dim3(cdiv(M, 2)), dim3(256), 0, s, part, SK,
+                    slab, b, w_out, b_out, alpha, h, logits, M, H);
+    }
+    return 0;
+}
+
+int ggan_critic_head_dgrad(int M, int K1, int K2, int H, const float* g, const float* h, const float* w, const float* w_out, float alpha,
+                           float* gh, float* d_a1, float* d_a2, void* ws, size_t ws_bytes, ggan_stream_t stream) {
+    GGAN_CHECK_ARG(g && h && w && w_out && gh, "null pointer");
+    GGAN_CHECK_ARG(M > 0 && K1 > 0 && K2 >= 0 && H > 0 && (K2 > 0 || !d_a2) && (K2 == 0 || K1 % BN == 0), "bad shape");
+    hipStream_t s = (hipStream_t)stream;
+    GGAN_LAUNCH("head_out_bwd_k", 3.0 * M * H, 8.0 * M * H, head_out_bwd_k, dim3(cdiv(H, 16)), dim3(256), 0, s, g, h, w_out, alpha, gh,
+                (float*)nullptr, (float*)nullptr, M, H);
+    if (d_a1 && d_a2)
+        return gemm_launch(0, 1, M, K1 + K2, H, gh, w, nullptr, d_a1, nullptr, GGAN_ACT_NONE, 0.f, ws, ws_bytes, s, nullptr, nullptr, 0, 0.f,
+                           nullptr, 0, d_a2, K1);
+    if (!d_a1 && !d_a2) return 0;
+    const int N = d_a1 ? K1 : K2;
+    const float* B = d_a1 ? w : w + (size_t)K1 * H;
+    float* C = d_a1 ? d_a1 : d_a2;
+    if (K2 == 0 || skinny_shape(0, 1, M, K1 + K2, H, false, false, false, false, 0, true, K1))
+        return gemm_launch(0, 1, M, N, H, gh, B, nullptr, C, nullptr, GGAN_ACT_NONE, 0.f, ws, ws_bytes, s);
+    GemmPlan G;
+    int rc = gemm_plan(G, 1, 0, 1, M, N, H, gh, B, nullptr, C, nullptr, GGAN_ACT_NONE, 0.f, ws, ws_bytes);
+    if (rc) return rc;
+    return gemm_launch_planned(G, 0, 1, s);
+}
+
+int ggan_critic_head_dgrad_bwd(int M, int K1, int K2, int H, const float* v1, const float* v2, const float* w, const float* g,
+                               const float* h, const float* w_out, float alpha, float* t_buf, float* d_wout, float* d_g, void* ws,
+                               size_t ws_bytes, ggan_stream_t stream) {
+    GGAN_CHECK_ARG(w && g && h && w_out && t_buf && (v1 || v2), "null pointer");
+    GGAN_CHECK_ARG(M > 0 && M <= kHeadTwiceRows && K1 > 0 && K2 >= 0 && H > 0 && (H % 4) == 0 && (K2 > 0 || !v2) && (K2 == 0 || K1 % 64 == 0),
+                   "bad shape");
+    GGAN_CHECK_ARG(al16(h) && al16(w_out) && al16(t_buf), "h, w_out, t_buf must be 16-byte aligned");
+    if (!d_wout && !d_g) return 0;
+    if (!v1) return 1;
+    hipStream_t s = (hipStream_t)stream;
+    const int K = K1 + K2;
+    const bool cut = K2 > 0 && !v2;
+    const float* A2 = K2 ? (cut ? v1 : v2) : nullptr;
+    const int a_split = K2 ? K1 : 0;
+    GemmPlan W;
+    int rc = gemm_plan(W, 0, 1, 0, H, 1, M, t_buf, g, nullptr, t_buf, nullptr, GGAN_ACT_NONE, 0.f, ws, ws_bytes);
+    if (rc) return rc;
+    if (W.P.SK > 32 || (W.P.fast != 0 && W.P.kps >= 2 * KSTEP)) return 1;
+    const bool skinny = skinny_shape(0, 0, M, H, K, false, false, false, A2 != nullptr, a_split, false, 0);
+    GemmPlan G;
+    if (skinny) {
+        if (cut && !skinny_shape(0, 0, M, H, K1, false, false, false, false, 0, false, 0)) return 1;
+    } else {
+        rc = gemm_plan(G, 0, 0, 0, M, H, K, v1, w, nullptr, t_buf, nullptr, GGAN_ACT_NONE, 0.f, ws, ws_bytes, nullptr, nullptr, 0, 0.f, A2, a_split);
+        if (rc) return rc;
+        if (cut) {
+            GemmPlan F = G;
+            rc = gemm_plan(G, 0, 0, 0, M, H, K1, v1, w, nullptr, t_buf, nullptr, GGAN_ACT_NONE, 0.f, ws, ws_bytes);
+            if (rc) return rc;
+            if ((G.P.fast != 0) != (F.P.fast != 0) || K1 % F.P.kps % KSTEP != 0) return 1;
+            G.P.kps = F.P.kps;
+            G.P.SK = cdiv(K1, F.P.kps);
+            G.P.slab_stride = G.P.out_elems;
+            G.P.C = G.P.SK > 1 ? (float*)G.ws : t_buf;
+        }
+        if (G.P.SK > 1 && !(al16(G.ws) && (G.P.slab_stride % 4) == 0)) return 1;
+    }
+    const float* part = t_buf;
+    int SK = 0;
+    size_t slab = 0;
+    if (skinny) {
+        rc = cut ? gemm_launch(0, 0, M, H, K1, v1, w, nullptr, t_buf, nullptr, GGAN_ACT_NONE, 0.f, ws, ws_bytes, s)
+                 : gemm_launch(0, 0, M, H, K, v1, w, nullptr, t_buf, nullptr, GGAN_ACT_NONE, 0.f, ws, ws_bytes, s, nullptr, nullptr, 0, 0.f, A2, a_split);
+        if (rc) return rc;
+    } else {
+        rc = gemm_launch_planned(G, 0, 0, s);
+        if (rc) return rc;
+        if (G.P.SK > 1) { part = (const float*)G.ws; SK = G.P.SK; slab = G.P.slab_stride; }
+    }
+    const int w4 = W.P.SK > 1 && splitk_reduce_is_small(W.P.SK, (size_t)H) ? 1 : 0;
+    const int ncol = d_wout ? cdiv(H, 16) : 0;
+    const dim3 grid(ncol + (d_g ? cdiv(M, 2) : 0));
+    if (SK > 1 && splitk_reduce_is_small(cut ? cdiv(K, G.P.kps) : SK, (size_t)M * H)) {
+        GGAN_LAUNCH("head_twice_bwd2_k<4>", 4.0 * M * H, 4.0 * M * H * (SK + 1), head_twice_bwd2_k<true>, grid, dim3(256), 0, s, part, SK, slab, g, h,
+                    w_out, alpha, d_wout, d_g, M, H, ncol, W.P.kps, W.P.SK, w4);
+    } else {
+        GGAN_LAUNCH("head_twice_bwd2_k<1>", 4.0 * M * H, 4.0 * M * H * (SK + 1), head_twice_bwd2_k<false>, grid, dim3(256), 0, s, part, SK, slab, g, h,
+                    w_out, alpha, d_wout, d_g, M, H, ncol, W.P.kps, W.P.SK, w4);
+    }
+    return 0;
+}
+
 int ggan_gemm(int ta, int tb, int M, int N, int K, const float* A, const float* B, const float* bias, float* C, int act,
               float alpha, void* ws, size_t ws_bytes, ggan_stream_t stream) {
     GGAN_CHECK_ARG(A && B && C, "null pointer");
diff --git a/graphical_gan_amd/csrc/pointwise.hip b/graphical_gan_amd/csrc/pointwise.hip
--- a/graphical_gan_amd/csrc/pointwise.hip
+++ b/graphical_gan_amd/csrc/pointwise.hip
@@ -604,19 +604,46 @@
     if (threadIdx.x == 0) pen[0] = lam * (s / (float)B);
 }
 
-__global__ void gp_fwd_grad_k(const float* __restrict__ g, float* __restrict__ slopes, float* __restrict__ pen, float* __restrict__ gg,
-                              int32_t* __restrict__ arrive, int B, int D, float lam) {
+template <bool ONEPASS>
+__global__ __launch_bounds__(256) void gp_fwd_grad_k(const float* __restrict__ g, float* __restrict__ slopes, float* __restrict__ pen,
+                                                     float* __restrict__ gg, int32_t* __restrict__ arrive, int B, int D, float lam) {
     __shared__ float sm[32];
     __shared__ int last;
+    __shared__ __attribute__((aligned(16))) float rowbuf[ONEPASS ? 3072 : 4];
     const int b = blockIdx.x;
     const float* row = g + (size_t)b * D;
-    float s = 0.f;
-    for (int i = threadIdx.x; i < D; i += blockDim.x) s += row[i] * row[i];
-    s = block_sum(s, sm);
-    const float sl = sqrtf(s);
-    const float coef = lam * 2.f * (sl - 1.f) / ((float)B * sl);
     float* orow = gg + (size_t)b * D;
-    for (int i = threadIdx.x; i < D; i += blockDim.x) orow[i] = coef * row[i];
+    float sl;
+    if (ONEPASS) {
+        const int n4 = D >> 2;
+        float4 v[3];
+#pragma unroll
+        for (int j = 0; j < 3; ++j) {
+            const int i = threadIdx.x + 256 * j;
+            if (i < n4) {
+                v[j] = reinterpret_cast<const float4*>(row)[i];
+                reinterpret_cast<float4*>(rowbuf)[i] = v[j];
+            }
+        }
+        __syncthreads();
+        float s = 0.f;
+        for (int i = threadIdx.x; i < D; i += 256) s += rowbuf[i] * rowbuf[i];
+        s = block_sum(s, sm);
+        sl = sqrtf(s);
+        const float coef = lam * 2.f * (sl - 1.f) / ((float)B * sl);
+#pragma unroll
+        for (int j = 0; j < 3; ++j) {
+            const int i = threadIdx.x + 256 * j;
+            if (i < n4) reinterpret_cast<float4*>(orow)[i] = make_float4(coef * v[j].x, coef * v[j].y, coef * v[j].z, coef * v[j].w);
+        }
+    } else {
+        float s = 0.f;
+        for (int i = threadIdx.x; i < D; i += blockDim.x) s += row[i] * row[i];
+        s = block_sum(s, sm);
+        sl = sqrtf(s);
+        const float coef = lam * 2.f * (sl - 1.f) / ((float)B * sl);
+        for (int i = threadIdx.x; i < D; i += blockDim.x) orow[i] = coef * row[i];
+    }
     if (threadIdx.x == 0) {
         __hip_atomic_store(slopes + b, sl, __ATOMIC_RELAXED, __HIP_MEMORY_SCOPE_AGENT);
         __threadfence();
@@ -1577,8 +1604,13 @@
 int ggan_gp_penalty_fwd_grad(const float* g, float* slopes, float* pen, float* gg_unit, int32_t* arrive, int B, int D, float lam,
                              ggan_stream_t stream) {
     GGAN_CHECK_ARG(g && slopes && pen && gg_unit && arrive && B > 0 && D > 0, "bad argument");
-    GGAN_LAUNCH("gp_fwd_grad", 0, 8.0 * B * D, gp_fwd_grad_k, dim3(B), dim3(256), 0, (hipStream_t)stream, g, slopes, pen, gg_unit, arrive, B, D,
-                lam);
+    if (D % 4 == 0 && D <= 3072 && aligned16(g) && aligned16(gg_unit)) {
+        GGAN_LAUNCH("gp_fwd_grad", 0, 8.0 * B * D, gp_fwd_grad_k<true>, dim3(B), dim3(256), 0, (hipStream_t)stream, g, slopes, pen, gg_unit, arrive, B,
+                    D, lam);
+    } else {
+        GGAN_LAUNCH("gp_fwd_grad", 0, 8.0 * B * D, gp_fwd_grad_k<false>, dim3(B), dim3(256), 0, (hipStream_t)stream, g, slopes, pen, gg_unit, arrive, B,
+                    D, lam);
+    }
     return 0;
 }
 
diff --git a/graphical_gan_amd/functional/__init__.py b/graphical_gan_amd/functional/__init__.py
--- a/graphical_gan_amd/functional/__init__.py
+++ b/graphical_gan_amd/functional/__init__.py
@@ -12,7 +12,7 @@
     DEBUG_POISON_CHECK, PendingCast, ConvFwd, _fused_conv_backward, ConvDgrad, ConvDgradMasked, ConvWgrad, ChanSum, TALL_ROWS,
     ColSum)
 from .linear import (
-    Gemm, _fused_linear_backward, Gemm2, _CONSTS, cached_const, Gemm2Dgrad, _HEAD_HINT, head_bce_hint, CriticHead, DynScan,
+    Gemm, _fused_linear_backward, Gemm2, _CONSTS, cached_const, Gemm2Dgrad, _HEAD_HINT, head_bce_hint, CriticHead, CriticHeadTwice, CriticHeadDgrad, DynScan,
     gemm_colsum_, linear)
 from .norm import BatchNormTrain, BatchNormGroupedTrain, BatchNormBwd, LinearBatchNormRows, _all_gather_rows, SyncBatchNormTrain
 from .rows import (
diff --git a/graphical_gan_amd/functional/linear.py b/graphical_gan_amd/functional/linear.py
--- a/graphical_gan_amd/functional/linear.py
+++ b/graphical_gan_amd/functional/linear.py
@@ -311,6 +311,156 @@
                 d_bout, None)
 
 
+def _head_composed(a1, a2, w, b, w_out, b_out, alpha):
+    if a2 is not None:
+        h = Gemm2.apply(a1, a2, w, b, _lib.ACT_LRELU, alpha)
+    else:
+        h = Gemm.apply(a1, w, b, False, False, _lib.ACT_LRELU, alpha)
+    return Gemm.apply(h, w_out if w_out.dim() == 2 else w_out.reshape(-1, 1), b_out, False, False, ACT_NONE, 0.0).reshape(-1)
+
+
+@_skip_undefined
+class CriticHeadTwice(Function):
+
+    @staticmethod
+    def usable(a1, a2, H):
+        return (a1.dim() == 2 and a1.shape[0] <= 512 and H % 4 == 0 and (a2 is None or (a2.dim() == 2 and Gemm2.usable(a1, a2))))
+
+    @staticmethod
+    def forward(ctx, a1, a2, w, b, w_out, b_out, alpha):
+        given = (a1, a2, w, b, w_out, b_out)
+        a1, w, b, w_out, b_out = _c(a1), _c(w), _c(b), _c(w_out), _c(b_out)
+        a2 = _c(a2) if a2 is not None else None
+        M, K1 = a1.shape
+        K2 = a2.shape[1] if a2 is not None else 0
+        H = w.shape[1]
+        assert w.shape[0] == K1 + K2 and w_out.numel() == H and b.numel() == H, (a1.shape, w.shape, w_out.shape)
+        h = torch.empty((M, H), dtype=torch.float32, device=a1.device)
+        logits = torch.empty((M,), dtype=torch.float32, device=a1.device)
+        ws = workspace(a1.device)
+        check(_L().ggan_critic_head_twice_fwd(M, K1, K2, H, _p(a1), _p(a2), _p(w), _p(b), _p(w_out), _p(b_out), float(alpha), _p(h),
+                                              _p(logits), _p(ws), ws.numel(), _stream()), 'ggan_critic_head_twice_fwd')
+        ctx.alpha = float(alpha)
+        ctx.params = tuple(_is_param(t) for t in (w, b, w_out, b_out))
+        ctx.save_for_backward(*given, h)
+        return logits
+
+    @staticmethod
+    def backward(ctx, g):
+        a1, a2, w, b, w_out, b_out, h = ctx.saved_tensors
+        need = ctx.needs_input_grad
+        M, K1 = a1.shape
+        K2 = a2.shape[1] if a2 is not None else 0
+        H = w.shape[1]
+        if not torch.is_grad_enabled():
+            g, a1, w, w_out = _c(g), _c(a1), _c(w), _c(w_out)
+            a2 = _c(a2) if a2 is not None else None
+            new = lambda *shape: torch.empty(shape, dtype=torch.float32, device=g.device)
+            want_a = need[0] or (a2 is not None and need[1])
+            gh = new(M, H)
+            d_a1 = new(M, K1) if want_a else None
+            d_a2 = new(M, K2) if (want_a and a2 is not None) else None
+            d_w = new(K1 + K2, H) if (need[2] or need[3]) else None
+            d_b = new(H) if need[3] else None
+            d_wout = new(*w_out.shape) if need[4] else None
+            d_bout = new(1) if need[5] else None
+            ws = workspace(g.device)
+            check(_L().ggan_critic_head_bwd(M, K1, K2, H, _p(g), _p(a1), _p(a2), _p(w), _p(h), _p(w_out), ctx.alpha, _p(gh), _p(d_a1), _p(d_a2),
+                                            _p(d_w), _p(d_b), _p(d_wout), _p(d_bout), _p(ws), ws.numel(), _stream()), 'ggan_critic_head_bwd')
+            return (d_a1 if need[0] else None, d_a2 if (a2 is not None and need[1]) else None, d_w if need[2] else None, d_b, d_wout,
+                    d_bout, None)
+        wanted = [need[2 + i] and not (_DATA_ONLY[0] and ctx.params[i]) for i in range(4)]
+        if not any(wanted):
+            d_a1, d_a2 = CriticHeadDgrad.apply(g, h, w, w_out, K1, ctx.alpha, bool(need[0]), bool(a2 is not None and need[1]))
+            return d_a1, d_a2, None, None, None, None, None
+        ins = [a1, a2, w, b, w_out, b_out]
+        pick = [i for i in range(6) if ins[i] is not None and (need[i] if i < 2 else wanted[i - 2])]
+        got = torch.autograd.grad(_head_composed(a1, a2, w, b, w_out, b_out, ctx.alpha), [ins[i] for i in pick], g, create_graph=True,
+                                  allow_unused=True)
+        out = [None] * 7
+        for i, t in zip(pick, got):
+            out[i] = t
+        return tuple(out)
+
+
+class CriticHeadDgrad(Function):
+
+    @staticmethod
+    def forward(ctx, g, h, w, w_out, K1, alpha, want1, want2):
+        g, h, w, w_out = _c(g), _c(h), _c(w), _c(w_out)
+        M, H = h.shape
+        K2 = w.shape[0] - K1
+        gh = torch.empty((M, H), dtype=torch.float32, device=g.device)
+        da1 = torch.empty((M, K1), dtype=torch.float32, device=g.device) if want1 else None
+        da2 = torch.empty((M, K2), dtype=torch.float32, device=g.device) if (want2 and K2) else None
+        ws = workspace(g.device)
+        check(_L().ggan_critic_head_dgrad(M, K1, K2, H, _p(g), _p(h), _p(w), _p(w_out), float(alpha), _p(gh), _p(da1), _p(da2), _p(ws),
+                                          ws.numel(), _stream()), 'ggan_critic_head_dgrad')
+        ctx.K1, ctx.alpha = K1, float(alpha)
+        ctx.w_param, ctx.wout_param = _is_param(w), _is_param(w_out)
+        ctx.set_materialize_grads(False)
+        ctx.save_for_backward(g, h, w, w_out, gh)
+        return da1, da2
+
+    @staticmethod
+    def backward(ctx, v1, v2):
+        none = (None,) * 8
+        if v1 is None and v2 is None:
+            return none
+        g, h, w, w_out, gh = ctx.saved_tensors
+        K1 = ctx.K1
+        M, H = h.shape
+        K = w.shape[0]
+        need = ctx.needs_input_grad
+        want_w = need[2] and not (_DATA_ONLY[0] and ctx.w_param)
+        want_wout = need[3] and not (_DATA_ONLY[0] and ctx.wout_param)
+        if torch.is_grad_enabled():
+            ghd = ActBwd.apply(Gemm.apply(g.reshape(-1, 1), w_out.reshape(-1, 1), None, False, True, ACT_NONE, 0.0), h, _lib.ACT_LRELU, ctx.alpha)
+            da = Gemm.apply(ghd, w, None, False, True, ACT_NONE, 0.0)
+            outs, seeds = [], []
+            if v1 is not None:
+                outs.append(da[:, :K1]); seeds.append(v1)
+            if v2 is not None:
+                outs.append(da[:, K1:]); seeds.append(v2)
+            ins = [g, w, w_out]
+            pick = [i for i, ok in enumerate((need[0], want_w, want_wout)) if ok]
+            if not pick:
+                return none
+            got = torch.autograd.grad(outs, [ins[i] for i in pick], seeds, create_graph=True, allow_unused=True)
+            res = dict(zip(pick, got))
+            return (res.get(0), None, res.get(1), res.get(2)) + (None,) * 4
+        v1 = _c(v1) if v1 is not None else None
+        v2 = _c(v2) if v2 is not None else None
+        new = lambda *shape: torch.empty(shape, dtype=torch.float32, device=g.device)
+        zeros = lambda v, cols: v if (v is not None or not cols) else cached_const(0.0, (M, cols), g.device)
+        ws = workspace(g.device)
+        d_g = d_w = d_wout = None
+        if need[0] or want_wout:
+            d_g = new(*g.shape) if need[0] else None
+            d_wout = new(*w_out.shape) if want_wout else None
+            t_buf = new(M, H)
+            rc = _L().ggan_critic_head_dgrad_bwd(M, K1, K - K1, H, _p(v1), _p(v2), _p(w), _p(g), _p(h), _p(w_out), ctx.alpha, _p(t_buf),
+                                                 _p(d_wout), _p(d_g), _p(ws), ws.numel(), _stream())
+            if rc == 1:
+                z1, z2 = zeros(v1, K1), zeros(v2, K - K1)
+                t = Gemm2.apply(z1, z2, w, None, ACT_NONE, 0.0) if K > K1 else Gemm.apply(z1, w, None, False, False, ACT_NONE, 0.0)
+                tm = ActBwd.apply(t, h, _lib.ACT_LRELU, ctx.alpha)
+                if want_wout:
+                    d_wout = Gemm.apply(tm, g.reshape(-1, 1), None, True, False, ACT_NONE, 0.0).view(w_out.shape)
+                if need[0]:
+                    d_g = Gemm.apply(tm, w_out.reshape(-1, 1), None, False, False, ACT_NONE, 0.0).view(g.shape)
+            else:
+                check(rc, 'ggan_critic_head_dgrad_bwd')
+        if want_w:
+            d_w = new(K, H)
+            if K == K1:
+                check(_L().ggan_gemm(1, 0, K, H, M, _p(v1), _p(gh), _p(None), _p(d_w), ACT_NONE, 0.0, _p(ws), ws.numel(), _stream()), 'ggan_gemm')
+            else:
+                check(_L().ggan_gemm_split(1, 0, K, H, M, _p(zeros(v1, K1)), _p(zeros(v2, K - K1)), K1, _p(gh), _p(None), _p(d_w), _p(None), 0, _p(None),
+                                           ACT_NONE, 0.0, _p(ws), ws.numel(), _stream()), 'ggan_gemm_split')
+        return (d_g, None, d_w, d_wout) + (None,) * 4
+
+
 class DynScan(Function):
 
     @staticmethod
diff --git a/graphical_gan_amd/tflib/ops/linear.py b/graphical_gan_amd/tflib/ops/linear.py
--- a/graphical_gan_amd/tflib/ops/linear.py
+++ b/graphical_gan_amd/tflib/ops/linear.py
@@ -1,3 +1,5 @@
+import os
+
 import numpy as np
 
 from ... import functional as F
@@ -90,8 +92,8 @@
 def LinearLReLULinear(name1, input_dim, hidden_dim, name2, inputs, alpha=0.2, differentiable=False):
     pair = isinstance(inputs, (tuple, list))
     x1, x2 = inputs if pair else (inputs, None)
-    usable = (not differentiable and x1.dim() == 2 and hidden_dim % 4 == 0
-              and (x2 is None or (x2.dim() == 2 and F.Gemm2.usable(x1, x2))))
+    usable = (x1.dim() == 2 and hidden_dim % 4 == 0 and (x2 is None or (x2.dim() == 2 and F.Gemm2.usable(x1, x2)))
+              and not (differentiable and (os.environ.get('GGAN_NO_HEAD_TWICE') or not F.CriticHeadTwice.usable(x1, x2, hidden_dim))))
     if not usable:
         h = Linear(name1, input_dim, hidden_dim, inputs, activation=F.ACT_LRELU, alpha=alpha)
         return Linear(name2, hidden_dim, 1, h).reshape(-1)
@@ -100,7 +102,7 @@
     w2 = _param(name2 + '.W', _initial(None, hidden_dim, 1) if _draw(name2 + '.W') else None)
     b2 = _param(name2 + '.b', np.zeros((1,), dtype='float32'))
     assert x1.shape[1] + (x2.shape[1] if x2 is not None else 0) == input_dim, (name1, x1.shape, input_dim)
-    return F.CriticHead.apply(x1, x2, w1, b1, w2, b2, float(alpha))
+    return (F.CriticHeadTwice if differentiable else F.CriticHead).apply(x1, x2, w1, b1, w2, b2, float(alpha))
 
 
 def linear_params(name, input_dim, output_dim):
diff --git a/include/ggan.h b/include/ggan.h
--- a/include/ggan.h
+++ b/include/ggan.h
@@ -68,6 +68,15 @@
 int ggan_critic_head_bwd(int M, int K1, int K2, int H, const float* g, const float* a1, const float* a2, const float* w, const float* h,
                          const float* w_out, float alpha, float* gh, float* d_a1, float* d_a2, float* d_w, float* d_b, float* d_wout,
                          float* d_bout, void* ws, size_t ws_bytes, ggan_stream_t stream);
+
+int ggan_critic_head_twice_fwd(int M, int K1, int K2, int H, const float* a1, const float* a2, const float* w, const float* b,
+                               const float* w_out, const float* b_out, float alpha, float* h, float* logits, void* ws, size_t ws_bytes,
+                               ggan_stream_t stream);
+int ggan_critic_head_dgrad(int M, int K1, int K2, int H, const float* g, const float* h, const float* w, const float* w_out, float alpha,
+                           float* gh, float* d_a1, float* d_a2, void* ws, size_t ws_bytes, ggan_stream_t stream);
+int ggan_critic_head_dgrad_bwd(int M, int K1, int K2, int H, const float* v1, const float* v2, const float* w, const float* g,
+                               const float* h, const float* w_out, float alpha, float* t_buf, float* d_wout, float* d_g, void* ws,
+                               size_t ws_bytes, ggan_stream_t stream);
 
 int ggan_critic_head_fwd_bce(int M, int K1, int K2, int H, const float* a1, const float* a2, const float* w, const float* b,
                              const float* w_out, const float* b_out, float alpha, float* h, float* logits, int kind, int nterms,
```

Measured after the change: 17560 images/sec (median of 6 runs). 1.02x the previous value.
